# kamenbliznashki/chexpert

Measured on AMD Instinct MI355X. Metric: images/sec fwd+bwd DenseNet121 320x320 bf16 (per-GPU rate in config.images_per_sec_per_gpu), higher is better.
Workload: dtype bf16; 1 GPU; densenet121 bf16 1xMI355X 320x320 bs=256 per GPU, U-Ones labels (BASELINE configs[1]); 14 classes; random-init weights, synthetic uint8 X-rays; per_gpu_batch=256, global_batch=256, parallelism=dp1, rccl_ranks=1, capture_failed=0, launch=hipGraph replay

## Files before the change

chexpert_amd/_lib.py:

```python
import ctypes as C
import os

_HERE = os.path.dirname(os.path.abspath(__file__))
LIB_PATH = os.path.join(_HERE, "libchexpert_hip.so")

PRO_NONE, PRO_AFFINE_RELU, PRO_AFFINE2, PRO_JOIN = 0, 1, 2, 3
MODE_CONV, MODE_POOL2, MODE_STEM = 0, 1, 2
EPI_STORE, EPI_MASK, EPI_JOIN = 0, 1, 2

_vp, _fp, _i32 = C.c_void_p, C.c_void_p, C.c_int32


class CxConv(C.Structure):
    _fields_ = [("x", _vp), ("x2", _vp), ("w", _vp), ("y", _vp),
                ("pa", _fp), ("pb", _fp), ("pc", _fp),
                ("stat_sum", _fp), ("stat_sq", _fp),
                ("ex", _vp), ("e_sc", _fp), ("e_sh", _fp), ("e_mu", _fp), ("e_r", _fp), ("e_scale", _fp),
                ("B", _i32), ("H", _i32), ("W", _i32), ("Ho", _i32), ("Wo", _i32),
                ("K", _i32), ("N", _i32),
                ("ldx", _i32), ("ldx2", _i32), ("ldy", _i32), ("ldex", _i32),
                ("kh", _i32), ("kw", _i32), ("stride", _i32), ("pad", _i32),
                ("prologue", _i32), ("mode", _i32), ("epilogue", _i32), ("accumulate", _i32), ("tstride", _i32),
                ("stat_replicas", _i32), ("stat_rstride", _i32), ("stat_det", _i32), ("dtype", _i32),
                ("pro_out", _vp), ("ldpo", _i32), ("dil", _i32), ("emask", _vp),
                ("x3", _vp), ("po_lo", _vp), ("po_mask", _vp), ("kernel_hint", _i32), ("pad2_", _i32)]


class CxWgrad(C.Structure):
    _fields_ = [("g", _vp), ("g2", _vp), ("x", _vp), ("dw", _fp),
                ("ga", _fp), ("gb", _fp), ("gc", _fp), ("pa", _fp), ("pb", _fp),
                ("B", _i32), ("H", _i32), ("W", _i32), ("Ho", _i32), ("Wo", _i32), ("K", _i32), ("N", _i32),
                ("ldg", _i32), ("ldg2", _i32), ("ldx", _i32),
                ("kh", _i32), ("kw", _i32), ("stride", _i32), ("pad", _i32),
                ("g_prologue", _i32), ("x_prologue", _i32), ("mode", _i32), ("splits", _i32), ("dtype", _i32), ("dil", _i32),
                ("scratch", _fp), ("scratch_floats", C.c_int64), ("kernel_hint", _i32), ("pad_", _i32)]


WGRAD_BATCH_MAX = 24


class CxWgradBatch(C.Structure):
    _fields_ = [("g", _vp * WGRAD_BATCH_MAX), ("x", _vp * WGRAD_BATCH_MAX), ("pa", _fp * WGRAD_BATCH_MAX), ("pb", _fp * WGRAD_BATCH_MAX),
                ("dw", _fp * WGRAD_BATCH_MAX), ("n", _i32), ("pad_", _i32)]


class CxChanMapDesc(C.Structure):
    _fields_ = [("real_off", C.c_int64), ("pad_off", C.c_int64), ("O", _i32), ("taps", _i32), ("Ireal", _i32), ("Ipad", _i32),
                ("c0r", _i32), ("c0p", _i32), ("k", _i32), ("kp", _i32), ("split", _i32), ("shift", _i32)]


class CxPackDesc(C.Structure):
    _fields_ = [("src_off", C.c_int64), ("dst_off", C.c_int64), ("O", _i32), ("I", _i32), ("kh", _i32), ("kw", _i32),
                ("transpose", _i32), ("stem", _i32)]


class CxReduceDesc(C.Structure):
    _fields_ = [("dw", _fp), ("slab", _fp), ("total", C.c_int64), ("splits", _i32), ("vec", _i32), ("first_block", _i32), ("pad_", _i32),
                ("cols", _i32), ("dw_ld", _i32), ("pad2_", C.c_int64)]


_f, _sz, _i = C.c_float, C.c_size_t, C.c_int
SIGNATURES = {
    "cx_abi_version": [],
    "cx_last_pro_out": [],
    "cx_last_kernel": [],
    "cx_wgrad_defer": [C.c_int],
    "cx_wgrad_defer_take": [C.POINTER(CxReduceDesc), C.c_int, C.POINTER(C.c_int64)],
    "cx_last_slab_floats": [],
    "cx_dw_reduce_table": [_vp, C.c_int, C.c_int64, _vp],
    "cx_error_string": [_i],
    "cx_conv_gemm": [C.POINTER(CxConv), _vp],
    "cx_conv3x3_wgrad_batch": [C.POINTER(CxWgrad), C.POINTER(CxWgradBatch), _vp],
    "cx_chan_map_table": [_vp, _vp, _vp, _i, _i, _i, _vp],
    "cx_conv_wgrad": [C.POINTER(CxWgrad), _vp],
    "cx_stem_input_grad": [_vp] * 7 + [_i] * 13 + [_vp],
    "cx_conv1x1_dgrad_wgrad": [C.POINTER(CxConv), _vp, _vp],
    "cx_conv1x1_dgrad_wgrad_ws": [C.POINTER(CxConv), _vp, _vp, C.c_int64, _vp],
    "cx_conv1x1_dgrad_wgrad_ld_ws": [C.POINTER(CxConv), _vp, _i, _vp, C.c_int64, _vp],
    "cx_conv1x1_dgrad_wgrad_pair_ws": [C.POINTER(CxConv), C.POINTER(CxConv), _vp, _i, _vp, _vp, C.c_int64, _vp],
    "cx_pack_weights": [_vp, _vp, _i, _i, _i, _i, _i, _i, _vp],
    "cx_pack_weights_table": [_vp, _vp, _vp, _i, _vp],
    "cx_nchw3_to_nhwc4": [_vp, _vp, _i, _i, _i, _vp],
    "cx_u8_to_nhwc4": [_vp, _vp, _sz, _f, _f, _vp],
    "cx_bn_coef": [_vp, _vp, _f, _vp, _vp, _f, _f, _vp, _vp, _vp, _vp, _vp, _vp, _i, _i, _i, _vp],
    "cx_bn_coef_moments": [_vp, _vp, _f, _vp, _vp, _f, _f, _vp, _vp, _vp, _vp, _i, _vp, _vp, _i, _i, _i, _i, _vp],
    "cx_last_stat_rows": [],
    "cx_bnrelu_maxpool_fwd_f32": [_vp, _vp, _vp, _vp, _vp, _vp, _vp, _i, _i, _i, _i, _i, _i, _vp],
    "cx_bnrelu_maxpool_bwd_f32": [_vp, _vp, _vp, _vp, _vp, _vp, _vp, _vp, _vp, _vp, _vp, _vp, _vp, _vp, _i, _i, _i, _i, _i, _i, _i, _vp],
    "cx_head_fwd_f32": [_vp, _vp, _vp, _vp, _vp, _vp, _vp, _i, _i, _i, _i, _i, _vp],
    "cx_gap_relu_bn_bwd_f32": [_vp, _vp, _vp, _vp, _vp, _vp, _vp, _vp, _vp, _vp, _i, _i, _i, _i, _i, _i, _vp],
    "cx_unpool2_mask_f32": [_vp, _vp, _vp, _vp, _vp, _vp, _vp, _vp, _vp, _vp, _i, _i, _i, _i, _i, _i, _i, _i, _vp],
    "cx_pack_weights_table_f32": [_vp, _vp, _vp, _i, _vp],
    "cx_nchw3_to_nhwc4_f32": [_vp, _vp, _i, _i, _i, _vp],
    "cx_u8_to_nhwc4_f32": [_vp, _vp, _sz, _f, _f, _vp],
    "cx_u8_jitter": [_vp, _vp, _i, _i, _vp, _vp, _vp, _vp],
    "cx_u8_affine": [_vp, _vp, _i, _i, _i, _vp, _i, _vp],
    "cx_u8_mix": [_vp, _vp, _i, _i, _i, _vp, _vp, _vp, _i, _vp],
    "cx_target_mix": [_vp, _vp, _i, _i, _vp, _vp, _vp],
    "cx_u8_clahe_lut": [_vp, _vp, _i, _i, _i, _i, _i, _i, _vp],
    "cx_u8_clahe_apply": [_vp, _vp, _vp, _i, _i, _i, _i, _i, _vp],
    "cx_bn_coef_eval": [_vp, _vp, _vp, _vp, _f, _vp, _vp, _vp, _vp, _i, _vp],
    "cx_bn_bwd_coef": [_vp, _vp, _f, _vp, _vp, _vp, _vp, _vp, _vp, _vp, _vp, _vp, _vp, _i, _i, _i, _vp, _vp, _vp, _i, _i, _vp],
    "cx_bn_bwd_coef_eval": [_vp] * 7 + [_f] + [_vp] * 5 + [_i] * 3 + [_vp] * 3 + [_i, _i, _vp],
    "cx_bn_bwd_slice_coef": [_vp, _vp, _vp, _vp, _vp, _vp, _vp, _i, _vp],
    "cx_bnrelu_maxpool_fwd": [_vp, _vp, _vp, _vp, _vp, _vp, _vp, _i, _i, _i, _i, _i, _i, _vp],
    "cx_bnrelu_maxpool_bwd": [_vp, _vp, _vp, _vp, _vp, _vp, _vp, _vp, _vp, _vp, _vp, _vp, _vp, _vp, _i, _i, _i, _i, _i, _i, _i, _vp],
    "cx_head_fwd": [_vp, _vp, _vp, _vp, _vp, _vp, _vp, _i, _i, _i, _i, _i, _vp],
    "cx_bce_fwd_bwd": [_vp, _vp, _vp, _vp, _vp, _f, _i, _i, _vp],
    "cx_bce_masked_fwd_bwd": [_vp, _vp, _vp, _vp, _vp, _vp, _f, _i, _i, _vp],
    "cx_aucm_fwd_bwd": [_vp, _vp, _vp, _vp, _f, _vp, _vp, _vp, _vp, _f, _i, _i, _vp],
    "cx_aucm_aux_step": [_vp, _vp, _vp, _i, _vp],
    "cx_asl_fwd_bwd": [_vp, _vp, _vp, _vp, _vp, _vp, _vp, _f, _i, _i, _vp],
    "cx_mc3_fwd_bwd": [_vp, _vp, _vp, _vp, _vp, _vp, _f, _i, _i, _vp],
    "cx_mc3_collapse": [_vp, _vp, _vp, _i, _i, _vp],
    "cx_softmax_ce_fwd_bwd": [_vp, _vp, _vp, _vp, _vp, _f, _i, _i, _vp],
    "cx_head_bwd": [_vp, _vp, _vp, _vp, _vp, _vp, _i, _i, _i, _vp],
    "cx_gap_relu_bn_bwd": [_vp, _vp, _vp, _vp, _vp, _vp, _vp, _vp, _vp, _vp, _i, _i, _i, _i, _i, _i, _vp],
    "cx_unpool2_mask": [_vp, _vp, _vp, _vp, _vp, _vp, _vp, _vp, _vp, _vp, _i, _i, _i, _i, _i, _i, _i, _i, _vp],
    "cx_affine2_inplace": [_vp, _vp, _vp, _vp, _vp, _sz, _i, _vp],
    "cx_affine2_relu": [_vp, _vp, _vp, _vp, _vp, _vp, _sz, _i, _vp],
    "cx_relu_bwd_stats": [_vp, _vp, _vp, _vp, _vp, _vp, _vp, _vp, _vp, _vp, _vp, _vp, _sz, _i, _i, _vp],
    "cx_dropout_slice_fwd": [_vp, _i, C.c_int64, _i, C.c_float, _vp, C.c_uint32, _vp, _vp, _i, _vp],
    "cx_dropout_slice_fwd_f32": [_vp, _i, C.c_int64, _i, C.c_float, _vp, C.c_uint32, _vp, _vp, _i, _vp],
    "cx_dropout_slice_bwd": [_vp, _i, _vp, _i, _vp, _vp, _vp, C.c_int64, _i, C.c_float, _vp, C.c_uint32, _vp],
    "cx_dropout_slice_bwd_f32": [_vp, _i, _vp, _i, _vp, _vp, _vp, C.c_int64, _i, C.c_float, _vp, C.c_uint32, _vp],
    "cx_join_fwd": [_vp, _vp, _vp, _vp, _vp, _vp, _vp, _vp, _vp, _sz, _i, _vp],
    "cx_affine2_relu_mask": [_vp, _vp, _vp, _vp, _vp, _vp, _vp, _sz, _i, _vp],
    "cx_affine2_relu_mask_f32": [_vp, _vp, _vp, _vp, _vp, _vp, _vp, _sz, _i, _vp],
    "cx_relu_bwd_stats_mask": [_vp, _vp, _vp, _vp, _vp, _vp, _vp, _vp, _vp, _vp, _vp, _vp, _vp, _sz, _i, _i, _vp],
    "cx_relu_bwd_stats_mask_f32": [_vp, _vp, _vp, _vp, _vp, _vp, _vp, _vp, _vp, _vp, _vp, _vp, _vp, _sz, _i, _i, _vp],
    "cx_adam_step": [_vp, _vp, _vp, _vp, _sz, _f, _f, _f, _f, _f, _i, _f, _vp],
    "cx_sgd_nesterov_step": [_vp, _vp, _vp, _sz, _f, _f, _f, _i, _f, _vp],
    "cx_rmsprop_step": [_vp, _vp, _vp, _vp, _sz, _f, _f, _f, _f, _f, _f, _vp],
    "cx_adam_step_dev": [_vp, _vp, _vp, _vp, _sz, _vp, _f, _f, _f, _f, _f, _vp],
    "cx_sgd_nesterov_step_dev": [_vp, _vp, _vp, _sz, _vp, _f, _f, _f, _vp],
    "cx_rmsprop_step_dev": [_vp, _vp, _vp, _vp, _sz, _vp, _f, _f, _f, _f, _f, _vp],
    "cx_optim_tick": [_vp, _vp],
    "cx_grad_norm_partials": [_sz],
    "cx_grad_norm": [_vp, _sz, _f, _f, _i, _vp, _sz, _vp, _vp],
    "cx_adam_step_ex": [_vp, _vp, _vp, _vp, _sz, _f, _f, _f, _f, _f, _i, _f, _vp, _vp, _f, _i, _i, _vp],
    "cx_sgd_nesterov_step_ex": [_vp, _vp, _vp, _sz, _f, _f, _f, _i, _i, _f, _vp, _vp, _f, _i, _i, _vp],
    "cx_rmsprop_step_ex": [_vp, _vp, _vp, _vp, _sz, _f, _f, _f, _f, _f, _i, _f, _vp, _vp, _f, _i, _i, _vp],
    "cx_adam_step_dev_ex": [_vp, _vp, _vp, _vp, _sz, _vp, _f, _f, _f, _f, _f, _vp, _vp, _f, _i, _i, _vp],
    "cx_sgd_nesterov_step_dev_ex": [_vp, _vp, _vp, _sz, _vp, _f, _f, _f, _vp, _vp, _f, _i, _i, _vp],
    "cx_rmsprop_step_dev_ex": [_vp, _vp, _vp, _vp, _sz, _vp, _f, _f, _f, _f, _f, _vp, _vp, _f, _i, _i, _vp],
    "cx_optim_item_vec4": [],
    "cx_grad_norm_items": [_vp, _sz, _vp, _i, _vp, _i, _f, _f, _i, _vp, _vp, _vp, _vp, _vp],
    "cx_adam_step_items": [_vp, _vp, _vp, _vp, _sz, _vp, _i, _vp, _i, _i, _vp, _f, _i, _f, _f, _f, _f, _vp, _vp, _f, _i, _i, _vp],
    "cx_sgd_nesterov_step_items": [_vp, _vp, _vp, _sz, _vp, _i, _vp, _i, _i, _vp, _f, _i, _f, _f, _vp, _vp, _f, _i, _i, _vp],
    "cx_rmsprop_step_items": [_vp, _vp, _vp, _vp, _sz, _vp, _i, _vp, _i, _i, _vp, _f, _i, _f, _f, _f, _f, _vp, _vp, _f, _i, _i, _vp],
    "cx_aa_attention_fwd": [_vp, _vp, _vp, _vp, _vp, _i, _i, _i, _i, _i, _i, _i, _vp],
    "cx_aa_attention_fwd_f32": [_vp, _vp, _vp, _vp, _vp, _i, _i, _i, _i, _i, _i, _i, _vp],
    "cx_aa_attention_weights": [_vp, _vp, _vp, _vp, _vp, _i, _i, _i, _i, _i, _i, _i, _vp],
    "cx_aa_attention_weights_f32": [_vp, _vp, _vp, _vp, _vp, _i, _i, _i, _i, _i, _i, _i, _vp],
    "cx_aa_attention_bwd": [_vp, _vp, _vp, _vp, _vp, _vp, _vp, _vp, _vp, _i, _i, _i, _i, _i, _i, _i, _vp, C.c_int64, _vp],
    "cx_aa_attention_bwd_f32": [_vp, _vp, _vp, _vp, _vp, _vp, _vp, _vp, _vp, _i, _i, _i, _i, _i, _i, _i, _vp, C.c_int64, _vp],
    "cx_aa_outproj_fwd": [_vp, _vp, _vp, _i, _vp, _vp, _sz, _i, _i, _i, _vp],
    "cx_aa_outproj_fwd_f32": [_vp, _vp, _vp, _i, _vp, _vp, _sz, _i, _i, _i, _vp],
    "cx_aa_outproj_bwd": [_vp, _i, _vp, _i, _vp, _vp, _vp, _vp, _vp, _vp, _vp, _sz, _i, _vp, C.c_int64, _vp],
    "cx_aa_outproj_bwd_f32": [_vp, _i, _vp, _i, _vp, _vp, _vp, _vp, _vp, _vp, _vp, _sz, _i, _vp, C.c_int64, _vp],
    "cx_rows_reduce": [_vp, _vp, _i, _i, _i, _i, _vp],
    "cx_stats_bc": [_vp, _vp, _vp, _i, _i, _i, _i, _vp],
    "cx_stats_bc_f32": [_vp, _vp, _vp, _i, _i, _i, _i, _vp],
    "cx_affine_relu_bc": [_vp, _vp, _vp, _vp, _i, _i, _i, _i, _vp],
    "cx_affine_relu_bc_f32": [_vp, _vp, _vp, _vp, _i, _i, _i, _i, _vp],
    "cx_in_relu_bwd": [_vp, _vp, _vp, _vp, _vp, _vp, _vp, _i, _i, _i, _i, _i, _vp],
    "cx_in_relu_bwd_f32": [_vp, _vp, _vp, _vp, _vp, _vp, _vp, _i, _i, _i, _i, _i, _vp],
    "cx_f32_to_bf16": [_vp, _vp, _sz, _vp],
    "cx_nchw3_to_nhwc8": [_vp, _vp, _i, _i, _i, _vp],
    "cx_nchw3_to_nhwc8_f32": [_vp, _vp, _i, _i, _i, _vp],
    "cx_u8_to_nhwc8": [_vp, _vp, _sz, _f, _f, _vp],
    "cx_u8_to_nhwc8_f32": [_vp, _vp, _sz, _f, _f, _vp],
    "cx_dwconv_fwd": [_vp] * 7 + [_i] * 8 + [_vp],
    "cx_dwconv_fwd_f32": [_vp] * 7 + [_i] * 8 + [_vp],
    "cx_dwconv_dgrad": [_vp] * 14 + [_i] * 9 + [_vp],
    "cx_dwconv_dgrad_f32": [_vp] * 14 + [_i] * 9 + [_vp],
    "cx_dwconv_wgrad": [_vp] * 9 + [_i] * 7 + [_vp, C.c_int64, _vp],
    "cx_dwconv_wgrad_f32": [_vp] * 9 + [_i] * 7 + [_vp, C.c_int64, _vp],
    "cx_pool_head_fwd": [_vp] * 6 + [_i] * 6 + [_vp],
    "cx_pool_head_fwd_f32": [_vp] * 6 + [_i] * 6 + [_vp],
    "cx_pool_head_bwd": [_vp] * 13 + [_i] * 8 + [_vp],
    "cx_pool_head_bwd_f32": [_vp] * 13 + [_i] * 8 + [_vp],
    "cx_pool_p_grad": [_vp] * 5 + [_i, _i, _vp],
    "cx_gap_affine_act": [_vp, _vp, _vp, _vp, _i, _i, _i, _i, _vp, C.c_int64, _vp],
    "cx_gap_affine_act_f32": [_vp, _vp, _vp, _vp, _i, _i, _i, _i, _vp, C.c_int64, _vp],
    "cx_se_fwd": [_vp] * 7 + [_i, _i, _i, _vp],
    "cx_se_bwd_fused": [_vp] * 15 + [_i, _i, _i, _i, _vp, C.c_int64, _vp, C.c_int64, _vp],
    "cx_se_bwd_fused_f32": [_vp] * 15 + [_i, _i, _i, _i, _vp, C.c_int64, _vp, C.c_int64, _vp],
    "cx_gap_se_fwd": [_vp] * 10 + [_i, _i, _i, _i, _i, _vp, C.c_int64, _vp],
    "cx_gap_se_fwd_f32": [_vp] * 10 + [_i, _i, _i, _i, _i, _vp, C.c_int64, _vp],
    "cx_se_bwd": [_vp] * 11 + [_i, _i, _i, _vp, C.c_int64, _vp],
    "cx_scale_act_bc": [_vp, _vp, _vp, _vp, _vp, _i, _i, _i, _vp],
    "cx_scale_act_bc_f32": [_vp, _vp, _vp, _vp, _vp, _i, _i, _i, _vp],
    "cx_se_bwd_reduce": [_vp, _vp, _vp, _vp, _vp, _i, _i, _i, _vp, C.c_int64, _vp],
    "cx_se_bwd_reduce_f32": [_vp, _vp, _vp, _vp, _vp, _i, _i, _i, _vp, C.c_int64, _vp],
    "cx_se_act_bwd": [_vp] * 11 + [_i, _i, _i, _i, _vp],
    "cx_se_act_bwd_f32": [_vp] * 11 + [_i, _i, _i, _i, _vp],
    "cx_bn_lin_bwd_stats": [_vp] * 6 + [_sz, _i, _i, _vp],
    "cx_bn_lin_bwd_stats_f32": [_vp] * 6 + [_sz, _i, _i, _vp],
    "cx_affine2_out": [_vp, _vp, _vp, _vp, _vp, _vp, _sz, _vp, _sz, _i, _vp],
    "cx_affine2_out_f32": [_vp, _vp, _vp, _vp, _vp, _vp, _sz, _vp, _sz, _i, _vp],
    "cx_scale_rows": [_vp, _vp, _sz, _vp, _sz, _i, _vp],
    "cx_scale_rows_f32": [_vp, _vp, _sz, _vp, _sz, _i, _vp],
    "cx_dropout_mask": [_vp, _sz, _f, C.c_ulonglong, _vp],
    "cx_dropout_mask_dev": [_vp, _sz, _f, C.c_ulonglong, _vp, _vp],
    "cx_counter_add": [_vp, C.c_ulonglong, _vp],
    "cx_mul_f32": [_vp, _vp, _vp, _sz, _vp],
    "cx_linear_fwd": [_vp, _vp, _vp, _vp, _i, _i, _i, _vp],
    "cx_gradcam_map": [_vp, _vp, _vp, _vp, _vp, _i, _i, _i, _i, _i, _vp],
    "cx_cam_norm_upsample": [_vp, _vp, _i, _i, _i, _i, _i, _vp],
    "cx_class_cam": [_vp] * 6 + [_i] * 9 + [_vp],
    "cx_class_cam_f32": [_vp] * 6 + [_i] * 9 + [_vp],
    "cx_boot_counts": [_vp, _i, _i, _i, _i, C.c_uint64, _vp],
    "cx_boot_auc": [_vp, _i, _i, _vp, C.POINTER(C.c_int64), C.POINTER(C.c_int32), _i, _vp, _vp, _vp, _i, _vp],
    "cx_boot_sweep": [_vp, _i, _i, _vp, C.POINTER(C.c_int64), C.POINTER(C.c_int32), _i, C.POINTER(C.c_int32), C.POINTER(C.c_int32), _i,
                      _vp, _vp, _vp, _vp, _i, _vp],
    "cx_calib_fit": [_vp, _vp, _i, _i, _i, _i, C.c_double, _i, _vp, _vp],
    "cx_boot_calib": [_vp, _i, _i, _vp, _vp, C.POINTER(C.c_int64), C.POINTER(C.c_int32), _i, _i, _vp, _vp, _vp, _vp, _i, _vp],
    "cx_delong_place": [_vp, C.POINTER(C.c_int64), C.POINTER(C.c_int32), _i, _i, _vp, _i, _vp],
    "cx_delong_gram": [_vp, _i, _i, _i, _vp, _vp],
    "cx_sal_points": [_vp, _vp, _f, _f, _f, _vp, _vp, _vp, C.c_uint64, C.c_uint64, _vp, _i, _i, _i, _i, _vp],
    "cx_sal_accumulate": [_vp, _vp, _vp, _vp, _i, _i, _i, _i, _i, _i, _vp],
    "cx_sal_finish": [_vp, _vp, _vp, _f, _f, _f, _vp, _vp, _vp, _vp, _i, _i, _i, _i, _i, _i, _vp],
    "cx_fill_f32": [_vp, _f, _sz, _vp],
    "cx_copy_stream": [_vp, _vp, _sz, _vp],
    "cx_affine_to_f32_nchw": [_vp, _vp, _vp, _i, _vp, _i, _i, _i, _i, _i, _vp],
    "cx_bf16_to_f32_nchw": [_vp, _vp, _i, _i, _i, _i, _i, _vp],
}

_lib = None


def lib():
    global _lib
    if _lib is None:
        if not os.path.exists(LIB_PATH):
            raise RuntimeError(
                "chexpert_amd: %s is missing -- build it with `python -c 'import __graft_entry__ as g; g.build()'` "
                "(hipcc --offload-arch=gfx950).  There is no CPU fallback." % LIB_PATH)
        import torch
        l = C.CDLL(LIB_PATH)
        for name, args in SIGNATURES.items():
            fn = getattr(l, name)
            fn.argtypes = args
            fn.restype = C.c_char_p if name in ("cx_error_string", "cx_last_kernel") else C.c_int
        if l.cx_abi_version() != 10:
            raise RuntimeError("chexpert_amd: ABI version mismatch")
        _lib = l
    return _lib


def check(rc, what):
    if rc != 0:
        raise RuntimeError("%s failed: %s (code %d)" % (what, lib().cx_error_string(rc).decode(), rc))


def ptr(t):
    return None if t is None else t.data_ptr()


def stream_ptr():
    import torch
    return torch.cuda.current_stream().cuda_stream


def require_cuda(*tensors):
    for t in tensors:
        if t is not None and not t.is_cuda:
            raise RuntimeError("chexpert_amd kernels run on the GPU only (got a %s tensor); there is no CPU fallback"
                               % t.device)
```

chexpert_amd/csrc/conv1x1_fwdk.hip:

```cpp
#include <cstdlib>
#include "common.h"

namespace {

constexpr int BM = 128, BN = 128;
constexpr int WAVES_N = 2, TM = 2, TN = 2;
constexpr int EPITCH = BN + 4;

template <int BK, int PRO>
__global__ __launch_bounds__(256, 2) void pw_fwdk_kernel(const CxConv p, const int M) {
  constexpr int PITCH = BK * 2 + 16;
  constexpr int CPR = BK / 8;
  constexpr int RPP = 256 / CPR;
  constexpr int NL = 128 / RPP;
  constexpr int A_BYTES = BM * PITCH;
  extern __shared__ __attribute__((aligned(16))) char smem[];
  float* coef = reinterpret_cast<float*>(smem);
  char* At = smem + 2 * p.K * 4;
  char* Bt = At + A_BYTES;
  const int tid = threadIdx.x, lane = tid & 63, wave = tid >> 6;
  const int wm = wave / WAVES_N, wn = wave % WAVES_N;
  const int mt = xcd_remap(blockIdx.x, gridDim.x);
  const bf16* __restrict__ X = reinterpret_cast<const bf16*>(p.x);
  const bf16* __restrict__ Wp = reinterpret_cast<const bf16*>(p.w);
  bf16* __restrict__ Y = reinterpret_cast<bf16*>(p.y);

  if (PRO == CX_PRO_AFFINE_RELU)
    for (int i = tid; i < p.K; i += 256) { coef[i] = p.pa[i]; coef[p.K + i] = p.pb[i]; }

  const int q = tid % CPR, r0 = tid / CPR;
  const int nsteps = (p.K + BK - 1) / BK;
  uint4 ra[NL], rw[NL];
  bool kok = true;
  auto issue_loads = [&](int s) __attribute__((always_inline)) {
    const int c = s * BK + q * 8;
    kok = c < p.K;
    const int cc = kok ? c : 0;
#pragma unroll
    for (int i = 0; i < NL; ++i) {
      const int row = r0 + RPP * i;
      const int m = mt * BM + row;
      const int mc = m < M ? m : M - 1;
      ra[i] = *reinterpret_cast<const uint4*>(X + (size_t)mc * p.ldx + cc);
      rw[i] = *reinterpret_cast<const uint4*>(Wp + (size_t)row * p.K + cc);
    }
  };
  auto write_stage = [&](int s) __attribute__((always_inline)) {
    const int c0 = s * BK + q * 8;
#pragma unroll
    for (int i = 0; i < NL; ++i) {
      const int row = r0 + RPP * i;
      U128 o;
      if (!kok || mt * BM + row >= M) {
        o.u = make_uint4(0, 0, 0, 0);
      } else if (PRO == CX_PRO_NONE) {
        o.u = ra[i];
      } else {
        o.u = cx_affine_relu8(ra[i], coef + c0, coef + p.K + c0);
      }
      *reinterpret_cast<uint4*>(At + row * PITCH + q * 16) = o.u;
      *reinterpret_cast<uint4*>(Bt + row * PITCH + q * 16) = kok ? rw[i] : make_uint4(0, 0, 0, 0);
    }
  };

  f32x16 acc[TM][TN];
#pragma unroll
  for (int i = 0; i < TM; ++i)
#pragma unroll
    for (int j = 0; j < TN; ++j)
#pragma unroll
      for (int r = 0; r < 16; ++r) acc[i][j][r] = 0.f;

  issue_loads(0);
  __syncthreads();
  const int lrow = lane & 31, lh = lane >> 5;
  for (int s = 0; s < nsteps; ++s) {
    write_stage(s);
    __syncthreads();
    if (s + 1 < nsteps) issue_loads(s + 1);
#pragma unroll
    for (int kk = 0; kk < BK / 16; ++kk) {
      bf16x8 af[TM], bfr[TN];
#pragma unroll
      for (int i = 0; i < TM; ++i) af[i] = *reinterpret_cast<const bf16x8*>(At + ((wm * TM + i) * 32 + lrow) * PITCH + kk * 32 + lh * 16);
#pragma unroll
      for (int j = 0; j < TN; ++j) bfr[j] = *reinterpret_cast<const bf16x8*>(Bt + ((wn * TN + j) * 32 + lrow) * PITCH + kk * 32 + lh * 16);
#pragma unroll
      for (int i = 0; i < TM; ++i)
#pragma unroll
        for (int j = 0; j < TN; ++j) acc[i][j] = __builtin_amdgcn_mfma_f32_32x32x16_bf16(af[i], bfr[j], acc[i][j], 0, 0, 0);
    }
    __syncthreads();
  }

  constexpr int ECPR = BN / 8, ERPP = 256 / ECPR, NPASS = 64 / ERPP;
  const int cq = tid % ECPR, rr = tid / ECPR;
  float* etile = reinterpret_cast<float*>(At);
  float s1[8], s2[8];
#pragma unroll
  for (int j = 0; j < 8; ++j) s1[j] = s2[j] = 0.f;
  const bool want_stats = p.stat_sum != nullptr;
#pragma unroll
  for (int half = 0; half < 2; ++half) {
    if (wm == half) {
#pragma unroll
      for (int i = 0; i < TM; ++i)
#pragma unroll
        for (int j = 0; j < TN; ++j)
#pragma unroll
          for (int r = 0; r < 16; ++r) {
            const int row = i * 32 + (r & 3) + 8 * (r >> 2) + 4 * lh;
            const int col = (wn * TN + j) * 32 + lrow;
            etile[row * EPITCH + col] = acc[i][j][r];
          }
    }
    __syncthreads();
#pragma unroll
    for (int pass = 0; pass < NPASS; ++pass) {
      const int row = pass * ERPP + rr;
      const int m = mt * BM + half * 64 + row;
      if (m < M) {
        const float4 v0 = *reinterpret_cast<const float4*>(etile + row * EPITCH + cq * 8);
        const float4 v1 = *reinterpret_cast<const float4*>(etile + row * EPITCH + cq * 8 + 4);
        const float v[8] = {v0.x, v0.y, v0.z, v0.w, v1.x, v1.y, v1.z, v1.w};
        U128 o;
        {
          uint32_t w4[4];
#pragma unroll
          for (int j = 0; j < 4; ++j) {
            w4[j] = cx_packbf(v[2 * j], v[2 * j + 1]);
            const float rl = cx_bf_lo(w4[j]), rh = cx_bf_hi(w4[j]);
            s1[2 * j] += rl;
            s1[2 * j + 1] += rh;
            s2[2 * j] += rl * rl;
            s2[2 * j + 1] += rh * rh;
          }
          o.u = make_uint4(w4[0], w4[1], w4[2], w4[3]);
        }
        *reinterpret_cast<uint4*>(Y + (size_t)m * p.ldy + cq * 8) = o.u;
      }
    }
    __syncthreads();
  }
  if (want_stats) {
#pragma unroll
    for (int j = 0; j < 8; ++j) {
#pragma unroll
      for (int d = ECPR; d < 64; d <<= 1) {
        s1[j] += __shfl_xor(s1[j], d);
        s2[j] += __shfl_xor(s2[j], d);
      }
    }
    float* scratch = reinterpret_cast<float*>(At);
    wg_stat_begin<4>(scratch, BN, tid, 256);
    if (lane < ECPR) {
#pragma unroll
      for (int j = 0; j < 8; ++j) wg_stat_put(scratch, BN, wave, cq * 8 + j, s1[j], s2[j]);
    }
    wg_stat_end<4>(scratch, BN, tid, 256, p.stat_sum, p.stat_sq, p.stat_det, (int)blockIdx.x, p.stat_replicas, p.stat_rstride, 0, p.N);
  }
}

template <int PRO, int D>
__global__ __launch_bounds__(256, 2) void pw_fwdp_kernel(const CxConv p, const int M) {
  constexpr int BK = 64;
  constexpr int PITCH = BK * 2 + 16;
  constexpr int CPR = BK / 8;
  constexpr int RPP = 256 / CPR;
  constexpr int NL = 128 / RPP;
  constexpr int A_BYTES = BM * PITCH;
  extern __shared__ __attribute__((aligned(16))) char smem[];
  float* coef = reinterpret_cast<float*>(smem);
  char* At = smem + 2 * p.K * 4;
  char* Bt = At + A_BYTES;
  const int tid = threadIdx.x, lane = tid & 63, wave = tid >> 6;
  const int wm = wave / WAVES_N, wn = wave % WAVES_N;
  const int mt = xcd_remap(blockIdx.x, gridDim.x);
  const bf16* __restrict__ X = reinterpret_cast<const bf16*>(p.x);
  const bf16* __restrict__ Wp = reinterpret_cast<const bf16*>(p.w);
  bf16* __restrict__ Y = reinterpret_cast<bf16*>(p.y);
  if (PRO == CX_PRO_AFFINE_RELU)
    for (int i = tid; i < p.K; i += 256) { coef[i] = p.pa[i]; coef[p.K + i] = p.pb[i]; }
  const int q = tid % CPR, r0 = tid / CPR;
  const int nsteps = (p.K + BK - 1) / BK;
  const bf16* xr[NL];
  const bf16* wr[NL];
#pragma unroll
  for (int i = 0; i < NL; ++i) {
    const int row = r0 + RPP * i;
    const int m = mt * BM + row;
    xr[i] = X + (size_t)(m < M ? m : M - 1) * p.ldx + q * 8;
    wr[i] = Wp + (size_t)row * p.K + q * 8;
  }
  uint4 ra[D][NL], rw[D][NL];
  auto issue = [&](uint4 (&a)[NL], uint4 (&w)[NL], int s) __attribute__((always_inline)) {
    const int sc = s < nsteps ? s : nsteps - 1;
    int c = sc * BK;
    if (c + q * 8 >= p.K) c = p.K - BK;
#pragma unroll
    for (int i = 0; i < NL; ++i) {
      a[i] = *reinterpret_cast<const uint4*>(xr[i] + c);
      w[i] = *reinterpret_cast<const uint4*>(wr[i] + c);
    }
  };
  auto stage = [&](const uint4 (&a)[NL], const uint4 (&w)[NL], int s) __attribute__((always_inline)) {
    const int c0 = s * BK + q * 8;
    const bool kok = c0 < p.K;
#pragma unroll
    for (int i = 0; i < NL; ++i) {
      const int row = r0 + RPP * i;
      U128 o;
      if (!kok || mt * BM + row >= M) {
        o.u = make_uint4(0, 0, 0, 0);
      } else if (PRO == CX_PRO_NONE) {
        o.u = a[i];
      } else {
        o.u = cx_affine_relu8(a[i], coef + c0, coef + p.K + c0);
      }
      *reinterpret_cast<uint4*>(At + row * PITCH + q * 16) = o.u;
      *reinterpret_cast<uint4*>(Bt + row * PITCH + q * 16) = kok ? w[i] : make_uint4(0, 0, 0, 0);
    }
  };
  f32x16 acc[TM][TN];
#pragma unroll
  for (int i = 0; i < TM; ++i)
#pragma unroll
    for (int j = 0; j < TN; ++j)
#pragma unroll
      for (int r = 0; r < 16; ++r) acc[i][j][r] = 0.f;
#pragma unroll
  for (int d = 0; d < D; ++d) issue(ra[d], rw[d], d);
  __syncthreads();
  const int lrow = lane & 31, lh = lane >> 5;
  for (int s0 = 0; s0 < nsteps; s0 += D) {
#pragma unroll
    for (int d = 0; d < D; ++d) {
      const int s = s0 + d;
      if (s < nsteps) {
        stage(ra[d], rw[d], s);
        __syncthreads();
        issue(ra[d], rw[d], s + D);
#pragma unroll
        for (int kk = 0; kk < BK / 16; ++kk) {
          bf16x8 af[TM], bfr[TN];
#pragma unroll
          for (int i = 0; i < TM; ++i) af[i] = *reinterpret_cast<const bf16x8*>(At + ((wm * TM + i) * 32 + lrow) * PITCH + kk * 32 + lh * 16);
#pragma unroll
          for (int j = 0; j < TN; ++j) bfr[j] = *reinterpret_cast<const bf16x8*>(Bt + ((wn * TN + j) * 32 + lrow) * PITCH + kk * 32 + lh * 16);
#pragma unroll
          for (int i = 0; i < TM; ++i)
#pragma unroll
            for (int j = 0; j < TN; ++j) acc[i][j] = __builtin_amdgcn_mfma_f32_32x32x16_bf16(af[i], bfr[j], acc[i][j], 0, 0, 0);
        }
        __syncthreads();
      }
    }
  }
  constexpr int ECPR = BN / 8, ERPP = 256 / ECPR, NPASS = 64 / ERPP;
  const int cq = tid % ECPR, rr = tid / ECPR;
  float* etile = reinterpret_cast<float*>(At);
  float s1[8], s2[8];
#pragma unroll
  for (int j = 0; j < 8; ++j) s1[j] = s2[j] = 0.f;
  const bool want_stats = p.stat_sum != nullptr;
#pragma unroll
  for (int half = 0; half < 2; ++half) {
    if (wm == half) {
#pragma unroll
      for (int i = 0; i < TM; ++i)
#pragma unroll
        for (int j = 0; j < TN; ++j)
#pragma unroll
          for (int r = 0; r < 16; ++r) {
            const int row = i * 32 + (r & 3) + 8 * (r >> 2) + 4 * lh;
            const int col = (wn * TN + j) * 32 + lrow;
            etile[row * EPITCH + col] = acc[i][j][r];
          }
    }
    __syncthreads();
#pragma unroll
    for (int pass = 0; pass < NPASS; ++pass) {
      const int row = pass * ERPP + rr;
      const int m = mt * BM + half * 64 + row;
      if (m < M) {
        const float4 v0 = *reinterpret_cast<const float4*>(etile + row * EPITCH + cq * 8);
        const float4 v1 = *reinterpret_cast<const float4*>(etile + row * EPITCH + cq * 8 + 4);
        const float v[8] = {v0.x, v0.y, v0.z, v0.w, v1.x, v1.y, v1.z, v1.w};
        U128 o;
        {
          uint32_t w4[4];
#pragma unroll
          for (int j = 0; j < 4; ++j) {
            w4[j] = cx_packbf(v[2 * j], v[2 * j + 1]);
            const float rl = cx_bf_lo(w4[j]), rh = cx_bf_hi(w4[j]);
            s1[2 * j] += rl;
            s1[2 * j + 1] += rh;
            s2[2 * j] += rl * rl;
            s2[2 * j + 1] += rh * rh;
          }
          o.u = make_uint4(w4[0], w4[1], w4[2], w4[3]);
        }
        *reinterpret_cast<uint4*>(Y + (size_t)m * p.ldy + cq * 8) = o.u;
      }
    }
    __syncthreads();
  }
  if (want_stats) {
#pragma unroll
    for (int j = 0; j < 8; ++j) {
#pragma unroll
      for (int d = ECPR; d < 64; d <<= 1) {
        s1[j] += __shfl_xor(s1[j], d);
        s2[j] += __shfl_xor(s2[j], d);
      }
    }
    float* scratch = reinterpret_cast<float*>(At);
    wg_stat_begin<4>(scratch, BN, tid, 256);
    if (lane < ECPR) {
#pragma unroll
      for (int j = 0; j < 8; ++j) wg_stat_put(scratch, BN, wave, cq * 8 + j, s1[j], s2[j]);
    }
    wg_stat_end<4>(scratch, BN, tid, 256, p.stat_sum, p.stat_sq, p.stat_det, (int)blockIdx.x, p.stat_replicas, p.stat_rstride, 0, p.N);
  }
}

template <int PRO, int D>
int launch_fwdp(const CxConv& p, hipStream_t st) {
  const long long M = (long long)p.B * p.Ho * p.Wo;
  const int m_tiles = (int)((M + BM - 1) / BM);
  const size_t stage = (size_t)2 * BM * (64 * 2 + 16);
  const size_t epi = (size_t)64 * EPITCH * 4;
  const size_t smem = (size_t)2 * p.K * 4 + (stage > epi ? stage : epi) + 2 * BN * 4;
  static bool attr = false;
  if (!attr) {
    (void)hipFuncSetAttribute(reinterpret_cast<const void*>(&pw_fwdp_kernel<PRO, D>), hipFuncAttributeMaxDynamicSharedMemorySize, 80 * 1024);
    attr = true;
  }
  if (smem > 80 * 1024) return CX_ESHAPE;
  if (const int e = stat_rows_check(p, m_tiles)) return e;
  CX_KTAG("pw_fwdp_kernel<%d, %d>", PRO, D);
  hipLaunchKernelGGL((pw_fwdp_kernel<PRO, D>), dim3(m_tiles), dim3(256), smem, st, p, (int)M);
  return launch_status();
}

template <int BK, int PRO>
int launch_fwdk(const CxConv& p, hipStream_t st) {
  const long long M = (long long)p.B * p.Ho * p.Wo;
  const int m_tiles = (int)((M + BM - 1) / BM);
  const size_t stage = (size_t)2 * BM * (BK * 2 + 16);
  const size_t epi = (size_t)64 * EPITCH * 4;
  const size_t smem = (size_t)2 * p.K * 4 + (stage > epi ? stage : epi) + 2 * BN * 4;
  static bool attr = false;
  if (!attr) {
    (void)hipFuncSetAttribute(reinterpret_cast<const void*>(&pw_fwdk_kernel<BK, PRO>), hipFuncAttributeMaxDynamicSharedMemorySize, 80 * 1024);
    attr = true;
  }
  if (smem > 80 * 1024) return CX_ESHAPE;
  if (const int e = stat_rows_check(p, m_tiles)) return e;
  CX_KTAG("pw_fwdk_kernel<%d, %d>", BK, PRO);
  hipLaunchKernelGGL((pw_fwdk_kernel<BK, PRO>), dim3(m_tiles), dim3(256), smem, st, p, (int)M);
  return launch_status();
}

}

int cx_try_pw_fwdk(const CxConv& p, hipStream_t st, bool* handled) {
  *handled = false;
  if (p.mode != CX_MODE_CONV || p.kh != 1 || p.kw != 1 || p.stride != 1 || p.pad != 0 || p.tstride > 1) return 0;
  if (p.epilogue != CX_EPI_STORE || p.accumulate || p.N != 128 || p.K <= 256 || p.K > 1280) return 0;
  if (p.prologue != CX_PRO_AFFINE_RELU && p.prologue != CX_PRO_NONE) return 0;
  if ((long long)p.B * p.Ho * p.Wo > 200000) return 0;
  *handled = true;
  static const int pipe = cx_diag_int("CX_FWDK_PIPE", 2);
  if (pipe == 2 && p.K % 32 == 0 && p.K >= 512)
    return p.prologue == CX_PRO_AFFINE_RELU ? launch_fwdp<CX_PRO_AFFINE_RELU, 2>(p, st) : launch_fwdp<CX_PRO_NONE, 2>(p, st);
  if (pipe == 3 && p.K % 32 == 0 && p.K >= 192)
    return p.prologue == CX_PRO_AFFINE_RELU ? launch_fwdp<CX_PRO_AFFINE_RELU, 3>(p, st) : launch_fwdp<CX_PRO_NONE, 3>(p, st);
  if (pipe == 4 && p.K % 32 == 0 && p.K >= 256)
    return p.prologue == CX_PRO_AFFINE_RELU ? launch_fwdp<CX_PRO_AFFINE_RELU, 4>(p, st) : launch_fwdp<CX_PRO_NONE, 4>(p, st);
  return p.prologue == CX_PRO_AFFINE_RELU ? launch_fwdk<128, CX_PRO_AFFINE_RELU>(p, st) : launch_fwdk<128, CX_PRO_NONE>(p, st);
}
```

chexpert_amd/csrc/conv1x1_xs.hip:

```cpp
#include <cstdlib>
#include "common.h"

namespace {

#ifndef XS_ABL
#define XS_ABL 0
#endif
constexpr int XS_PITCH = 144;
constexpr int XS_STAGE = 128 * XS_PITCH;
constexpr int XS_EP = 68;
typedef uint32_t xs_u32x4 __attribute__((ext_vector_type(4)));

template <int PRO>
struct XsCoef {
  static constexpr int v = (PRO == CX_PRO_NONE) ? 0 : (PRO == CX_PRO_AFFINE_RELU ? 2 : 3);
};

template <int PRO>
__device__ __forceinline__ uint32_t xs_pro(const uint32_t g, const uint32_t y, const float* ca, const float* cb, const float* cc, const int j) {
  if (PRO == CX_PRO_NONE) return g;
  if (PRO == CX_PRO_AFFINE_RELU)
    return cx_relu_pk(cx_packbf(fmaf(cx_bf_lo(g), ca[2 * j], cb[2 * j]), fmaf(cx_bf_hi(g), ca[2 * j + 1], cb[2 * j + 1])));
  return cx_packbf(fmaf(cx_bf_lo(g), ca[2 * j], fmaf(cx_bf_lo(y), cb[2 * j], cc[2 * j])),
                   fmaf(cx_bf_hi(g), ca[2 * j + 1], fmaf(cx_bf_hi(y), cb[2 * j + 1], cc[2 * j + 1])));
}

template <int KC, int PRO, int EPI>
__global__ __launch_bounds__(256) __attribute__((amdgpu_waves_per_eu(2, 2))) void pw_xs_kernel(const CxConv p, const int M, const int rpt) {
  constexpr int K = KC * 64, NKK = K / 16;
  constexpr int NCO = XsCoef<PRO>::v;
  extern __shared__ __attribute__((aligned(16))) char smem[];
  float* coef = reinterpret_cast<float*>(smem);
  char* Bs = smem + NCO * K * 4;
  float* Es = reinterpret_cast<float*>(Bs + 2 * XS_STAGE);
  float* St = Es + 4 * 32 * XS_EP;
  const int tid = threadIdx.x, lane = tid & 63, wave = tid >> 6;
  const int wm = wave >> 1, wn = wave & 1;
  const int lrow = lane & 31, lh = lane >> 5;
  const int mt = xcd_remap(blockIdx.x, gridDim.x);
  const int m0 = mt * rpt;
  const char* __restrict__ X = reinterpret_cast<const char*>(p.x);
  const char* __restrict__ X2 = reinterpret_cast<const char*>(p.x2);
  const char* __restrict__ Wb = reinterpret_cast<const char*>(p.w);
  bf16* __restrict__ Y = reinterpret_cast<bf16*>(p.y);

  if (PRO != CX_PRO_NONE) {
    for (int i = tid; i < K; i += 256) {
      coef[i] = p.pa[i];
      coef[K + i] = p.pb[i];
      if (PRO == CX_PRO_AFFINE2) coef[2 * K + i] = p.pc[i];
    }
  }

  const int q = tid & 7, r0 = tid >> 3;
  const int NC = p.N >> 7, T = NC * KC;
  const char* wthr = Wb + ((size_t)r0 * K + q * 8) * 2;
  xs_u32x4 wreg[4];
  auto issue_w = [&](int t) __attribute__((always_inline)) {
    t = t < T ? t : T - 1;
    const int nc = t / KC, ks = t - nc * KC;
    const char* src = wthr + ((size_t)nc * 128 * K + ks * 64) * 2;
#pragma unroll
    for (int u = 0; u < 4; ++u) wreg[u] = *reinterpret_cast<const xs_u32x4*>(src + (size_t)u * 32 * K * 2);
  };
  auto store_w = [&](int stage) __attribute__((always_inline)) {
#pragma unroll
    for (int u = 0; u < 4; ++u) *reinterpret_cast<xs_u32x4*>(Bs + stage * XS_STAGE + (r0 + 32 * u) * XS_PITCH + q * 16) = wreg[u];
  };
  issue_w(0);

  xs_u32x4 afr[2][NKK];
  bool rok[2];
#pragma unroll
  for (int i = 0; i < 2; ++i) {
    const int rl = wm * 64 + i * 32 + lrow;
    const int m = m0 + rl;
    rok[i] = rl < rpt && m < M;
    const size_t mc = rok[i] ? m : M - 1;
    const char* xp = X + (mc * p.ldx + lh * 8) * 2;
#pragma unroll
    for (int kk = 0; kk < NKK; ++kk) afr[i][kk] = *reinterpret_cast<const xs_u32x4*>(xp + kk * 32);
  }
  __syncthreads();
  if (PRO != CX_PRO_NONE) {
    const float* cf = coef;
#pragma unroll
    for (int i = 0; i < 2; ++i) {
      xs_u32x4 sec[PRO == CX_PRO_AFFINE2 ? NKK : 1];
      if (PRO == CX_PRO_AFFINE2) {
        const size_t mc = rok[i] ? m0 + wm * 64 + i * 32 + lrow : M - 1;
        const char* xp = X2 + (mc * p.ldx2 + lh * 8) * 2;
#pragma unroll
        for (int kk = 0; kk < NKK; ++kk) sec[kk] = *reinterpret_cast<const xs_u32x4*>(xp + kk * 32);
      }
#pragma unroll
      for (int kk = 0; kk < NKK; ++kk) {
        uint32_t z;
        asm volatile("v_and_b32 %0, 0, %1" : "=v"(z) : "v"(afr[i][kk][0]));
        const int c0 = kk * 16 + lh * 8 + (int)z;
        float ca[8], cb[8], cc[8];
        *reinterpret_cast<float4*>(ca) = *reinterpret_cast<const float4*>(cf + c0);
        *reinterpret_cast<float4*>(ca + 4) = *reinterpret_cast<const float4*>(cf + c0 + 4);
        *reinterpret_cast<float4*>(cb) = *reinterpret_cast<const float4*>(cf + K + c0);
        *reinterpret_cast<float4*>(cb + 4) = *reinterpret_cast<const float4*>(cf + K + c0 + 4);
        if (PRO == CX_PRO_AFFINE2) {
          *reinterpret_cast<float4*>(cc) = *reinterpret_cast<const float4*>(cf + 2 * K + c0);
          *reinterpret_cast<float4*>(cc + 4) = *reinterpret_cast<const float4*>(cf + 2 * K + c0 + 4);
        }
#pragma unroll
        for (int j = 0; j < 4; ++j) afr[i][kk][j] = xs_pro<PRO>(afr[i][kk][j], PRO == CX_PRO_AFFINE2 ? sec[kk][j] : 0u, ca, cb, cc, j);
        asm volatile("" : "+v"(afr[i][kk]));
      }
    }
  }
#pragma unroll
  for (int i = 0; i < 2; ++i) {
    const uint32_t keep = rok[i] ? 0xffffffffu : 0u;
#pragma unroll
    for (int kk = 0; kk < NKK; ++kk) afr[i][kk] &= keep;
  }

  store_w(0);
  issue_w(1);

  const int cq = lane & 7;
  float* Ew = Es + wave * 32 * XS_EP;
  const bool want_stats = p.stat_sum != nullptr;
  const int srow = p.stat_det ? mt : (int)blockIdx.x;

  for (int nc = 0; nc < NC; ++nc) {
    f32x16 acc[2][2];
#pragma unroll
    for (int i = 0; i < 2; ++i)
#pragma unroll
      for (int j = 0; j < 2; ++j)
#pragma unroll
        for (int r = 0; r < 16; ++r) acc[i][j][r] = 0.f;
#pragma unroll
    for (int ks = 0; ks < KC; ++ks) {
      const int t = nc * KC + ks;
      __syncthreads();
      if (ks == 0 && nc > 0 && want_stats && tid < 128) {
        const float* s = St + ((nc - 1) & 1) * 512;
        const int n = (nc - 1) * 128 + tid;
        const float a = s[tid] + s[256 + tid];
        float b = s[128 + tid] + s[384 + tid];
        if (EPI == CX_EPI_JOIN) b = p.e_r[n] * (b - p.e_mu[n] * a);
        if (p.stat_det) {
          p.stat_sum[(size_t)srow * p.stat_rstride + n] = a;
          p.stat_sq[(size_t)srow * p.stat_rstride + n] = b;
        } else {
          const size_t rep = p.stat_replicas > 1 ? (size_t)(srow % p.stat_replicas) * p.stat_rstride : 0;
          atomicAdd(&p.stat_sum[rep + n], a);
          atomicAdd(&p.stat_sq[rep + n], b);
        }
      }
      const char* Bt = Bs + (t & 1) * XS_STAGE + (wn * 64 + lrow) * XS_PITCH + lh * 16;
#pragma unroll
      for (int kk = 0; kk < 4; ++kk) {
        const bf16x8 b0 = *reinterpret_cast<const bf16x8*>(Bt + kk * 32);
        const bf16x8 b1 = *reinterpret_cast<const bf16x8*>(Bt + 32 * XS_PITCH + kk * 32);
        const bf16x8 a0 = __builtin_bit_cast(bf16x8, afr[0][ks * 4 + kk]);
        const bf16x8 a1 = __builtin_bit_cast(bf16x8, afr[1][ks * 4 + kk]);
        acc[0][0] = __builtin_amdgcn_mfma_f32_32x32x16_bf16(a0, b0, acc[0][0], 0, 0, 0);
        acc[0][1] = __builtin_amdgcn_mfma_f32_32x32x16_bf16(a0, b1, acc[0][1], 0, 0, 0);
        acc[1][0] = __builtin_amdgcn_mfma_f32_32x32x16_bf16(a1, b0, acc[1][0], 0, 0, 0);
        acc[1][1] = __builtin_amdgcn_mfma_f32_32x32x16_bf16(a1, b1, acc[1][1], 0, 0, 0);
        if (kk == 1 && !(XS_ABL & 2)) {
          store_w((t + 1) & 1);
          issue_w(t + 2);
        }
      }
    }

    float s1[8], s2[8];
#pragma unroll
    for (int j = 0; j < 8; ++j) s1[j] = s2[j] = 0.f;
    const int ncol = nc * 128 + wn * 64 + cq * 8;
#pragma unroll
    for (int i = 0; i < ((XS_ABL & 1) ? 0 : 2); ++i) {
#pragma unroll
      for (int j = 0; j < 2; ++j)
#pragma unroll
        for (int r = 0; r < 16; ++r) Ew[((r & 3) + 8 * (r >> 2) + 4 * lh) * XS_EP + j * 32 + lrow] = acc[i][j][r];
#pragma unroll
      for (int u = 0; u < 4; ++u) {
        const int row = (lane >> 3) + 8 * u;
        const int rl = wm * 64 + i * 32 + row;
        const int m = m0 + rl;
        const float4 v0 = *reinterpret_cast<const float4*>(Ew + row * XS_EP + cq * 8);
        const float4 v1 = *reinterpret_cast<const float4*>(Ew + row * XS_EP + cq * 8 + 4);
        if (rl < rpt && m < M) {
          float t8[8] = {v0.x, v0.y, v0.z, v0.w, v1.x, v1.y, v1.z, v1.w};
          bf16* yp = Y + (size_t)m * p.ldy + ncol;
          if (EPI == CX_EPI_JOIN) {
            const uint4 old = *reinterpret_cast<const uint4*>(yp);
            const uint4 xv = *reinterpret_cast<const uint4*>(reinterpret_cast<const bf16*>(p.ex) + (size_t)m * p.ldex + ncol);
            const unsigned mk = p.emask[cx_side_chunk((size_t)m, ncol >> 3, (size_t)M, p.N)];
            const uint32_t ow[4] = {old.x, old.y, old.z, old.w}, xw[4] = {xv.x, xv.y, xv.z, xv.w};
            uint32_t w4[4];
#pragma unroll
            for (int j = 0; j < 4; ++j) {
              const uint32_t bits = mk >> (2 * j);
              const uint32_t keep = ((bits & 1u) ? 0x0000ffffu : 0u) | ((bits & 2u) ? 0xffff0000u : 0u);
              w4[j] = cx_packbf(t8[2 * j] + cx_bf_lo(ow[j]), t8[2 * j + 1] + cx_bf_hi(ow[j])) & keep;
              const float dl = cx_bf_lo(w4[j]), du = cx_bf_hi(w4[j]);
              s1[2 * j] += dl;
              s1[2 * j + 1] += du;
              s2[2 * j] = fmaf(dl, cx_bf_lo(xw[j]), s2[2 * j]);
              s2[2 * j + 1] = fmaf(du, cx_bf_hi(xw[j]), s2[2 * j + 1]);
            }
            *reinterpret_cast<uint4*>(yp) = make_uint4(w4[0], w4[1], w4[2], w4[3]);
          } else {
            if (p.accumulate) {
              const uint4 old = *reinterpret_cast<const uint4*>(yp);
              const uint32_t ow[4] = {old.x, old.y, old.z, old.w};
#pragma unroll
              for (int j = 0; j < 4; ++j) { t8[2 * j] += cx_bf_lo(ow[j]); t8[2 * j + 1] += cx_bf_hi(ow[j]); }
            }
            *reinterpret_cast<uint4*>(yp) = cx_pack8_stats(t8, true, true, s1, s2);
          }
        }
      }
    }
    if (XS_ABL & 1) {
      float t = 0.f;
#pragma unroll
      for (int r = 0; r < 16; ++r) t += acc[0][0][r] + acc[0][1][r] + acc[1][0][r] + acc[1][1][r];
      if (t == 1.2345f) Y[0] = f2bf(t);
    }
    if (want_stats) {
#pragma unroll
      for (int j = 0; j < 8; ++j) {
#pragma unroll
        for (int d = 8; d < 64; d <<= 1) {
          s1[j] += __shfl_xor(s1[j], d);
          s2[j] += __shfl_xor(s2[j], d);
        }
      }
      if (lane < 8) {
        float* s = St + (nc & 1) * 512 + wm * 256 + wn * 64 + cq * 8;
#pragma unroll
        for (int j = 0; j < 8; ++j) { s[j] = s1[j]; s[128 + j] = s2[j]; }
      }
    }
  }
  if (want_stats) {
    __syncthreads();
    if (tid < 128) {
      const float* s = St + ((NC - 1) & 1) * 512;
      const int n = (NC - 1) * 128 + tid;
      const float a = s[tid] + s[256 + tid];
      float b = s[128 + tid] + s[384 + tid];
      if (EPI == CX_EPI_JOIN) b = p.e_r[n] * (b - p.e_mu[n] * a);
      if (p.stat_det) {
        p.stat_sum[(size_t)srow * p.stat_rstride + n] = a;
        p.stat_sq[(size_t)srow * p.stat_rstride + n] = b;
      } else {
        const size_t rep = p.stat_replicas > 1 ? (size_t)(srow % p.stat_replicas) * p.stat_rstride : 0;
        atomicAdd(&p.stat_sum[rep + n], a);
        atomicAdd(&p.stat_sq[rep + n], b);
      }
    }
  }
}

template <int KC, int PRO, int EPI>
int launch_xs(const CxConv& p, hipStream_t st, int M, int rpt) {
  const int m_tiles = (M + rpt - 1) / rpt;
  const size_t smem = (size_t)XsCoef<PRO>::v * KC * 64 * 4 + 2 * XS_STAGE + 4 * 32 * XS_EP * 4 + 2 * 512 * 4;
  static bool attr = false;
  if (!attr) {
    (void)hipFuncSetAttribute(reinterpret_cast<const void*>(&pw_xs_kernel<KC, PRO, EPI>), hipFuncAttributeMaxDynamicSharedMemorySize, 80 * 1024);
    attr = true;
  }
  CX_KTAG("pw_xs_kernel<%d, %d, %d>", KC, PRO, EPI);
  hipLaunchKernelGGL((pw_xs_kernel<KC, PRO, EPI>), dim3(m_tiles), dim3(256), smem, st, p, M, rpt);
  return launch_status();
}

template <int PRO, int EPI>
int launch_xs_k(const CxConv& p, hipStream_t st, int M, int rpt) {
  if (p.K == 256) return launch_xs<4, PRO, EPI>(p, st, M, rpt);
  if (p.K == 128) return launch_xs<2, PRO, EPI>(p, st, M, rpt);
  return launch_xs<1, PRO, EPI>(p, st, M, rpt);
}

}

int cx_try_pw_xs(const CxConv& p, hipStream_t st, bool* handled) {
  *handled = false;
  static const int env_on = cx_diag_int("CX_XS", 1);
  const int hint_on = (p.kernel_hint & 0xff) - 1, hint_form = ((p.kernel_hint >> 8) & 0xff) - 1;
  if (hint_on == 0 || (hint_form >= 0 && hint_form != 5) || (!env_on && hint_form != 5)) return 0;
  if (p.mode != CX_MODE_CONV || p.dtype != CX_DT_BF16 || p.kh != 1 || p.kw != 1 || p.stride != 1 || p.pad != 0 || p.tstride > 1) return 0;
  if (p.K != 64 && p.K != 128 && p.K != 256) return 0;
  if ((p.N % 128) || p.N < 2 * p.K || p.N < 256) return 0;
  if (p.epilogue != CX_EPI_STORE && !(p.epilogue == CX_EPI_JOIN && p.prologue == CX_PRO_AFFINE2 && hint_form == 5)) return 0;
  if (p.prologue != CX_PRO_NONE && p.prologue != CX_PRO_AFFINE_RELU && p.prologue != CX_PRO_AFFINE2) return 0;
  if (p.Ho != p.H || p.Wo != p.W) return 0;
  const long long M = (long long)p.B * p.H * p.W;
  if (M >= (1ll << 31)) return 0;
  const long long full = (M + 127) / 128;
  const long long tiles = (full + 511) / 512 * 512;
  int rpt = (int)((M + tiles - 1) / tiles);
  rpt = (rpt + 3) & ~3;
  rpt = rpt < 64 ? 64 : rpt > 128 ? 128 : rpt;
  if (p.stat_det && p.stat_sum && ((M + rpt - 1) / rpt > p.stat_replicas)) rpt = 128;
  if (const int e = stat_rows_check(p, (int)((M + rpt - 1) / rpt))) {
    if (hint_form == 5) { *handled = true; return e; }
    return 0;
  }
  *handled = true;
  if (p.epilogue == CX_EPI_JOIN) return launch_xs_k<CX_PRO_AFFINE2, CX_EPI_JOIN>(p, st, (int)M, rpt);
  if (p.prologue == CX_PRO_NONE) return launch_xs_k<CX_PRO_NONE, CX_EPI_STORE>(p, st, (int)M, rpt);
  if (p.prologue == CX_PRO_AFFINE_RELU) return launch_xs_k<CX_PRO_AFFINE_RELU, CX_EPI_STORE>(p, st, (int)M, rpt);
  return launch_xs_k<CX_PRO_AFFINE2, CX_EPI_STORE>(p, st, (int)M, rpt);
}
```

chexpert_amd/csrc/conv_gemm.hip:

```cpp
#include "common.h"

namespace {

constexpr int BM = 128;
constexpr int BK = 32;
constexpr int PITCH = 80;
constexpr int A_BYTES = BM * PITCH;

template <int BN>
struct Geo {
  static constexpr int WAVES_N = (BN >= 64) ? 2 : 1;
  static constexpr int WAVES_M = 4 / WAVES_N;
  static constexpr int TM = BM / (WAVES_M * 32);
  static constexpr int TN = BN / (WAVES_N * 32);
  static constexpr int B_BYTES = BN * PITCH;
  static constexpr int STAGE = A_BYTES + B_BYTES;
  static constexpr int EPITCH = BN + 4;
  static constexpr int EPI_BYTES = 64 * EPITCH * 4;
  static constexpr int MAIN_BYTES = (2 * STAGE > EPI_BYTES) ? 2 * STAGE : EPI_BYTES;
};

template <int PRO>
struct NCoef {
  static constexpr int v = (PRO == CX_PRO_NONE) ? 0 : (PRO == CX_PRO_AFFINE_RELU ? 2 : 3);
// ... 63 lines not shown
    (void)s;
    const int tap = q_tap, kc = q_kc;
    const int dy = (MODE == CX_MODE_CONV) ? q_dy * cdil : tap;
    const int dx = (MODE == CX_MODE_CONV) ? q_dx * cdil : 0;
    w_kc = kc;
#pragma unroll
    for (int i = 0; i < 2; ++i) {
      if (MODE == CX_MODE_STEM) {
        const int iy = riy[i] + dy, ix = rix[i];
        av[i] = rvalid[i] & (iy >= 0) & (iy < p.H) & (ix >= 0) & (ix < p.W);
        const int cy = av[i] ? iy : 0, cx = av[i] ? ix : 0;
        ra[i][0] = *reinterpret_cast<const uint4*>(X + ((size_t)(rb[i] * p.H + cy) * p.W + cx) * 4);
      } else if (MODE == CX_MODE_POOL2) {
        av[i] = rvalid[i];
#pragma unroll
        for (int a = 0; a < 4; ++a) {
          const size_t pix = (size_t)(rb[i] * p.H + riy[i] + (a >> 1)) * p.W + rix[i] + (a & 1);
          ra[i][a] = *reinterpret_cast<const uint4*>(X + pix * p.ldx + kc * BK + qa * 8);
        }
      } else {
        int iy = riy[i] + dy, ix = rix[i] + dx;
        bool ok = rvalid[i] & (iy >= 0) & (ix >= 0) & (((iy | ix) & ts_sh) == 0);
        iy >>= ts_sh;
        ix >>= ts_sh;
        const bool kok = kc * BK + qa * 8 < p.K;
        av[i] = ok & (iy < p.H) & (ix < p.W) & kok;
        const int cy = av[i] ? iy : 0, cx = av[i] ? ix : 0;
        const int ck = kok ? kc * BK + qa * 8 : 0;
        const size_t pix = (size_t)(rb[i] * p.H + cy) * p.W + cx;
        ra[i][0] = *reinterpret_cast<const uint4*>(X + pix * p.ldx + ck);
        if (PRO == CX_PRO_AFFINE2) ra2[i] = *reinterpret_cast<const uint4*>(X2 + pix * p.ldx2 + ck);
      }
    }
#pragma unroll
    for (int i = 0; i < 2; ++i) {
      const int nb = (tid >> 2) + 64 * i;
      if (nb < BN) {
        const int n = n0 + nb;
        const bool kok = (MODE == CX_MODE_STEM) || (kc * BK + qa * 8 < p.K);
        wv[i] = n < p.N && kok;
        const int nc = wv[i] ? n : 0;
        const size_t off = ((size_t)tap * p.N + nc) * (size_t)(MODE == CX_MODE_STEM ? BK : p.K) + (kok ? kc * BK + qa * 8 : 0);
        rbw[i] = *reinterpret_cast<const uint4*>(Wp + off);
      }
    }
    if (++q_kc == kpt) {
      q_kc = 0;
      ++q_tap;
      if (++q_dx == p.kw) {
        q_dx = 0;
        ++q_dy;
      }
    }
  };

  auto write_stage = [&](int s, int buf) {
    (void)s;
    const int tap = 0, kc = w_kc;
    char* A = tiles + buf * G::STAGE;
    char* Bt = A + A_BYTES;
    const int c0 = kc * BK + qa * 8;
#pragma unroll
    for (int i = 0; i < 2; ++i) {
      U128 o;
      if (!av[i]) {
        o.u = make_uint4(0, 0, 0, 0);
      } else if (PRO == CX_PRO_NONE) {
        o.u = ra[i][0];
      } else if (PRO == CX_PRO_AFFINE_RELU) {
        float acc[8];
#pragma unroll
        for (int j = 0; j < 8; ++j) acc[j] = 0.f;
#pragma unroll
        for (int a = 0; a < NSRC; ++a) {
          const uint32_t w4[4] = {ra[i][a].x, ra[i][a].y, ra[i][a].z, ra[i][a].w};
#pragma unroll
          for (int j = 0; j < 4; ++j) {
            acc[2 * j] += fmaxf(fmaf(cx_bf_lo(w4[j]), coef[c0 + 2 * j], coef[p.K + c0 + 2 * j]), 0.f);
            acc[2 * j + 1] += fmaxf(fmaf(cx_bf_hi(w4[j]), coef[c0 + 2 * j + 1], coef[p.K + c0 + 2 * j + 1]), 0.f);
          }
        }
        {
          const float sc_ = NSRC == 4 ? 0.25f : 1.f;
          o.u = make_uint4(cx_packbf(acc[0] * sc_, acc[1] * sc_), cx_packbf(acc[2] * sc_, acc[3] * sc_), cx_packbf(acc[4] * sc_, acc[5] * sc_),
                           cx_packbf(acc[6] * sc_, acc[7] * sc_));
        }
      } else {
        o.u = cx_affine2_8(ra[i][0], ra2[i], coef + c0, coef + p.K + c0, coef + 2 * p.K + c0);
      }
      *reinterpret_cast<uint4*>(A + ((tid >> 2) + 64 * i) * PITCH + qa * 16) = o.u;
    }
#pragma unroll
    for (int i = 0; i < 2; ++i) {
      const int nb = (tid >> 2) + 64 * i;
      if (nb < BN) *reinterpret_cast<uint4*>(Bt + nb * PITCH + qa * 16) = wv[i] ? rbw[i] : make_uint4(0, 0, 0, 0);
    }
    (void)tap;
  };

  f32x16 acc[G::TM][G::TN];
#pragma unroll
  for (int i = 0; i < G::TM; ++i)
#pragma unroll
    for (int j = 0; j < G::TN; ++j)
#pragma unroll
      for (int r = 0; r < 16; ++r) acc[i][j][r] = 0.f;

  issue_loads(0);
  __syncthreads();
  write_stage(0, 0);
  __syncthreads();

  const int lrow = lane & 31, lh = lane >> 5;
  for (int s = 0; s < nsteps; ++s) {
    const int buf = s & 1;
    if (s + 1 < nsteps) issue_loads(s + 1);
    const char* A = tiles + buf * G::STAGE;
    const char* Bt = A + A_BYTES;
#pragma unroll
    for (int kk = 0; kk < 2; ++kk) {
      bf16x8 af[G::TM], bfr[G::TN];
#pragma unroll
      for (int i = 0; i < G::TM; ++i)
        af[i] = *reinterpret_cast<const bf16x8*>(A + ((wm * G::TM + i) * 32 + lrow) * PITCH + kk * 32 + lh * 16);
#pragma unroll
      for (int j = 0; j < G::TN; ++j)
        bfr[j] = *reinterpret_cast<const bf16x8*>(Bt + ((wn * G::TN + j) * 32 + lrow) * PITCH + kk * 32 + lh * 16);
#pragma unroll
      for (int i = 0; i < G::TM; ++i)
#pragma unroll
        for (int j = 0; j < G::TN; ++j)
          acc[i][j] = __builtin_amdgcn_mfma_f32_32x32x16_bf16(af[i], bfr[j], acc[i][j], 0, 0, 0);
    }
    if (s + 1 < nsteps) write_stage(s + 1, buf ^ 1);
    __syncthreads();
  }

  constexpr int CPR = BN / 8;
  constexpr int RPP = 256 / CPR;
  const int cq = tid % CPR, rr = tid / CPR;
  const int nch = n0 + cq * 8;
  const bool nvalid = nch < p.N;
  float* etile = reinterpret_cast<float*>(tiles);
  bf16* __restrict__ Y = reinterpret_cast<bf16*>(p.y);
  const bf16* __restrict__ EX = reinterpret_cast<const bf16*>(p.ex);
  float s1[8], s2[8];
#pragma unroll
  for (int j = 0; j < 8; ++j) s1[j] = s2[j] = 0.f;
  float esc[8], esh[8], emu[8], er[8], escale[8];
  if (EPI == CX_EPI_MASK && nvalid) {
#pragma unroll
    for (int j = 0; j < 8; ++j) {
      esc[j] = p.e_sc[nch + j];
      esh[j] = p.e_sh[nch + j];
      emu[j] = p.e_mu[nch + j];
      er[j] = p.e_r[nch + j];
      escale[j] = p.e_scale[nch + j];
    }
  }
  const bool want_stats = p.stat_sum != nullptr;

  constexpr int NPASS = 64 / RPP;
  U128 xv[2][NPASS], old[2][NPASS];
  {
    const int ncl = nvalid ? nch : 0;
    if (EPI == CX_EPI_MASK) {
#pragma unroll
      for (int half = 0; half < 2; ++half)
#pragma unroll
        for (int pass = 0; pass < NPASS; ++pass) {
          const int m = mt * BM + half * 64 + pass * RPP + rr;
          const int mc = m < M ? m : M - 1;
          xv[half][pass].u = *reinterpret_cast<const uint4*>(EX + (size_t)mc * p.ldex + ncl);
        }
    }
    if (p.accumulate) {
#pragma unroll
      for (int half = 0; half < 2; ++half)
#pragma unroll
        for (int pass = 0; pass < NPASS; ++pass) {
          const int m = mt * BM + half * 64 + pass * RPP + rr;
          const int mc = m < M ? m : M - 1;
          old[half][pass].u = *reinterpret_cast<const uint4*>(Y + (size_t)mc * p.ldy + ncl);
        }
    } else {
#pragma unroll
      for (int half = 0; half < 2; ++half)
#pragma unroll
        for (int pass = 0; pass < NPASS; ++pass) old[half][pass].u = make_uint4(0, 0, 0, 0);
    }
  }

#pragma unroll
  for (int half = 0; half < 2; ++half) {
    if (wm / (G::WAVES_M / 2) == half) {
      const int wml = wm % (G::WAVES_M / 2);
#pragma unroll
      for (int i = 0; i < G::TM; ++i)
#pragma unroll
        for (int j = 0; j < G::TN; ++j)
#pragma unroll
          for (int r = 0; r < 16; ++r) {
            const int row = (wml * G::TM + i) * 32 + (r & 3) + 8 * (r >> 2) + 4 * lh;
            const int col = (wn * G::TN + j) * 32 + lrow;
            etile[row * G::EPITCH + col] = acc[i][j][r];
          }
    }
    __syncthreads();
#pragma unroll
    for (int pass = 0; pass < NPASS; ++pass) {
      const int row = pass * RPP + rr;
      const int m = mt * BM + half * 64 + row;
      if (m < M && nvalid) {
        const float4 v0 = *reinterpret_cast<const float4*>(etile + row * G::EPITCH + cq * 8);
        const float4 v1 = *reinterpret_cast<const float4*>(etile + row * G::EPITCH + cq * 8 + 4);
        float v[8] = {v0.x, v0.y, v0.z, v0.w, v1.x, v1.y, v1.z, v1.w};
        U128 o;
        const uint32_t ow[4] = {old[half][pass].u.x, old[half][pass].u.y, old[half][pass].u.z, old[half][pass].u.w};
        if (EPI == CX_EPI_STORE) {
          float t[8];
#pragma unroll
          for (int j = 0; j < 4; ++j) { t[2 * j] = v[2 * j] + cx_bf_lo(ow[j]); t[2 * j + 1] = v[2 * j + 1] + cx_bf_hi(ow[j]); }
          o.u = cx_pack8_stats(t, true, true, s1, s2);
        } else {
          const uint32_t xw[4] = {xv[half][pass].u.x, xv[half][pass].u.y, xv[half][pass].u.z, xv[half][pass].u.w};
          uint32_t w4[4];
#pragma unroll
          for (int j = 0; j < 4; ++j) {
            const float xl = cx_bf_lo(xw[j]), xu = cx_bf_hi(xw[j]);
            const float dl = (fmaf(xl, esc[2 * j], esh[2 * j]) > 0.f) ? v[2 * j] : 0.f;
            const float du = (fmaf(xu, esc[2 * j + 1], esh[2 * j + 1]) > 0.f) ? v[2 * j + 1] : 0.f;
            s1[2 * j] += dl;
            s1[2 * j + 1] += du;
            s2[2 * j] += dl * (xl - emu[2 * j]) * er[2 * j];
            s2[2 * j + 1] += du * (xu - emu[2 * j + 1]) * er[2 * j + 1];
            w4[j] = cx_packbf(fmaf(escale[2 * j], dl, cx_bf_lo(ow[j])), fmaf(escale[2 * j + 1], du, cx_bf_hi(ow[j])));
          }
          o.u = make_uint4(w4[0], w4[1], w4[2], w4[3]);
        }
        *reinterpret_cast<uint4*>(Y + (size_t)m * p.ldy + nch) = o.u;
      }
    }
    __syncthreads();
  }

  if (want_stats) {
#pragma unroll
    for (int j = 0; j < 8; ++j) {
#pragma unroll
      for (int d = CPR; d < 64; d <<= 1) {
        s1[j] += __shfl_xor(s1[j], d);
        s2[j] += __shfl_xor(s2[j], d);
      }
    }
    float* scratch = reinterpret_cast<float*>(tiles);
    wg_stat_begin<4>(scratch, BN, tid, 256);
    if (lane < CPR) {
#pragma unroll
      for (int j = 0; j < 8; ++j) wg_stat_put(scratch, BN, wave, cq * 8 + j, s1[j], s2[j]);
    }
    wg_stat_end<4>(scratch, BN, tid, 256, p.stat_sum, p.stat_sq, p.stat_det, p.stat_det ? mt : (int)blockIdx.x, p.stat_replicas,
                   p.stat_rstride, n0, p.N);
  }
}

template <int BN, int PRO, int MODE, int EPI>
int launch(const CxConv& p, hipStream_t st) {
  using G = Geo<BN>;
  const long long M = (long long)p.B * p.Ho * p.Wo;
  const int m_tiles = (int)((M + BM - 1) / BM);
  const int n_tiles = (p.N + BN - 1) / BN;
  const size_t smem = (size_t)NCoef<PRO>::v * p.K * 4 + G::MAIN_BYTES + 2 * BN * 4;
  if (smem > 160 * 1024) return CX_ESHAPE;
  if (const int e = stat_rows_check(p, m_tiles)) return e;
  static bool attr_set = false;
  if (!attr_set && smem > 64 * 1024) {
    (void)hipFuncSetAttribute(reinterpret_cast<const void*>(&conv_gemm_kernel<BN, PRO, MODE, EPI>),
                        hipFuncAttributeMaxDynamicSharedMemorySize, 160 * 1024);
    attr_set = true;
  }
  CX_KTAG("conv_gemm_kernel<%d, %d, %d, %d>", BN, PRO, MODE, EPI);
  hipLaunchKernelGGL((conv_gemm_kernel<BN, PRO, MODE, EPI>), dim3(m_tiles * n_tiles), dim3(256), smem, st, p, (int)M,
                     n_tiles);
  return launch_status();
}

template <int PRO, int MODE, int EPI>
int launch_bn(const CxConv& p, hipStream_t st) {
  if (p.N % 128 == 0) return launch<128, PRO, MODE, EPI>(p, st);
  if (p.N == 32) return launch<32, PRO, MODE, EPI>(p, st);
  return launch<64, PRO, MODE, EPI>(p, st);
}

}

int cx_try_pc_fwd(const CxConv& p, hipStream_t st, bool* handled);
int cx_try_ring_fwd(const CxConv& p, hipStream_t st, bool* handled);
int cx_try_strip_fwd(const CxConv& p, hipStream_t st, bool* handled);
int cx_try_ring_dgrad(const CxConv& p, hipStream_t st, bool* handled);
int cx_try_strip_dgrad(const CxConv& p, hipStream_t st, bool* handled);
int cx_try_pw_dgrad(const CxConv& p, hipStream_t st, bool* handled);
int cx_try_pw_fwd(const CxConv& p, hipStream_t st, bool* handled);
int cx_try_pw_fwdk(const CxConv& p, hipStream_t st, bool* handled);
int cx_try_pw_xs(const CxConv& p, hipStream_t st, bool* handled);
int cx_try_stem_fwd(const CxConv& p, hipStream_t st, bool* handled);
int cx_conv_gemm_f32(const CxConv& p, hipStream_t st);
int cx_try_conv_mm(const CxConv& p, hipStream_t st, bool* handled);

thread_local int cx_tl_stat_rows = 0;
thread_local int cx_tl_pro_out = 0;
thread_local char cx_tl_kernel[112] = "";
extern "C" const char* cx_last_kernel(void) { return cx_tl_kernel; }
extern "C" int cx_last_stat_rows(void) { return cx_tl_stat_rows; }
extern "C" int cx_last_pro_out(void) { return cx_tl_pro_out; }

static inline int dil_extent(int k, int dil) { return (dil > 1 ? dil : 1) * (k - 1) + 1; }

extern "C" int cx_conv_gemm(const CxConv* pp, void* stream) {
  if (!pp) return CX_EINVAL;
  const CxConv& p = *pp;
  cx_tl_pro_out = 0;
  if (!p.x || !p.w || !p.y) return CX_EINVAL;
  if (p.B <= 0 || p.H <= 0 || p.W <= 0 || p.Ho <= 0 || p.Wo <= 0) return CX_ESHAPE;
  if (p.dtype == CX_DT_F32) {
    if (p.K <= 0 || p.N <= 0) return CX_ESHAPE;
    if (!aligned16(p.x) || !aligned16(p.y) || !aligned16(p.w)) return CX_EALIGN;
    if ((long long)p.B * p.Ho * p.Wo >= (1ll << 31)) return CX_ESHAPE;
    if (p.prologue != CX_PRO_NONE && (!p.pa || !p.pb)) return CX_EINVAL;
    if (p.prologue == CX_PRO_AFFINE2 && (!p.x2 || !p.pc)) return CX_EINVAL;
    if (p.epilogue == CX_EPI_MASK && (!p.ex || !p.e_sc || !p.e_sh || !p.e_mu || !p.e_r || !p.e_scale || !p.stat_sum || !p.stat_sq))
      return CX_EINVAL;
    if ((p.stat_sum == nullptr) != (p.stat_sq == nullptr)) return CX_EINVAL;
    if (p.mode == CX_MODE_CONV) {
      if (p.kh <= 0 || p.kw <= 0 || p.stride <= 0 || p.pad < 0 || p.ldx < p.K || p.dil < 0) return CX_ESHAPE;
      const int keh = dil_extent(p.kh, p.dil), kew = dil_extent(p.kw, p.dil);
      if (p.tstride > 1) {
        const int fpad = keh - 1 - p.pad;
        if (p.stride != 1 || fpad < 0) return CX_ESHAPE;
        if (p.H != (p.Ho + 2 * fpad - keh) / p.tstride + 1 || p.W != (p.Wo + 2 * fpad - kew) / p.tstride + 1) return CX_ESHAPE;
      } else if (p.Ho != (p.H + 2 * p.pad - keh) / p.stride + 1 || p.Wo != (p.W + 2 * p.pad - kew) / p.stride + 1) {
        return CX_ESHAPE;
      }
    } else if (p.mode == CX_MODE_POOL2) {
      if ((p.H & 1) || (p.W & 1) || p.Ho != p.H / 2 || p.Wo != p.W / 2 || p.ldx < p.K) return CX_ESHAPE;
    }
    return cx_conv_gemm_f32(p, as_stream(stream));
  }
  if (p.dtype != CX_DT_BF16) return CX_EINVAL;
  if (p.K <= 0 || p.N <= 0 || (p.K % 8) || (p.N % 8)) return CX_ESHAPE;
  if (p.mode == CX_MODE_POOL2 && (p.K % 32)) return CX_ESHAPE;
  if (p.mode == CX_MODE_STEM ? (p.ldx != 4) : (p.ldx % 8 != 0)) return CX_EALIGN;
  if ((p.ldy % 8) || !aligned16(p.x) || !aligned16(p.y) || !aligned16(p.w)) return CX_EALIGN;
  if ((long long)p.B * p.Ho * p.Wo >= (1ll << 31)) return CX_ESHAPE;
  if (p.prologue != CX_PRO_NONE && (!p.pa || !p.pb)) return CX_EINVAL;
  if (p.prologue == CX_PRO_AFFINE2 && (!p.x2 || !p.pc || (p.ldx2 % 8) || !aligned16(p.x2))) return CX_EINVAL;
  if (p.epilogue == CX_EPI_MASK) {
    if (!p.ex || !p.e_sc || !p.e_sh || !p.e_mu || !p.e_r || !p.e_scale || !p.stat_sum || !p.stat_sq) return CX_EINVAL;
    if ((p.ldex % 8) || !aligned16(p.ex)) return CX_EALIGN;
  }
  if (p.epilogue == CX_EPI_JOIN) {
    if (!p.ex || !p.emask || !p.e_mu || !p.e_r || !p.stat_sum || !p.stat_sq || !p.accumulate) return CX_EINVAL;
    if ((p.ldex % 8) || !aligned16(p.ex)) return CX_EALIGN;
  }
  if ((p.stat_sum == nullptr) != (p.stat_sq == nullptr)) return CX_EINVAL;
  if (p.stat_replicas < 0 || (p.stat_replicas > 1 && p.stat_rstride < p.N)) return CX_EINVAL;
  hipStream_t st = as_stream(stream);
  if (p.prologue == CX_PRO_JOIN) {
    if (!p.x2 || !p.pc || !p.pro_out) return CX_EINVAL;
    if ((p.ldx2 % 8) || (p.ldpo % 8) || !aligned16(p.x2) || !aligned16(p.pro_out) || (((uintptr_t)p.po_lo) & 7) || (p.x3 && (((uintptr_t)p.x3) & 7)))
      return CX_EALIGN;
    if (p.mode != CX_MODE_CONV || p.epilogue != CX_EPI_STORE || p.kh != 1 || p.kw != 1 || p.stride != 1 || p.pad != 0 || p.tstride > 1 ||
        p.accumulate || (p.K % 64) || p.Ho != p.H || p.Wo != p.W || p.ldx < p.K || p.ldx2 < p.K || p.ldpo < p.K)
      return CX_EUNSUPPORTED;
    bool handled = false;
    const int rc = cx_try_conv_mm(p, st, &handled);
    return handled ? rc : CX_EUNSUPPORTED;
  }
  if (p.mode == CX_MODE_CONV) {
    if (p.kh <= 0 || p.kw <= 0 || p.stride <= 0 || p.pad < 0 || p.dil < 0) return CX_ESHAPE;
    if (p.tstride > 2) return CX_EUNSUPPORTED;
    const int keh = dil_extent(p.kh, p.dil), kew = dil_extent(p.kw, p.dil);
    if (p.tstride > 1) {
      const int fpad = keh - 1 - p.pad;
      if (p.stride != 1 || fpad < 0) return CX_ESHAPE;
      if (p.H != (p.Ho + 2 * fpad - keh) / p.tstride + 1 || p.W != (p.Wo + 2 * fpad - kew) / p.tstride + 1) return CX_ESHAPE;
    } else if (p.Ho != (p.H + 2 * p.pad - keh) / p.stride + 1 || p.Wo != (p.W + 2 * p.pad - kew) / p.stride + 1) {
      return CX_ESHAPE;
    }
    if (p.ldx < p.K) return CX_ESHAPE;
    if (p.dil <= 1) {
      bool handled = false;
      int rc = cx_try_pc_fwd(p, st, &handled);
      if (handled) return rc;
      rc = cx_try_ring_fwd(p, st, &handled);
      if (handled) return rc;
      rc = cx_try_strip_fwd(p, st, &handled);
      if (handled) return rc;
      rc = cx_try_ring_dgrad(p, st, &handled);
      if (handled) return rc;
      rc = cx_try_strip_dgrad(p, st, &handled);
      if (handled) return rc;
      rc = cx_try_pw_dgrad(p, st, &handled);
      if (handled) return rc;
      rc = cx_try_pw_fwd(p, st, &handled);
      if (handled) return rc;
      rc = cx_try_pw_fwdk(p, st, &handled);
      if (handled) return rc;
      rc = cx_try_pw_xs(p, st, &handled);
      if (handled) return rc;
      rc = cx_try_conv_mm(p, st, &handled);
      if (handled) return rc;
    }
    if (p.epilogue == CX_EPI_STORE) {
      if (p.prologue == CX_PRO_NONE) return launch_bn<CX_PRO_NONE, CX_MODE_CONV, CX_EPI_STORE>(p, st);
      if (p.prologue == CX_PRO_AFFINE_RELU) return launch_bn<CX_PRO_AFFINE_RELU, CX_MODE_CONV, CX_EPI_STORE>(p, st);
      if (p.prologue == CX_PRO_AFFINE2) return launch_bn<CX_PRO_AFFINE2, CX_MODE_CONV, CX_EPI_STORE>(p, st);
    } else if (p.epilogue == CX_EPI_MASK) {
      if (p.prologue == CX_PRO_AFFINE2) return launch_bn<CX_PRO_AFFINE2, CX_MODE_CONV, CX_EPI_MASK>(p, st);
      if (p.prologue == CX_PRO_NONE) return launch_bn<CX_PRO_NONE, CX_MODE_CONV, CX_EPI_MASK>(p, st);
    }
    return CX_EUNSUPPORTED;
  }
  if (p.mode == CX_MODE_POOL2) {
    if (p.prologue != CX_PRO_AFFINE_RELU || p.epilogue != CX_EPI_STORE) return CX_EUNSUPPORTED;
    if ((p.H & 1) || (p.W & 1) || p.Ho != p.H / 2 || p.Wo != p.W / 2 || p.ldx < p.K) return CX_ESHAPE;
    return launch_bn<CX_PRO_AFFINE_RELU, CX_MODE_POOL2, CX_EPI_STORE>(p, st);
  }
  if (p.mode == CX_MODE_STEM) {
    if (p.prologue != CX_PRO_NONE || p.epilogue != CX_EPI_STORE) return CX_EUNSUPPORTED;
    if (p.K != 32 || (p.W & 1) || p.Ho != (p.H + 6 - 7) / 2 + 1 || p.Wo != (p.W + 6 - 7) / 2 + 1) return CX_ESHAPE;
    {
      bool handled = false;
      const int rc = cx_try_stem_fwd(p, st, &handled);
      if (handled) return rc;
    }
    return launch_bn<CX_PRO_NONE, CX_MODE_STEM, CX_EPI_STORE>(p, st);
  }
  return CX_EUNSUPPORTED;
}
```

chexpert_amd/csrc/conv_mm.hip:

```cpp
#include <cstdlib>
#include <type_traits>
#include "common.h"

namespace {

typedef float f32x2 __attribute__((ext_vector_type(2)));
typedef uint32_t u32x4 __attribute__((ext_vector_type(4)));

#ifndef CX_MM_INTERLEAVE
#define CX_MM_INTERLEAVE 1
#endif
constexpr bool kInterleave = CX_MM_INTERLEAVE;
constexpr int BK = 64;
constexpr int PITCH = 144;

template <int WMW, int WNW>
struct MG {
  static constexpr int BM = 64 * WMW;
  static constexpr int BN = 64 * WNW;
  static constexpr int NW = WMW * WNW;
  static constexpr int NT = 64 * NW;
  static constexpr int RSTEP = NT / 8;
  static constexpr int NA = BM / RSTEP;
  static constexpr int NB = BN / RSTEP;
// ... 257 lines not shown
        acc[q >> 1][q & 1] = __builtin_amdgcn_mfma_f32_32x32x16_bf16(fa[cur][q >> 1], fb[cur][q & 1], acc[q >> 1][q & 1], 0, 0, 0);
        if (FENCE) __builtin_amdgcn_sched_barrier(0);
        const int slot = kk * 4 + q;
        if (ISSUE && q == 0 && kk < G::NA) issue_a(Rn, kk);
        if (STAGE) {
          if ((slot * G::NA) % 4 == 0) {
            const int u = slot * G::NA / 4;
            stage_unit(Rc, u >> 2, u & 3, o[u >> 2], As);
          }
          if (q == 2 && kk < G::NB) stage_w(kk, Bs);
        }
        if (ISSUE) {
          if (q == 3 && kk < G::NB) issue_w(kk);
          if (slot == 15) advance(Rn);
        }
        if (FENCE) __builtin_amdgcn_sched_barrier(0);
      }
    }
  };
  using T = std::true_type;
  using F = std::false_type;

  {
#pragma unroll
    for (int i = 0; i < G::NA; ++i) issue_a(set0, i);
#pragma unroll
    for (int i = 0; i < G::NB; ++i) issue_w(i);
    advance(set0);
    __syncthreads();
    load_coef(set0);
    u32x4 o[G::NA];
#pragma unroll
    for (int i = 0; i < G::NA; ++i)
#pragma unroll
      for (int j = 0; j < 4; ++j) stage_unit(set0, i, j, o[i], tiles);
#pragma unroll
    for (int i = 0; i < G::NB; ++i) stage_w(i, tiles + G::A_BYTES);
    if (nsteps > 1) {
#pragma unroll
      for (int i = 0; i < G::NA; ++i) issue_a(set1, i);
#pragma unroll
      for (int i = 0; i < G::NB; ++i) issue_w(i);
      advance(set1);
    }
    __syncthreads();
  }

  int s = 0;
  unsigned long long tacc[5] = {0, 0, 0, 0, 0}, tprev = 0;
  auto stamp = [&](int k) __attribute__((always_inline)) {
    if (DBG) {
      const unsigned long long t = __builtin_amdgcn_s_memtime();
      tacc[k] += t - tprev;
      tprev = t;
    }
  };
  if (DBG) tprev = __builtin_amdgcn_s_memtime();
  for (; s + 3 < nsteps; s += 2) {
    step(set0, set1, 0, 1, T{}, T{});
    stamp(0);
    __syncthreads();
    stamp(1);
    step(set1, set0, 1, 0, T{}, T{});
    stamp(0);
    __syncthreads();
    stamp(1);
  }
  if (DBG && (wave == 0 || wave == G::NW - 1) && lane == 0 && blockIdx.x < 2048) {
    unsigned long long* o = conv_mm_stamps + (blockIdx.x * 2 + (wave ? 1 : 0)) * 8;
    for (int k = 0; k < 4; ++k) o[k] = tacc[k];
    o[4] = s;
  }
  const int left = nsteps - s;
  if (left == 3) {
    step(set0, set1, 0, 1, T{}, T{});
    __syncthreads();
    step(set1, set0, 1, 0, F{}, T{});
    __syncthreads();
    step(set0, set1, 0, 1, F{}, F{});
  } else if (left == 2) {
    step(set0, set1, 0, 1, F{}, T{});
    __syncthreads();
    step(set1, set0, 1, 0, F{}, F{});
  } else {
    step(set0, set1, 0, 1, F{}, F{});
  }
  __syncthreads();

  constexpr int CPR = BN / 8;
  constexpr int RPP = G::NT / CPR;
  constexpr int NPASS = 64 / RPP;
  constexpr int NGRP = G::BM / 64;
  const int cq = tid % CPR, rr = tid / CPR;
  const bool nok = n0 + cq * 8 < p.N;
  const int nch = nok ? n0 + cq * 8 : 0;
  float* etile = reinterpret_cast<float*>(tiles);
  bf16* __restrict__ Y = reinterpret_cast<bf16*>(p.y);
  const bf16* __restrict__ EX = reinterpret_cast<const bf16*>(p.ex);
  float s1[8], s2[8];
#pragma unroll
  for (int j = 0; j < 8; ++j) s1[j] = s2[j] = 0.f;
  float esc[8], esh[8], emu[8], er[8], escale[8];
  if (EPI == CX_EPI_MASK) {
#pragma unroll
    for (int j = 0; j < 8; ++j) {
      esc[j] = p.e_sc[nch + j];
      esh[j] = p.e_sh[nch + j];
      emu[j] = p.e_mu[nch + j];
      er[j] = p.e_r[nch + j];
      escale[j] = p.e_scale[nch + j];
    }
  }
  if (EPI == CX_EPI_JOIN) {
#pragma unroll
    for (int j = 0; j < 8; ++j) {
      emu[j] = p.e_mu[nch + j];
      er[j] = p.e_r[nch + j];
    }
  }
  unsigned mkb[NGRP][NPASS];
  const bool want_stats = p.stat_sum != nullptr;

  U128 xv[NGRP][NPASS], old[NGRP][NPASS];
  int mo[NGRP][NPASS];
#pragma unroll
  for (int g = 0; g < NGRP; ++g)
#pragma unroll
    for (int pass = 0; pass < NPASS; ++pass) {
      const int m = mt * c.rpt + g * 64 + pass * RPP + rr;
      int mc = m < M ? m : M - 1;
      if (c.o_mul != 1) {
        const int hw = c.Hq * c.Wq;
        const int b = mc / hw;
        const int rem = mc - b * hw;
        const int oy = rem / c.Wq, ox = rem - oy * c.Wq;
        mc = (b * p.Ho + oy * c.o_mul + c.oy_add) * p.Wo + ox * c.o_mul + c.ox_add;
      }
      mo[g][pass] = mc;
      if (EPI == CX_EPI_MASK || EPI == CX_EPI_JOIN) xv[g][pass].u = *reinterpret_cast<const uint4*>(EX + (size_t)mc * p.ldex + nch);
      if (EPI == CX_EPI_JOIN) mkb[g][pass] = p.emask[cx_side_chunk((size_t)mc, nch >> 3, (size_t)p.B * p.Ho * p.Wo, p.N)];
      if (p.accumulate)
        old[g][pass].u = *reinterpret_cast<const uint4*>(Y + (size_t)mc * p.ldy + nch);
      else
        old[g][pass].u = make_uint4(0, 0, 0, 0);
    }

#pragma unroll
  for (int g = 0; g < NGRP; ++g) {
    if (wm == g) {
#pragma unroll
      for (int i = 0; i < 2; ++i)
#pragma unroll
        for (int j = 0; j < 2; ++j)
#pragma unroll
          for (int r = 0; r < 16; ++r) {
            const int row = i * 32 + (r & 3) + 8 * (r >> 2) + 4 * lh;
            const int col = (wn * 2 + j) * 32 + lrow;
            etile[row * G::EPITCH + col] = acc[i][j][r];
          }
    }
    __syncthreads();
#pragma unroll
    for (int pass = 0; pass < NPASS; ++pass) {
      const int row = pass * RPP + rr;
      const int m = mt * c.rpt + g * 64 + row;
      if (m < M && g * 64 + row < c.rpt && nok) {
        const float4 v0 = *reinterpret_cast<const float4*>(etile + row * G::EPITCH + cq * 8);
        const float4 v1 = *reinterpret_cast<const float4*>(etile + row * G::EPITCH + cq * 8 + 4);
        float v[8] = {v0.x, v0.y, v0.z, v0.w, v1.x, v1.y, v1.z, v1.w};
        U128 o;
        if (EPI == CX_EPI_STORE) {
          const uint32_t ow[4] = {old[g][pass].u.x, old[g][pass].u.y, old[g][pass].u.z, old[g][pass].u.w};
          float t[8];
#pragma unroll
          for (int j = 0; j < 4; ++j) { t[2 * j] = v[2 * j] + cx_bf_lo(ow[j]); t[2 * j + 1] = v[2 * j + 1] + cx_bf_hi(ow[j]); }
          o.u = cx_pack8_stats(t, true, true, s1, s2);
        } else if (EPI == CX_EPI_JOIN) {
          const uint32_t ow[4] = {old[g][pass].u.x, old[g][pass].u.y, old[g][pass].u.z, old[g][pass].u.w};
          const uint32_t xw[4] = {xv[g][pass].u.x, xv[g][pass].u.y, xv[g][pass].u.z, xv[g][pass].u.w};
          uint32_t w4[4];
#pragma unroll
          for (int j = 0; j < 4; ++j) {
            const uint32_t bits = mkb[g][pass] >> (2 * j);
            const uint32_t keep = ((bits & 1u) ? 0x0000ffffu : 0u) | ((bits & 2u) ? 0xffff0000u : 0u);
            w4[j] = cx_packbf(v[2 * j] + cx_bf_lo(ow[j]), v[2 * j + 1] + cx_bf_hi(ow[j])) & keep;
            const float dl = cx_bf_lo(w4[j]), du = cx_bf_hi(w4[j]);
            s1[2 * j] += dl;
            s1[2 * j + 1] += du;
            s2[2 * j] += dl * (cx_bf_lo(xw[j]) - emu[2 * j]) * er[2 * j];
            s2[2 * j + 1] += du * (cx_bf_hi(xw[j]) - emu[2 * j + 1]) * er[2 * j + 1];
          }
          o.u = make_uint4(w4[0], w4[1], w4[2], w4[3]);
        } else {
          const uint32_t ow[4] = {old[g][pass].u.x, old[g][pass].u.y, old[g][pass].u.z, old[g][pass].u.w};
          const uint32_t xw[4] = {xv[g][pass].u.x, xv[g][pass].u.y, xv[g][pass].u.z, xv[g][pass].u.w};
          uint32_t w4[4];
#pragma unroll
          for (int j = 0; j < 4; ++j) {
            const float xl = cx_bf_lo(xw[j]), xu = cx_bf_hi(xw[j]);
            const float dl = (fmaf(xl, esc[2 * j], esh[2 * j]) > 0.f) ? v[2 * j] : 0.f;
            const float du = (fmaf(xu, esc[2 * j + 1], esh[2 * j + 1]) > 0.f) ? v[2 * j + 1] : 0.f;
            s1[2 * j] += dl;
            s1[2 * j + 1] += du;
            s2[2 * j] += dl * (xl - emu[2 * j]) * er[2 * j];
            s2[2 * j + 1] += du * (xu - emu[2 * j + 1]) * er[2 * j + 1];
            w4[j] = cx_packbf(fmaf(escale[2 * j], dl, cx_bf_lo(ow[j])), fmaf(escale[2 * j + 1], du, cx_bf_hi(ow[j])));
          }
          o.u = make_uint4(w4[0], w4[1], w4[2], w4[3]);
        }
        *reinterpret_cast<uint4*>(Y + (size_t)mo[g][pass] * p.ldy + nch) = o.u;
      }
    }
    __syncthreads();
  }

  if (want_stats) {
#pragma unroll
    for (int j = 0; j < 8; ++j) {
#pragma unroll
      for (int d = CPR; d < 64; d <<= 1) {
        s1[j] += __shfl_xor(s1[j], d);
        s2[j] += __shfl_xor(s2[j], d);
      }
    }
    float* scratch = reinterpret_cast<float*>(tiles);
    wg_stat_begin<G::NW>(scratch, BN, tid, G::NT);
    if (lane < CPR) {
#pragma unroll
      for (int j = 0; j < 8; ++j) wg_stat_put(scratch, BN, wave, cq * 8 + j, s1[j], s2[j]);
    }
    wg_stat_end<G::NW>(scratch, BN, tid, G::NT, p.stat_sum, p.stat_sq, p.stat_det, p.stat_det ? c.row0 + mt : (int)blockIdx.x, p.stat_replicas,
                       p.stat_rstride, n0, p.N);
  }
}

#ifdef CX_DIAG
static int g_mm_dbg = 0;
extern "C" int dbg_conv_mm_stamps(unsigned long long* host, int n_words) {
  if (!host) {
    g_mm_dbg = n_words;
    return 0;
  }
  return (int)hipMemcpyFromSymbol(host, HIP_SYMBOL(conv_mm_stamps), (size_t)n_words * 8, 0, hipMemcpyDeviceToHost);
}
#endif

template <int WMW, int WNW, int PRO, int EPI>
int launch(const CxConv& p, const Cls& c, hipStream_t st) {
  using G = MG<WMW, WNW>;
  const int m_tiles = (c.Mq + c.rpt - 1) / c.rpt;
  const int n_tiles = (p.N + G::BN - 1) / G::BN;
  const size_t smem = (size_t)NCoef<PRO>::v * ((p.K + BK - 1) / BK * BK) * 4 + G::MAIN_BYTES;
  if (smem > 160 * 1024) return CX_ESHAPE;
  static bool attr_set = false;
  if (!attr_set) {
    (void)hipFuncSetAttribute(reinterpret_cast<const void*>(&conv_mm_kernel<WMW, WNW, PRO, EPI>), hipFuncAttributeMaxDynamicSharedMemorySize,
                              160 * 1024);
    attr_set = true;
  }
#ifdef CX_DIAG
  if (g_mm_dbg && (PRO == CX_PRO_AFFINE_RELU || PRO == CX_PRO_NONE) && EPI == CX_EPI_STORE) {
    constexpr int DP = PRO == CX_PRO_NONE ? CX_PRO_NONE : CX_PRO_AFFINE_RELU;
    (void)hipFuncSetAttribute(reinterpret_cast<const void*>(&conv_mm_kernel<WMW, WNW, DP, CX_EPI_STORE, true>),
                              hipFuncAttributeMaxDynamicSharedMemorySize, 160 * 1024);
    hipLaunchKernelGGL((conv_mm_kernel<WMW, WNW, DP, CX_EPI_STORE, true>), dim3(m_tiles * n_tiles), dim3(G::NT), smem, st, p, c, n_tiles);
    return launch_status();
  }
#endif
  CX_KTAG("conv_mm_kernel<%d, %d, %d, %d, false>%s", WMW, WNW, PRO, EPI, p.tstride > 1 ? " x parity classes" : "");
  hipLaunchKernelGGL((conv_mm_kernel<WMW, WNW, PRO, EPI>), dim3(m_tiles * n_tiles), dim3(G::NT), smem, st, p, c, n_tiles);
  return launch_status();
}

template <int PRO, int EPI>
int launch_form(const CxConv& p, const Cls& c, hipStream_t st, int form) {
  if (form == 3) return launch<2, 4, PRO, EPI>(p, c, st);
  return launch<2, 2, PRO, EPI>(p, c, st);
}

int launch_any(const CxConv& p, const Cls& c, hipStream_t st, int form) {
  if (p.prologue == CX_PRO_JOIN) return launch<2, 4, CX_PRO_JOIN, CX_EPI_STORE>(p, c, st);
  if (p.epilogue == CX_EPI_STORE) {
    if (p.prologue == CX_PRO_NONE) return launch_form<CX_PRO_NONE, CX_EPI_STORE>(p, c, st, form);
    if (p.prologue == CX_PRO_AFFINE_RELU) return launch_form<CX_PRO_AFFINE_RELU, CX_EPI_STORE>(p, c, st, form);
    return launch_form<CX_PRO_AFFINE2, CX_EPI_STORE>(p, c, st, form);
  }
  if (p.epilogue == CX_EPI_JOIN) return launch_form<CX_PRO_AFFINE2, CX_EPI_JOIN>(p, c, st, form);
  if (p.prologue == CX_PRO_AFFINE2) return launch_form<CX_PRO_AFFINE2, CX_EPI_MASK>(p, c, st, form);
  return launch_form<CX_PRO_NONE, CX_EPI_MASK>(p, c, st, form);
}

}


static int mm_min_steps() {
  static const int v = cx_diag_int("CX_MM_MIN_STEPS", 14);
  return v;
}

int cx_try_conv_mm(const CxConv& p, hipStream_t st, bool* handled) {
  *handled = false;
  static const int env_on0 = cx_diag_int("CX_MM", 1);
  static const int env_form0 = cx_diag_int("CX_MM_FORM", 0);
  const int g_mm_on = (p.kernel_hint & 0xff) - 1, g_mm_form = ((p.kernel_hint >> 8) & 0xff) - 1;
  const bool pjoin = p.prologue == CX_PRO_JOIN;
  const int env_on = (p.epilogue == CX_EPI_JOIN || pjoin) ? 1 : g_mm_on >= 0 ? g_mm_on : env_on0;
  const int env_form = g_mm_form >= 0 ? g_mm_form : env_form0;
  if (!env_on || p.mode != CX_MODE_CONV || p.tstride > 2 || (p.K % 8) || p.K < BK || (p.N % 8) || p.kh * p.kw > 32 || p.dtype != CX_DT_BF16) return 0;
  const bool ok_combo = (p.epilogue == CX_EPI_STORE && (p.prologue == CX_PRO_NONE || p.prologue == CX_PRO_AFFINE_RELU || p.prologue == CX_PRO_AFFINE2)) ||
                        (p.epilogue == CX_EPI_MASK && (p.prologue == CX_PRO_NONE || p.prologue == CX_PRO_AFFINE2)) ||
                        (p.epilogue == CX_EPI_JOIN && p.prologue == CX_PRO_AFFINE2 && p.tstride <= 1 && (p.N % 128) == 0) ||
                        (pjoin && p.epilogue == CX_EPI_STORE);
  if (!ok_combo) return 0;
  const bool join = p.epilogue == CX_EPI_JOIN || pjoin;
  if ((unsigned long long)p.B * p.H * p.W * (unsigned long long)(p.ldx > p.ldx2 ? p.ldx : p.ldx2) * 2 >= (1ull << 32)) return 0;
  if ((unsigned long long)p.kh * p.kw * p.N * p.K * 2 >= (1ull << 32)) return 0;
  if (pjoin && (unsigned long long)p.B * p.H * p.W * (unsigned long long)p.ldpo * 2 >= (1ull << 32)) return 0;
  const int ts = p.tstride > 1 ? 2 : 1;
  const int nsteps = (ts == 2 ? (p.kh * p.kw + 3) / 4 : p.kh * p.kw) * ((p.K + BK - 1) / BK);
  if (!env_form && !join && ts == 1 && nsteps <= 2) return 0;
  if (!env_form && !pjoin && (p.N % 128) && (nsteps < mm_min_steps() || p.N < 96)) return 0;
  const int pad1 = (p.N + 127) / 128 * 128, pad3 = (p.N + 255) / 256 * 256;
  int form = (pad3 == pad1 && nsteps > 4) ? 3 : 1;
  if (env_form) form = env_form == 3 ? 3 : 1;
  if (form == 3 && (size_t)NCoef<CX_PRO_AFFINE2>::v * ((p.K + BK - 1) / BK * BK) * 4 + MG<2, 4>::MAIN_BYTES > 160 * 1024) form = 1;
  const int bm = 128;

  if (ts == 1) {
    Cls c;
    c.nty = p.kh, c.ntx = p.kw;
    c.i_mul = p.stride, c.iy_add = -p.pad, c.ix_add = -p.pad;
    c.wy0 = c.wx0 = 0, c.wstep = 1;
    c.Hq = p.Ho, c.Wq = p.Wo, c.Mq = p.B * p.Ho * p.Wo;
    c.o_mul = 1, c.oy_add = c.ox_add = 0, c.row0 = 0;
    c.rpt = bm;
    if (pjoin && p.N <= 256) {
      const int rounds = ((c.Mq + bm - 1) / bm + 255) / 256;
      int r = (c.Mq + rounds * 256 - 1) / (rounds * 256);
      r = (r + 3) & ~3;
      c.rpt = r < 32 ? 32 : r > bm ? bm : r;
    }
    if (const int e = stat_rows_check(p, (c.Mq + c.rpt - 1) / c.rpt)) {
      *handled = true;
      return e;
    }
    *handled = true;
    return launch_any(p, c, st, form);
  }

  Cls cls[4];
  int n = 0, rows = 0;
  for (int py = 0; py < 2; ++py)
    for (int px = 0; px < 2; ++px) {
      const int d0y = (p.pad + py) & 1, d0x = (p.pad + px) & 1;
      Cls c;
      c.nty = d0y < p.kh ? (p.kh - d0y + 1) / 2 : 0;
      c.ntx = d0x < p.kw ? (p.kw - d0x + 1) / 2 : 0;
      c.Hq = (p.Ho - py + 1) / 2, c.Wq = (p.Wo - px + 1) / 2;
      c.Mq = p.B * c.Hq * c.Wq;
      if (c.Mq <= 0) continue;
      if (c.nty * c.ntx == 0) {
        if (!p.accumulate) return 0;
        continue;
      }
      c.i_mul = 1;
      c.iy_add = (py + d0y - p.pad) >> 1, c.ix_add = (px + d0x - p.pad) >> 1;
      c.wy0 = d0y, c.wx0 = d0x, c.wstep = 2;
      c.o_mul = 2, c.oy_add = py, c.ox_add = px;
      c.row0 = rows;
      c.rpt = bm;
      rows += (c.Mq + bm - 1) / bm;
      cls[n++] = c;
    }
  if (n == 0) return 0;
  *handled = true;
  if (const int e = stat_rows_check(p, rows)) return e;
  for (int i = 0; i < n; ++i)
    if (const int e = launch_any(p, cls[i], st, form)) return e;
  return 0;
}
```

chexpert_amd/ops.py:

```python
import os

import torch

from . import _lib as L
from ._lib import (EPI_JOIN, EPI_MASK, EPI_STORE, MODE_CONV, MODE_POOL2, MODE_STEM, PRO_AFFINE2, PRO_AFFINE_RELU, PRO_JOIN, PRO_NONE,
                   CxConv, CxWgrad, check, lib, ptr, require_cuda, stream_ptr)
import ctypes as C


def _nhwc(t):
    assert t.dtype in (torch.bfloat16, torch.float32) and t.dim() == 4, "expected a bf16 (or fp32-mode) NHWC tensor"
    B, H, W, Cc = t.shape
    sb, sh, sw, sc = t.stride()
    assert sc == 1 and sh == W * sw and sb == H * sh, "NHWC slice must be dense in (B,H,W) with a channel pitch"
    return B, H, W, Cc, sw


def _dense(t, like=None):
    B, H, W, Cc, ld = _nhwc(t)
    assert ld == Cc, "this kernel takes dense NHWC tensors (no channel pitch)"
    assert like is None or (t.shape == like.shape and t.dtype == like.dtype), "NHWC operands of one launch share shape and storage type"
    return B, H, W, Cc


def _f32(*tensors, n=0):
    for t in tensors:
        assert t is None or (t.dtype == torch.float32 and t.is_contiguous() and t.numel() >= n), "expected a contiguous fp32 tensor"


WGRAD_SCRATCH_DEFAULT = 0 if os.environ.get("CHEXPERT_DET_WGRAD", "1") == "0" else 16 << 20
WGRAD_SCRATCH_FLOATS = 0


def set_det_wgrad(on):
    global WGRAD_SCRATCH_FLOATS
    WGRAD_SCRATCH_FLOATS = WGRAD_SCRATCH_DEFAULT if on else 0


_wgrad_scratch = {}


def wgrad_scratch(device):
    if WGRAD_SCRATCH_FLOATS <= 0:
        return None
    key = (device.index, torch.cuda.current_stream(device).cuda_stream)
    t = _wgrad_scratch.get(key)
    if t is None or t.numel() != WGRAD_SCRATCH_FLOATS:
        t = _wgrad_scratch[key] = torch.empty(WGRAD_SCRATCH_FLOATS, dtype=torch.float32, device=device)
    return t


class _WgradArena:
    START = int(os.environ.get("CHEXPERT_WGRAD_ARENA_MB", "256")) * (1 << 20) // 4
    MIN_FREE = 16 << 20

    def __init__(self, device):
        self.device = device
        self.buf = torch.empty(self.START, dtype=torch.float32, device=device)
        self.off = 0
        self.need = 0
        self.tables = {}
        self.active = False


_arenas = {}


def _arena(device):
    a = _arenas.get(device.index)
    if a is None:
        a = _arenas[device.index] = _WgradArena(device)
    return a


def wgrad_defer_begin(device):
    if WGRAD_SCRATCH_FLOATS <= 0:
        return False
    a = _arena(device)
    if a.need > a.buf.numel():
        a.buf = None
        a.buf = torch.empty(int(a.need * 1.05) + a.MIN_FREE, dtype=torch.float32, device=device)
        a.tables.clear()
    a.off, a.need, a.active = 0, 0, True
    lib().cx_wgrad_defer(1)
    return True


def _wgrad_ws(device):
    a = _arenas.get(device.index)
    if a is not None and a.active:
        if a.buf.numel() - a.off >= a.MIN_FREE:
            return a.buf[a.off:], a, True
        lib().cx_wgrad_defer(0)
        return wgrad_scratch(device), a, False
    return wgrad_scratch(device), None, False


def _wgrad_used(a, deferred):
    if a is not None:
        n = (lib().cx_last_slab_floats() + 63) // 64 * 64
        a.need += n
        if deferred:
            a.off += n
        else:
            lib().cx_wgrad_defer(1)


def wgrad_defer_flush(device, keep=False):
    a = _arenas.get(device.index)
    if a is None or not a.active:
        return
    a.active = bool(keep)
    cap = 1024
    arr = (L.CxReduceDesc * cap)()
    blocks = C.c_int64(0)
    n = lib().cx_wgrad_defer_take(arr, cap, C.byref(blocks))
    if not keep:
        lib().cx_wgrad_defer(-1)
    if n < 0:
        raise RuntimeError("more than %d deferred weight-gradient sums" % cap)
    if n == 0:
        return
    key = bytes(memoryview(arr).cast("B")[:n * C.sizeof(L.CxReduceDesc)])
    t = a.tables.get(key)
    if t is None:
        if len(a.tables) > 256:
            a.tables.clear()
        t = a.tables[key] = torch.frombuffer(bytearray(key), dtype=torch.uint8).to(device)
    check(lib().cx_dw_reduce_table(ptr(t), n, blocks.value, stream_ptr()), "cx_dw_reduce_table")


def wgrad_defer_abort(device):
    a = _arenas.get(device.index)
    if a is not None and a.active:
        a.active = False
        lib().cx_wgrad_defer(-1)


def conv_gemm(x, w_packed, y, *, fused_dw=None, **kw):
    p = _conv_params(x, w_packed, y, **kw)
    if fused_dw is None:
        check(lib().cx_conv_gemm(C.byref(p), stream_ptr()), "cx_conv_gemm")
    else:
        require_cuda(fused_dw)
        assert x.dtype == torch.bfloat16, "the fused 1x1 input + weight gradient is a bf16 kernel"
        assert fused_dw.dtype == torch.float32
        ws, arena, dfr = _wgrad_ws(fused_dw.device)
        check(lib().cx_conv1x1_dgrad_wgrad_ld_ws(C.byref(p), ptr(fused_dw), _dw_pitch(fused_dw, p.N), ptr(ws),
                                                 0 if ws is None else ws.numel(), stream_ptr()), "cx_conv1x1_dgrad_wgrad_ld_ws")
        _wgrad_used(arena, dfr)
    return lib().cx_last_stat_rows() if p.stat_det else None


def _dw_pitch(dw, n):
    if dw.dim() == 1:
        assert dw.numel() == 128 * n and dw.is_contiguous()
        return n
    assert dw.shape[0] == 128 and dw.shape[1] == n and dw.numel() == 128 * n and dw.stride(1) == 1 and dw.stride(0) >= n, \
        (tuple(dw.shape), dw.stride())
    return dw.stride(0)


def conv1x1_bwd_pair(a, b, dw_a, dw_b):
    pa = _conv_params(a[0], a[1], a[2], **a[3])
    pb = _conv_params(b[0], b[1], b[2], **b[3])
    require_cuda(dw_a, dw_b)
    assert dw_a.dtype == torch.float32 and dw_b.dtype == torch.float32 and dw_b.is_contiguous()
    ws, arena, dfr = _wgrad_ws(dw_a.device)
    check(lib().cx_conv1x1_dgrad_wgrad_pair_ws(C.byref(pa), C.byref(pb), ptr(dw_a), _dw_pitch(dw_a, pa.N), ptr(dw_b), ptr(ws),
                                               0 if ws is None else ws.numel(), stream_ptr()), "cx_conv1x1_dgrad_wgrad_pair_ws")
    _wgrad_used(arena, dfr)
    return lib().cx_last_stat_rows() if pa.stat_det else None


def last_stat_rows():
    return lib().cx_last_stat_rows()


def last_kernel():
    return lib().cx_last_kernel().decode()


def last_pro_out():
    return bool(lib().cx_last_pro_out())


def kernel_hint(on=-1, form=-1):
    return (0 if on < 0 else on + 1) | ((0 if form < 0 else form + 1) << 8)


KERNEL_HINT = 0


def _conv_params(x, w_packed, y, *, N, kh=1, kw=1, stride=1, pad=0, mode=MODE_CONV, prologue=PRO_NONE, pa=None, pb=None,
                 pc=None, x2=None, epilogue=EPI_STORE, stat_sum=None, stat_sq=None, ex=None, e_sc=None, e_sh=None,
                 e_mu=None, e_r=None, e_scale=None, accumulate=False, K=None, tstride=1, stat_replicas=1, stat_rstride=0,
                 stat_det=False, pro_out=None, emask=None, x3=None, po_lo=None, po_mask=None, dil=1, hint=None):
    require_cuda(x, w_packed, y)
    p = CxConv()
    p.kernel_hint = KERNEL_HINT if hint is None else hint
    B, H, W, Cx, ldx = _nhwc(x)
    By, Ho, Wo, Cy, ldy = _nhwc(y)
    assert By == B and Cy == N
    p.x, p.w, p.y = ptr(x), ptr(w_packed), ptr(y)
    p.B, p.H, p.W, p.Ho, p.Wo = B, H, W, Ho, Wo
    p.K = (32 if mode == MODE_STEM else Cx) if K is None else K
    p.N = N
    p.ldx, p.ldy = ldx, ldy
    p.kh, p.kw, p.stride, p.pad = kh, kw, stride, pad
    p.prologue, p.mode, p.epilogue, p.accumulate = prologue, mode, epilogue, int(accumulate)
    p.dil = dil
    p.tstride = tstride
    p.pa, p.pb, p.pc = ptr(pa), ptr(pb), ptr(pc)
    if x2 is not None:
        assert x2.shape == x.shape
        p.x2, p.ldx2 = ptr(x2), _nhwc(x2)[4]
    p.stat_sum, p.stat_sq = ptr(stat_sum), ptr(stat_sq)
    p.stat_replicas, p.stat_rstride, p.stat_det = stat_replicas, stat_rstride, int(bool(stat_det))
    p.dtype = 1 if x.dtype == torch.float32 else 0
    for t_ in (w_packed, y, x2, ex):
        assert t_ is None or t_.dtype == x.dtype, "all tensors of one convolution share the storage type"
    if ex is not None:
        assert ex.shape == y.shape
        p.ex, p.ldex = ptr(ex), _nhwc(ex)[4]
    p.e_sc, p.e_sh, p.e_mu, p.e_r, p.e_scale = ptr(e_sc), ptr(e_sh), ptr(e_mu), ptr(e_r), ptr(e_scale)
    if pro_out is not None:
        require_cuda(pro_out)
        assert pro_out.dtype == x.dtype and tuple(pro_out.shape) == tuple(x.shape)
        p.pro_out, p.ldpo = ptr(pro_out), _nhwc(pro_out)[4]
    if emask is not None:
        require_cuda(emask)
        assert emask.dtype == torch.uint8 and emask.is_contiguous() and emask.numel() * 8 == B * Ho * Wo * N
        p.emask = ptr(emask)
    if prologue == PRO_JOIN:
        assert x2 is not None and pro_out is not None and x.is_contiguous() and x2.is_contiguous()
        for t_, n_ in ((x3, x.numel()), (po_lo, x.numel()), (po_mask, x.numel() // 8)):
            if t_ is not None:
                require_cuda(t_)
                assert t_.dtype in (torch.int8, torch.uint8) and t_.is_contiguous() and t_.numel() == n_
        p.x3, p.po_lo, p.po_mask = ptr(x3), ptr(po_lo), ptr(po_mask)
    p._keep = (x, w_packed, y, pa, pb, pc, x2, stat_sum, stat_sq, ex, e_sc, e_sh, e_mu, e_r, e_scale, pro_out, emask, x3, po_lo, po_mask)
    return p


def conv_wgrad(g, x, dw, *, kh=1, kw=1, stride=1, pad=0, mode=MODE_CONV, g_prologue=PRO_NONE, g2=None, ga=None, gb=None,
               gc=None, x_prologue=PRO_NONE, pa=None, pb=None, splits=0, K=None, dil=1, hint=None):
    require_cuda(g, x, dw)
    p = CxWgrad()
    p.kernel_hint = KERNEL_HINT if hint is None else hint
    p.dil = dil
    B, Ho, Wo, N, ldg = _nhwc(g)
    Bx, H, W, Cx, ldx = _nhwc(x)
    assert Bx == B and dw.dtype == torch.float32 and dw.is_contiguous()
    p.g, p.x, p.dw = ptr(g), ptr(x), ptr(dw)
    p.B, p.H, p.W, p.Ho, p.Wo = B, H, W, Ho, Wo
    p.K = (32 if mode == MODE_STEM else Cx) if K is None else K
    p.N = N
    p.ldg, p.ldx = ldg, ldx
    if g2 is not None:
        assert g2.shape == g.shape
        p.g2, p.ldg2 = ptr(g2), _nhwc(g2)[4]
    p.ga, p.gb, p.gc, p.pa, p.pb = ptr(ga), ptr(gb), ptr(gc), ptr(pa), ptr(pb)
    p.kh, p.kw, p.stride, p.pad = kh, kw, stride, pad
    p.g_prologue, p.x_prologue, p.mode, p.splits = g_prologue, x_prologue, mode, splits
    p.dtype = 1 if g.dtype == torch.float32 else 0
    assert x.dtype == g.dtype and (g2 is None or g2.dtype == g.dtype)
    ws, arena, dfr = _wgrad_ws(dw.device)
    if ws is not None:
        p.scratch, p.scratch_floats = ptr(ws), ws.numel()
    check(lib().cx_conv_wgrad(C.byref(p), stream_ptr()), "cx_conv_wgrad")
    _wgrad_used(arena, dfr)


def stem_input_grad(dz, y, pa, pb, pc, w, dx, *, stride, pad):
    require_cuda(dz, y, pa, pb, pc, w, dx)
    B, Ho, Wo, C0, ldz = _nhwc(dz)
    By, Hy, Wy, Cy, ldy = _nhwc(y)
    assert (By, Hy, Wy, Cy) == (B, Ho, Wo, C0) and y.dtype == dz.dtype
    assert w.dtype == torch.float32 and w.is_contiguous() and w.dim() == 4 and w.shape[0] == C0 and w.shape[2] == w.shape[3]
    assert dx.dtype == torch.float32 and dx.is_contiguous() and dx.dim() == 4 and dx.shape[:2] == (B, 3)
    for t in (pa, pb, pc):
        assert t.dtype == torch.float32 and t.is_contiguous() and t.numel() >= C0
    H, W = dx.shape[2], dx.shape[3]
    check(lib().cx_stem_input_grad(ptr(dz), ptr(y), ptr(pa), ptr(pb), ptr(pc), ptr(w), ptr(dx), ldz, ldy, w.shape[1], B, H, W, Ho, Wo, C0,
                                   w.shape[2], stride, pad, 1 if dz.dtype == torch.float32 else 0, stream_ptr()), "cx_stem_input_grad")
    return dx


def conv3x3_wgrad_batch(items):
    n = len(items)
    if n == 0:
        return True
    g0, x0 = items[0][0], items[0][1]
    if n > L.WGRAD_BATCH_MAX or g0.dtype != torch.bfloat16:
        return False
    p, bt = CxWgrad(), L.CxWgradBatch()
    B, H, W, N, ldg = _nhwc(g0)
    _, _, _, K, ldx = _nhwc(x0)
    p.B, p.H, p.W, p.Ho, p.Wo, p.K, p.N = B, H, W, H, W, K, N
    p.ldg, p.ldx = ldg, ldx
    p.kh, p.kw, p.stride, p.pad = 3, 3, 1, 1
    p.g_prologue, p.x_prologue, p.mode, p.dtype = PRO_NONE, PRO_AFFINE_RELU, MODE_CONV, 0
    for i, (g, x, pa, pb, dw) in enumerate(items):
        require_cuda(g, x, dw)
        assert _nhwc(g) == (B, H, W, N, ldg) and _nhwc(x) == (B, H, W, K, ldx) and g.dtype == x.dtype == torch.bfloat16
        assert dw.dtype == torch.float32 and dw.is_contiguous() and dw.numel() == N * K * 9
        bt.g[i], bt.x[i], bt.pa[i], bt.pb[i], bt.dw[i] = ptr(g), ptr(x), ptr(pa), ptr(pb), ptr(dw)
    bt.n = n
    ws, arena, dfr = _wgrad_ws(g0.device)
    if ws is None:
        return False
    p.scratch, p.scratch_floats = ptr(ws), ws.numel()
    rc = lib().cx_conv3x3_wgrad_batch(C.byref(p), C.byref(bt), stream_ptr())
    if rc == -4:
        if arena is not None and not dfr:
            lib().cx_wgrad_defer(1)
        return False
    check(rc, "cx_conv3x3_wgrad_batch")
    _wgrad_used(arena, dfr)
    return True


def pack_weights(w, transpose=False, stem=False, out=None):
    require_cuda(w)
    O, I, kh, kw = w.shape
    n = 7 * O * 32 if stem else kh * kw * O * I
    if out is None:
        out = torch.empty(n, dtype=torch.bfloat16, device=w.device)
    assert w.is_contiguous() and w.dtype == torch.float32 and out.numel() >= n
    check(lib().cx_pack_weights(ptr(w), ptr(out), O, I, kh, kw, int(transpose), int(stem), stream_ptr()), "cx_pack_weights")
    return out


def _fn(name, t):
    return getattr(lib(), name + "_f32" if t.dtype == torch.float32 else name)


def pack_weights_table(flat, packed, desc_dev, n_desc):
    if packed.dtype == torch.float32:
        check(lib().cx_pack_weights_table_f32(ptr(flat), ptr(packed), ptr(desc_dev), n_desc, stream_ptr()), "cx_pack_weights_table_f32")
    else:
        check(lib().cx_pack_weights_table(ptr(flat), ptr(packed), ptr(desc_dev), n_desc, stream_ptr()), "cx_pack_weights_table")


def u8_to_nhwc4(x, out=None, mean=0.5330, std=0.0349):
    require_cuda(x)
    assert x.dtype == torch.uint8 and x.is_contiguous()
    if x.dim() == 4:
        assert x.shape[1] == 1
        B, _, H, W = x.shape
    else:
        B, H, W = x.shape
    if out is None:
        out = torch.empty(B, H, W, 4, dtype=torch.bfloat16, device=x.device)
    check(_fn("cx_u8_to_nhwc4", out)(ptr(x), ptr(out), B * H * W, mean, std, stream_ptr()), "cx_u8_to_nhwc4")
    return out


def u8_jitter(x, brightness, contrast, order, out=None):
    require_cuda(x, brightness, contrast, order)
    assert x.dtype == torch.uint8 and x.is_contiguous() and order.dtype == torch.int32
    B = x.shape[0]
    HW = x.numel() // B
    if out is None:
        out = torch.empty_like(x)
    check(lib().cx_u8_jitter(ptr(x), ptr(out), B, HW, ptr(brightness), ptr(contrast), ptr(order), stream_ptr()), "cx_u8_jitter")
    return out


def u8_affine(x, mat, fill=0, out=None):
    require_cuda(x, mat, out)
    assert x.dtype == torch.uint8 and x.is_contiguous() and x.dim() in (3, 4) and (x.dim() == 3 or x.shape[1] == 1)
    B, H, W = x.shape[0], x.shape[-2], x.shape[-1]
    assert mat.dtype == torch.float32 and mat.is_contiguous() and tuple(mat.shape) == (B, 6)
    if out is None:
        out = torch.empty_like(x)
    assert out.dtype == torch.uint8 and out.shape == x.shape and out.is_contiguous()
    check(lib().cx_u8_affine(ptr(x), ptr(out), B, H, W, ptr(mat), int(fill), stream_ptr()), "cx_u8_affine")
    return out


def _plan_i32(v, shape, name):
    assert v.dtype == torch.int32 and v.is_contiguous() and tuple(v.shape) == shape, "%s: int32 %s expected" % (name, shape)


def u8_mix(x, perm, lam_q, box, fill=0, out=None):
    require_cuda(x, perm, lam_q, box, out)
    assert x.dtype == torch.uint8 and x.is_contiguous() and x.dim() in (3, 4) and (x.dim() == 3 or x.shape[1] == 1)
    B, H, W = x.shape[0], x.shape[-2], x.shape[-1]
    _plan_i32(perm, (B,), "perm"), _plan_i32(lam_q, (B,), "lam_q"), _plan_i32(box, (B, 4), "box")
    if out is None:
        out = torch.empty_like(x)
    assert out.dtype == torch.uint8 and out.shape == x.shape and out.is_contiguous()
    check(lib().cx_u8_mix(ptr(x), ptr(out), B, H, W, ptr(perm), ptr(lam_q), ptr(box), int(fill), stream_ptr()), "cx_u8_mix")
    return out


def target_mix(t, perm, tw_q, out=None):
    require_cuda(t, perm, tw_q, out)
    assert t.dtype == torch.float32 and t.is_contiguous() and t.dim() == 2
    B, n = t.shape
    _plan_i32(perm, (B,), "perm"), _plan_i32(tw_q, (B,), "tw_q")
    if out is None:
        out = torch.empty_like(t)
    assert out.dtype == torch.float32 and out.shape == t.shape and out.is_contiguous()
    check(lib().cx_target_mix(ptr(t), ptr(out), B, n, ptr(perm), ptr(tw_q), stream_ptr()), "cx_target_mix")
    return out


def _u8_images(x):
    assert x.dtype == torch.uint8 and x.is_contiguous() and x.dim() in (3, 4) and (x.dim() == 3 or x.shape[1] == 1)
    return x.shape[0], x.shape[-2], x.shape[-1]


def u8_clahe_lut(x, grid, clip_count):
    require_cuda(x)
    B, H, W = _u8_images(x)
    GY, GX = int(grid[0]), int(grid[1])
    lut = torch.empty(B, max(GY, 0), max(GX, 0), 256, dtype=torch.uint8, device=x.device)
    check(lib().cx_u8_clahe_lut(ptr(x), ptr(lut), B, H, W, GY, GX, int(clip_count), stream_ptr()), "cx_u8_clahe_lut")
    return lut


def u8_clahe_apply(x, lut, out=None):
    require_cuda(x, lut, out)
    B, H, W = _u8_images(x)
    assert lut.dtype == torch.uint8 and lut.is_contiguous() and lut.dim() == 4 and lut.shape[0] == B and lut.shape[3] == 256
    if out is None:
        out = torch.empty_like(x)
    assert out.dtype == torch.uint8 and out.shape == x.shape and out.is_contiguous()
    check(lib().cx_u8_clahe_apply(ptr(x), ptr(lut), ptr(out), B, H, W, lut.shape[1], lut.shape[2], stream_ptr()), "cx_u8_clahe_apply")
    return out


def u8_clahe(x, grid=(8, 8), clip_limit=2.0, out=None):
    from .augment import clahe_clip_count
    B, H, W = _u8_images(x)
    GY, GX = int(grid[0]), int(grid[1])
    if GY < 1 or GX < 1 or H % GY or W % GX:
        raise RuntimeError("u8_clahe: grid %s does not divide a %d x %d image (unsupported shape)" % ((GY, GX), H, W))
    return u8_clahe_apply(x, u8_clahe_lut(x, (GY, GX), clahe_clip_count(clip_limit, H // GY, W // GX)), out)


def nchw3_to_nhwc4(x, out=None):
    require_cuda(x)
    B, Cc, H, W = x.shape
    assert Cc == 3 and x.dtype == torch.float32 and x.is_contiguous()
    if out is None:
        out = torch.empty(B, H, W, 4, dtype=torch.bfloat16, device=x.device)
    check(_fn("cx_nchw3_to_nhwc4", out)(ptr(x), ptr(out), B, H, W, stream_ptr()), "cx_nchw3_to_nhwc4")
    return out


def u8_to_nhwc8(x, out, mean=0.5330, std=0.0349):
    require_cuda(x, out)
    B, H, W, Cc = _dense(out)
    assert x.dtype == torch.uint8 and x.is_contiguous() and tuple(x.shape) == (B, 1, H, W) and Cc == 8
    check(_fn("cx_u8_to_nhwc8", out)(ptr(x), ptr(out), B * H * W, mean, std, stream_ptr()), "cx_u8_to_nhwc8")


def nchw3_to_nhwc8(x, out):
    require_cuda(x, out)
    B, H, W, Cc = _dense(out)
    assert x.dtype == torch.float32 and x.is_contiguous() and tuple(x.shape) == (B, 3, H, W) and Cc == 8
    check(_fn("cx_nchw3_to_nhwc8", out)(ptr(x), ptr(out), B, H, W, stream_ptr()), "cx_nchw3_to_nhwc8")


def chan_map_table(real, padded, table, n_desc, direction, accumulate=0):
    require_cuda(real, padded, table)
    _f32(real, padded)
    assert table.dtype == torch.uint8 and table.is_contiguous() and table.numel() == n_desc * C.sizeof(L.CxChanMapDesc)
    check(lib().cx_chan_map_table(ptr(real), ptr(padded), ptr(table), n_desc, direction, accumulate, stream_ptr()), "cx_chan_map_table")


def bn_coef(s, q, count, gamma, beta, eps, momentum, rmean, rvar, scale, shift, mean, rstd, Cn=None, replicas=1, rstride=0):
    Cn = Cn if Cn is not None else s.numel()
    check(lib().cx_bn_coef(ptr(s), ptr(q), float(count), ptr(gamma), ptr(beta), eps, momentum, ptr(rmean), ptr(rvar),
                           ptr(scale), ptr(shift), ptr(mean), ptr(rstd), Cn, replicas, rstride, stream_ptr()), "cx_bn_coef")


def bn_coef_moments(mean, rstd, count, gamma, beta, eps, momentum, rmean, rvar, scale, shift, Cn, fresh=None):
    fs, fq, rows, rstride, c_lo, c_n = fresh if fresh is not None else (None, None, 0, 0, 0, 0)
    check(lib().cx_bn_coef_moments(ptr(mean), ptr(rstd), float(count), ptr(gamma), ptr(beta), eps, momentum, ptr(rmean), ptr(rvar),
                                   ptr(scale), ptr(shift), Cn, ptr(fs), ptr(fq), rows, rstride, c_lo, c_n, stream_ptr()),
          "cx_bn_coef_moments")


def bn_coef_eval(rmean, rvar, gamma, beta, eps, scale, shift, mean, rstd, Cn=None):
    Cn = Cn if Cn is not None else rmean.numel()
    check(lib().cx_bn_coef_eval(ptr(rmean), ptr(rvar), ptr(gamma), ptr(beta), eps, ptr(scale), ptr(shift), ptr(mean),
                                ptr(rstd), Cn, stream_ptr()), "cx_bn_coef_eval")


# ... 924 lines not shown
```

include/chexpert_hip.h:

```cpp
#ifndef CHEXPERT_HIP_H
#define CHEXPERT_HIP_H

#include <stddef.h>
#include <stdint.h>

#ifdef __cplusplus
extern "C" {
#endif

#define CX_ABI_VERSION 10

enum { CX_EINVAL = -1, CX_EALIGN = -2, CX_ESHAPE = -3, CX_EUNSUPPORTED = -4, CX_ESTATROWS = -5 };

enum { CX_DT_BF16 = 0, CX_DT_F32 = 1 };

enum {
  CX_PRO_NONE = 0,
  CX_PRO_AFFINE_RELU = 1,
  CX_PRO_AFFINE2 = 2,
  CX_PRO_JOIN = 3
};
enum {
  CX_MODE_CONV = 0,
  CX_MODE_POOL2 = 1,
  CX_MODE_STEM = 2
};
enum {
  CX_EPI_STORE = 0,
  CX_EPI_MASK = 1,
  CX_EPI_JOIN = 2
};

typedef struct CxConv {
  const void* x;
  const void* x2;
  const void* w;
  void* y;
  const float* pa; const float* pb; const float* pc;
  float* stat_sum; float* stat_sq;
  const void* ex;
  const float* e_sc; const float* e_sh; const float* e_mu; const float* e_r; const float* e_scale;
  int32_t B, H, W, Ho, Wo;
  int32_t K, N;
  int32_t ldx, ldx2, ldy, ldex;
  int32_t kh, kw, stride, pad;
  int32_t prologue, mode, epilogue, accumulate;
  int32_t tstride;
  int32_t stat_replicas;
  int32_t stat_rstride;
  int32_t stat_det;
  int32_t dtype;
  void* pro_out;
  int32_t ldpo;
  int32_t dil;
  const uint8_t* emask;
  const int8_t* x3;
  int8_t* po_lo;
  uint8_t* po_mask;
  int32_t kernel_hint;
  int32_t pad2_;
} CxConv;
#define CX_KERNEL_HINT(on, form) ((((on) < 0) ? 0 : (on) + 1) | ((((form) < 0) ? 0 : (form) + 1) << 8))

typedef struct CxWgrad {
  const void* g; const void* g2;
  const void* x;
  float* dw;
  const float* ga; const float* gb; const float* gc;
  const float* pa; const float* pb;
  int32_t B, H, W, Ho, Wo, K, N;
  int32_t ldg, ldg2, ldx;
  int32_t kh, kw, stride, pad;
  int32_t g_prologue, x_prologue, mode;
  int32_t splits;
  int32_t dtype;
  int32_t dil;
  float* scratch;
  int64_t scratch_floats;
  int32_t kernel_hint;
  int32_t pad_;
} CxWgrad;

#define CX_WGRAD_BATCH_MAX 24
typedef struct CxWgradBatch {
  const void* g[CX_WGRAD_BATCH_MAX];
  const void* x[CX_WGRAD_BATCH_MAX];
  const float* pa[CX_WGRAD_BATCH_MAX];
  const float* pb[CX_WGRAD_BATCH_MAX];
  float* dw[CX_WGRAD_BATCH_MAX];
  int32_t n, pad_;
} CxWgradBatch;
int cx_conv3x3_wgrad_batch(const CxWgrad* geo, const CxWgradBatch* items, void* stream);

typedef struct CxChanMapDesc {
  int64_t real_off, pad_off;
  int32_t O, taps, Ireal, Ipad;
  int32_t c0r, c0p, k, kp;
  int32_t split, shift;
} CxChanMapDesc;
int cx_chan_map_table(float* real_flat, float* padded_flat, const CxChanMapDesc* table_dev, int n_desc, int dir, int accumulate,
                      void* stream);

typedef struct CxReduceDesc {
  float* dw; const float* slab;
  int64_t total;
  int32_t splits, vec, first_block, pad_;
  int32_t cols, dw_ld;
  int64_t pad2_;
} CxReduceDesc;
int cx_wgrad_defer(int on);
int cx_wgrad_defer_take(CxReduceDesc* out_host, int capacity, int64_t* total_blocks);
int cx_last_slab_floats(void);
int cx_dw_reduce_table(const CxReduceDesc* table_dev, int n, int64_t total_blocks, void* stream);

int cx_abi_version(void);
int cx_last_pro_out(void);
const char* cx_error_string(int code);
const char* cx_last_kernel(void);
int cx_last_stat_rows(void);

int cx_conv_gemm(const CxConv* p, void* stream);
int cx_conv_wgrad(const CxWgrad* p, void* stream);
int cx_stem_input_grad(const void* dz, const void* y, const float* pa, const float* pb, const float* pc, const float* w, float* dx,
                       int ldz, int ldy, int wc, int B, int H, int W, int Ho, int Wo, int C0, int k, int stride, int pad, int dtype,
                       void* stream);

int cx_conv1x1_dgrad_wgrad(const CxConv* p, float* dw, void* stream);
int cx_conv1x1_dgrad_wgrad_ws(const CxConv* p, float* dw, float* scratch, int64_t scratch_floats, void* stream);
int cx_conv1x1_dgrad_wgrad_ld_ws(const CxConv* p, float* dw, int dw_ld, float* scratch, int64_t scratch_floats, void* stream);
int cx_conv1x1_dgrad_wgrad_pair_ws(const CxConv* a, const CxConv* b, float* dw_a, int dw_ld_a, float* dw_b, float* scratch,
                                   int64_t scratch_floats, void* stream);

int cx_pack_weights(const float* w_oihw, void* packed, int O, int I, int kh, int kw, int transpose, int stem,
                    void* stream);

typedef struct CxPackDesc {
  int64_t src_off, dst_off;
  int32_t O, I, kh, kw, transpose, stem;
} CxPackDesc;
int cx_pack_weights_table(const float* flat, void* packed, const CxPackDesc* table_dev, int n_desc, void* stream);

int cx_nchw3_to_nhwc4(const float* x, void* y, int B, int H, int W, void* stream);
int cx_u8_to_nhwc4(const uint8_t* x, void* y, size_t npix, float mean, float std, void* stream);

int cx_bn_coef(const float* sum, const float* sq, float count, const float* gamma, const float* beta, float eps,
               float momentum, float* running_mean, float* running_var, float* scale, float* shift, float* mean,
               float* rstd, int C, int replicas, int rstride, void* stream);
int cx_bn_coef_moments(float* mean, float* rstd, float count, const float* gamma, const float* beta, float eps, float momentum,
                       float* running_mean, float* running_var, float* scale, float* shift, int C, const float* sum, const float* sq,
                       int rows, int rstride, int c_lo, int c_n, void* stream);
int cx_bn_coef_eval(const float* running_mean, const float* running_var, const float* gamma, const float* beta,
                    float eps, float* scale, float* shift, float* mean, float* rstd, int C, void* stream);

int cx_bn_bwd_coef(const float* S1, const float* S2, float count, const float* gamma, const float* mean,
                   const float* rstd, float* dgamma, float* dbeta, float* A, float* Bc, float* pa, float* pb,
                   float* pc, int C, int replicas, int rstride,
                   float* qa, float* qb, float* qc, int q_lo, int q_n, void* stream);
int cx_bn_bwd_coef_eval(const float* S1, const float* S2, const float* mean, const float* rstd, const float* running_mean,
                        const float* running_var, const float* gamma, float eps, float* dgamma, float* dbeta, float* pa, float* pb,
                        float* pc, int C, int replicas, int rstride, float* qa, float* qb, float* qc, int q_lo, int q_n,
                        void* stream);
int cx_bn_bwd_slice_coef(const float* A, const float* Bc, const float* mean, const float* rstd, float* pa,
                         float* pb, float* pc, int C, void* stream);

int cx_bnrelu_maxpool_fwd(const void* x, const float* scale, const float* shift, void* y, uint8_t* argmax,
                          float* stat_sum, float* stat_sq, int B, int H, int W, int C, int ldy, int stat_rows, void* stream);
int cx_bnrelu_maxpool_bwd(const void* x, const float* scale, const float* shift, const float* mean,
                          const float* rstd, const uint8_t* argmax, const void* g, const void* gx, const float* ga,
                          const float* gb, const float* gc, void* dz, float* S1, float* S2, int B, int H, int W, int C,
                          int ldg, int ldgx, int stat_rows, void* stream);

int cx_head_fwd(const void* x, const float* scale, const float* shift, const float* w, const float* bias,
                float* pooled, float* logits, int B, int HW, int C, int ldx, int n_classes, void* stream);
int cx_bce_fwd_bwd(const float* logits, const float* target, float* loss, float* loss_elem, float* dlogits,
                   float grad_scale, int B, int n_classes, void* stream);
int cx_bce_masked_fwd_bwd(const float* logits, const float* target, const float* pos_weight, float* loss, float* loss_elem,
                          float* dlogits, float grad_scale, int B, int n_classes, void* stream);
int cx_aucm_fwd_bwd(const float* logits, const float* target, const float* prior, const float* aux, float margin, float* loss,
                    float* loss_class, float* dlogits, float* daux, float grad_scale, int B, int n_classes, void* stream);
int cx_aucm_aux_step(float* aux, const float* daux, const float* lr_aux_dev, int n_classes, void* stream);
int cx_asl_fwd_bwd(const float* logits, const float* target, const float* pos_weight, const float* focus, float* loss,
                   float* loss_elem, float* dlogits, float grad_scale, int B, int n_classes, void* stream);
int cx_mc3_fwd_bwd(const float* logits, const float* target, const float* class_weight, float* loss, float* loss_elem,
                   float* dlogits, float grad_scale, int B, int n, void* stream);
int cx_mc3_collapse(const float* logits, float* z, float* p_unc, int B, int n, void* stream);
int cx_softmax_ce_fwd_bwd(const float* logits, const int64_t* target, float* loss, float* loss_elem, float* dlogits,
                          float grad_scale, int B, int n_classes, void* stream);
int cx_head_bwd(const float* dlogits, const float* pooled, const float* w, float* dw, float* db,
                float* dpooled, int B, int C, int n_classes, void* stream);
int cx_gap_relu_bn_bwd(const float* dpooled, const void* x, const float* scale, const float* shift,
                       const float* mean, const float* rstd, const float* e_scale, void* g, float* S1, float* S2,
                       int B, int HW, int C, int ldx, int ldg, int stat_rows, void* stream);

int cx_unpool2_mask(const void* d, const void* x, const float* sc, const float* sh, const float* mean,
                    const float* rstd, const float* e_scale, void* g, float* S1, float* S2, int B, int H, int W,
                    int C, int ldd, int ldx, int ldg, int stat_rows, void* stream);

int cx_affine2_relu(const void* a, const void* b, const float* pa, const float* pb, const float* pc, void* out, size_t rows,
                    int C, void* stream);
int cx_dropout_slice_fwd(void* y, int ld, int64_t rows, int C, float p, const int64_t* seed, uint32_t uid, float* S1, float* S2,
                         int stat_rows, void* stream);
int cx_dropout_slice_fwd_f32(void* y, int ld, int64_t rows, int C, float p, const int64_t* seed, uint32_t uid, float* S1, float* S2,
                             int stat_rows, void* stream);
int cx_dropout_slice_bwd(void* g, int ldg, const void* x, int ldx, const float* qa, const float* qb, const float* qc, int64_t rows, int C,
                         float p, const int64_t* seed, uint32_t uid, void* stream);
int cx_dropout_slice_bwd_f32(void* g, int ldg, const void* x, int ldx, const float* qa, const float* qb, const float* qc, int64_t rows,
                             int C, float p, const int64_t* seed, uint32_t uid, void* stream);
int cx_relu_bwd_stats(const void* dout, const void* out, const void* a, const float* mu_a, const float* r_a, const void* b,
                      const float* mu_b, const float* r_b, void* dz, float* S1, float* S2a, float* S2b, size_t rows, int C,
                      int stat_rows, void* stream);
int cx_join_fwd(const void* a, const void* b, const int8_t* b_lo, const float* pa, const float* pb, const float* pc, void* out,
                int8_t* out_lo, uint8_t* mask, size_t rows, int C, void* stream);
int cx_affine2_relu_mask(const void* a, const void* b, const float* pa, const float* pb, const float* pc, void* out, uint8_t* mask,
                         size_t rows, int C, void* stream);
int cx_relu_bwd_stats_mask(const void* dout, const void* out, const uint8_t* mask, const void* a, const float* mu_a,
                           const float* r_a, const void* b, const float* mu_b, const float* r_b, void* dz, float* S1, float* S2a,
                           float* S2b, size_t rows, int C, int stat_rows, void* stream);
int cx_affine2_relu_mask_f32(const void* a, const void* b, const float* pa, const float* pb, const float* pc, void* out, uint8_t* mask,
                             size_t rows, int C, void* stream);
int cx_relu_bwd_stats_mask_f32(const void* dout, const void* out, const uint8_t* mask, const void* a, const float* mu_a, const float* r_a,
                               const void* b, const float* mu_b, const float* r_b, void* dz, float* S1, float* S2a, float* S2b,
                               size_t rows, int C, int stat_rows, void* stream);

int cx_affine2_inplace(void* dz, const void* x, const float* pa, const float* pb, const float* pc, size_t rows,
                       int C, void* stream);

int cx_adam_step(float* p, const float* g, float* m, float* v, size_t n, float lr, float beta1, float beta2,
                 float eps, float weight_decay, int step, float grad_scale, void* stream);
int cx_sgd_nesterov_step(float* p, const float* g, float* buf, size_t n, float lr, float momentum,
                         float weight_decay, int first_step, float grad_scale, void* stream);
int cx_rmsprop_step(float* p, const float* g, float* sq, float* buf, size_t n, float lr, float alpha, float eps,
                    float momentum, float weight_decay, float grad_scale, void* stream);

int cx_adam_step_dev(float* p, const float* g, float* m, float* v, size_t n, const float* hyper, float beta1, float beta2,
                     float eps, float weight_decay, float grad_scale, void* stream);
int cx_sgd_nesterov_step_dev(float* p, const float* g, float* buf, size_t n, const float* hyper, float momentum,
                             float weight_decay, float grad_scale, void* stream);
int cx_rmsprop_step_dev(float* p, const float* g, float* sq, float* buf, size_t n, const float* hyper, float alpha, float eps,
                        float momentum, float weight_decay, float grad_scale, void* stream);
int cx_optim_tick(float* hyper, void* stream);

int cx_grad_norm_partials(size_t n);
int cx_grad_norm(const float* g, size_t n, float grad_scale, float max_norm, int skip_nonfinite, float* workspace,
                 size_t workspace_floats, float* clip, void* stream);
int cx_adam_step_ex(float* p, const float* g, float* m, float* v, size_t n, float lr, float beta1, float beta2, float eps,
                    float weight_decay, int step, float grad_scale, const float* clip, float* ema, float ema_decay, int ema_warmup,
                    int skip_nonfinite, void* stream);
int cx_sgd_nesterov_step_ex(float* p, const float* g, float* buf, size_t n, float lr, float momentum, float weight_decay,
                            int first_step, int step, float grad_scale, const float* clip, float* ema, float ema_decay,
                            int ema_warmup, int skip_nonfinite, void* stream);
int cx_rmsprop_step_ex(float* p, const float* g, float* sq, float* buf, size_t n, float lr, float alpha, float eps, float momentum,
                       float weight_decay, int step, float grad_scale, const float* clip, float* ema, float ema_decay,
                       int ema_warmup, int skip_nonfinite, void* stream);
int cx_adam_step_dev_ex(float* p, const float* g, float* m, float* v, size_t n, const float* hyper, float beta1, float beta2,
                        float eps, float weight_decay, float grad_scale, const float* clip, float* ema, float ema_decay,
                        int ema_warmup, int skip_nonfinite, void* stream);
int cx_sgd_nesterov_step_dev_ex(float* p, const float* g, float* buf, size_t n, const float* hyper, float momentum,
                                float weight_decay, float grad_scale, const float* clip, float* ema, float ema_decay, int ema_warmup,
                                int skip_nonfinite, void* stream);
int cx_rmsprop_step_dev_ex(float* p, const float* g, float* sq, float* buf, size_t n, const float* hyper, float alpha, float eps,
                           float momentum, float weight_decay, float grad_scale, const float* clip, float* ema, float ema_decay,
                           int ema_warmup, int skip_nonfinite, void* stream);

int cx_optim_item_vec4(void);
int cx_grad_norm_items(const float* g, size_t n, const uint32_t* items, int n_items, const float* groups, int n_groups,
                       float grad_scale, float max_norm, int skip_nonfinite, float* partials, float* group_sq, float* group_norm,
                       float* clip, void* stream);
int cx_adam_step_items(float* p, const float* g, float* m, float* v, size_t n, const uint32_t* items, int n_items, const float* groups,
                       int n_groups, int decoupled, const float* hyper, float lr, int step, float beta1, float beta2, float eps,
                       float grad_scale, const float* clip, float* ema, float ema_decay, int ema_warmup, int skip_nonfinite,
                       void* stream);
int cx_sgd_nesterov_step_items(float* p, const float* g, float* buf, size_t n, const uint32_t* items, int n_items, const float* groups,
                               int n_groups, int decoupled, const float* hyper, float lr, int step, float momentum, float grad_scale,
                               const float* clip, float* ema, float ema_decay, int ema_warmup, int skip_nonfinite, void* stream);
int cx_rmsprop_step_items(float* p, const float* g, float* sq, float* buf, size_t n, const uint32_t* items, int n_items,
                          const float* groups, int n_groups, int decoupled, const float* hyper, float lr, int step, float alpha, float eps,
                          float momentum, float grad_scale, const float* clip, float* ema, float ema_decay, int ema_warmup,
                          int skip_nonfinite, void* stream);

int cx_aa_attention_fwd(const void* qkv, const float* key_rel_h, const float* key_rel_w, float* o, float* lse, int B, int H, int W,
                        int nh, int dk, int dv, int ldq, void* stream);
int cx_aa_attention_weights(const void* qkv, const float* key_rel_h, const float* key_rel_w, const float* lse, float* weights, int B,
                            int H, int W, int nh, int dk, int dv, int ldq, void* stream);
int cx_aa_attention_bwd(const void* qkv, const float* key_rel_h, const float* key_rel_w, const float* o, const float* d_o,
                        const float* lse, float* dqkv, float* d_rel_h, float* d_rel_w, int B, int H, int W, int nh, int dk, int dv,
                        int ldq, float* scratch, int64_t scratch_floats, void* stream);
int cx_aa_outproj_fwd(const float* o, const float* w, void* y, int ldy, float* stat_sum, float* stat_sq, size_t npix, int dv,
                      int stat_rows, int stat_rstride, void* stream);
int cx_aa_outproj_bwd(const void* g, int ldg, const void* gx, int ldgx, const float* ga, const float* gb, const float* gc,
                      const float* o, const float* w, float* d_o, float* dw, size_t npix, int dv, float* scratch, int64_t scratch_floats,
                      void* stream);
int cx_rows_reduce(float* dst, const float* rows, int n_rows, int C, int rstride, int accumulate, void* stream);
int cx_stats_bc(const void* x, float* sum, float* sq, int B, int HW, int C, int ldx, void* stream);
int cx_affine_relu_bc(const void* x, const float* sc, const float* sh, void* y, int B, int HW, int C, int ldx, void* stream);
int cx_in_relu_bwd(const void* da, const void* x, const float* sc, const float* sh, float* S1, float* S2, void* gout, int B, int HW,
                   int C, int ldx, int ldg, void* stream);
int cx_aa_attention_fwd_f32(const void* qkv, const float* rel_h, const float* rel_w, float* o, float* lse, int B, int H, int W, int nh,
                        int dk, int dv, int ldq, void* stream);
int cx_aa_attention_weights_f32(const void* qkv, const float* rel_h, const float* rel_w, const float* lse, float* weights, int B, int H,
                            int W, int nh, int dk, int dv, int ldq, void* stream);
int cx_aa_attention_bwd_f32(const void* qkv, const float* rel_h, const float* rel_w, const float* o, const float* d_o, const float* lse,
                        float* dqkv, float* d_rel_h, float* d_rel_w, int B, int H, int W, int nh, int dk, int dv, int ldq,
                        float* scratch, int64_t scratch_floats, void* stream);
int cx_stats_bc_f32(const void* x, float* sum, float* sq, int B, int HW, int C, int ldx, void* stream);
int cx_affine_relu_bc_f32(const void* x, const float* sc, const float* sh, void* y, int B, int HW, int C, int ldx, void* stream);
int cx_aa_outproj_fwd_f32(const float* o, const float* w, void* y, int ldy, float* stat_sum, float* stat_sq, size_t npix, int dv,
                      int stat_rows, int stat_rstride, void* stream);
int cx_aa_outproj_bwd_f32(const void* g, int ldg, const void* gx, int ldgx, const float* ga, const float* gb, const float* gc,
                      const float* o, const float* w, float* d_o, float* dw, size_t npix, int dv, float* scratch, int64_t scratch_floats,
                      void* stream);
int cx_in_relu_bwd_f32(const void* da, const void* x, const float* sc, const float* sh, float* S1, float* S2, void* gout, int B, int HW,
                   int C, int ldx, int ldg, void* stream);
int cx_f32_to_bf16(const float* x, void* y, size_t n, void* stream);

int cx_nchw3_to_nhwc8(const float* x, void* y, int B, int H, int W, void* stream);
int cx_u8_to_nhwc8(const uint8_t* x, void* y, size_t npix, float mean, float std, void* stream);
int cx_dwconv_fwd(const void* x, const float* w, const float* sc, const float* sh, void* y, float* stat_sum, float* stat_sq, int B, int H,
                  int W, int C, int k, int stride, int pad, int stat_rows, void* stream);
int cx_dwconv_dgrad(const void* g, const void* g2, const float* ga, const float* gb, const float* gc, const float* w, const void* x,
                    const float* sc, const float* sh, const float* mean, const float* rstd, void* dz, float* S1, float* S2, int B, int H,
                    int W, int C, int k, int stride, int pad, int accumulate, int stat_rows, void* stream);
int cx_dwconv_wgrad(const void* g, const void* g2, const float* ga, const float* gb, const float* gc, const void* x, const float* sc,
                    const float* sh, float* dw, int B, int H, int W, int C, int k, int stride, int pad, float* scratch,
                    int64_t scratch_floats, void* stream);
int cx_gap_affine_act(const void* x, const float* sc, const float* sh, float* pooled, int B, int HW, int C, int act, float* scratch,
                      int64_t scratch_floats, void* stream);
int cx_se_fwd(const float* pooled, const float* w1, const float* b1, const float* w2, const float* b2, float* h1, float* s, int B, int C,
              int R, void* stream);
int cx_gap_se_fwd(const void* x, const float* sc, const float* sh, float* pooled, const float* w1, const float* b1, const float* w2,
                  const float* b2, float* h1, float* s, int B, int HW, int C, int R, int act, float* scratch, int64_t scratch_floats,
                  void* stream);
int cx_gap_se_fwd_f32(const void* x, const float* sc, const float* sh, float* pooled, const float* w1, const float* b1, const float* w2,
                      const float* b2, float* h1, float* s, int B, int HW, int C, int R, int act, float* scratch, int64_t scratch_floats,
                      void* stream);
int cx_se_bwd(const float* ds, const float* s, const float* h1, const float* pooled, const float* w1, const float* w2, float* dw1,
              float* db1, float* dw2, float* db2, float* dpooled, int B, int C, int R, float* scratch, int64_t scratch_floats,
              void* stream);
int cx_se_bwd_fused(const void* du, const void* x, const float* sc, const float* sh, float* ds, const float* s, const float* h1,
                    const float* pooled, const float* w1, const float* w2, float* dw1, float* db1, float* dw2, float* db2, float* dpooled,
                    int B, int HW, int C, int R, float* rows_scratch, int64_t rows_floats, float* scratch, int64_t scratch_floats,
                    void* stream);
int cx_se_bwd_fused_f32(const void* du, const void* x, const float* sc, const float* sh, float* ds, const float* s, const float* h1,
                        const float* pooled, const float* w1, const float* w2, float* dw1, float* db1, float* dw2, float* db2, float* dpooled,
                        int B, int HW, int C, int R, float* rows_scratch, int64_t rows_floats, float* scratch, int64_t scratch_floats,
                        void* stream);
int cx_scale_act_bc(const void* x, const float* sc, const float* sh, const float* s, void* u, int B, int HW, int C, void* stream);
int cx_se_bwd_reduce(const void* du, const void* x, const float* sc, const float* sh, float* ds, int B, int HW, int C, float* scratch,
                     int64_t scratch_floats, void* stream);
int cx_se_act_bwd(const void* du, const void* x, const float* sc, const float* sh, const float* mean, const float* rstd, const float* s,
                  const float* dpooled, void* dz, float* S1, float* S2, int B, int HW, int C, int stat_rows, void* stream);
int cx_bn_lin_bwd_stats(const void* g, const void* y, const float* mean, const float* rstd, float* S1, float* S2, size_t rows, int C,
                        int stat_rows, void* stream);
int cx_affine2_out(const void* a, const void* b, const float* pa, const float* pb, const float* pc, const float* sample_scale,
                   size_t rows_per_sample, void* out, size_t rows, int C, void* stream);
int cx_scale_rows(const void* g, const float* sample_scale, size_t rows_per_sample, void* out, size_t rows, int C, void* stream);
int cx_nchw3_to_nhwc8_f32(const float* x, void* y, int B, int H, int W, void* stream);
int cx_u8_to_nhwc8_f32(const uint8_t* x, void* y, size_t npix, float mean, float std, void* stream);
int cx_dwconv_fwd_f32(const void* x, const float* w, const float* sc, const float* sh, void* y, float* stat_sum, float* stat_sq, int B, int H,
                  int W, int C, int k, int stride, int pad, int stat_rows, void* stream);
int cx_dwconv_dgrad_f32(const void* g, const void* g2, const float* ga, const float* gb, const float* gc, const float* w, const void* x,
                    const float* sc, const float* sh, const float* mean, const float* rstd, void* dz, float* S1, float* S2, int B, int H,
                    int W, int C, int k, int stride, int pad, int accumulate, int stat_rows, void* stream);
int cx_dwconv_wgrad_f32(const void* g, const void* g2, const float* ga, const float* gb, const float* gc, const void* x, const float* sc,
                    const float* sh, float* dw, int B, int H, int W, int C, int k, int stride, int pad, float* scratch,
                    int64_t scratch_floats, void* stream);
int cx_gap_affine_act_f32(const void* x, const float* sc, const float* sh, float* pooled, int B, int HW, int C, int act, float* scratch,
                      int64_t scratch_floats, void* stream);
int cx_scale_act_bc_f32(const void* x, const float* sc, const float* sh, const float* s, void* u, int B, int HW, int C, void* stream);
int cx_bn_lin_bwd_stats_f32(const void* g, const void* y, const float* mean, const float* rstd, float* S1, float* S2, size_t rows, int C,
                        int stat_rows, void* stream);
int cx_se_bwd_reduce_f32(const void* du, const void* x, const float* sc, const float* sh, float* ds, int B, int HW, int C, float* scratch,
                     int64_t scratch_floats, void* stream);
int cx_se_act_bwd_f32(const void* du, const void* x, const float* sc, const float* sh, const float* mean, const float* rstd, const float* s,
                  const float* dpooled, void* dz, float* S1, float* S2, int B, int HW, int C, int stat_rows, void* stream);
int cx_affine2_out_f32(const void* a, const void* b, const float* pa, const float* pb, const float* pc, const float* sample_scale,
                   size_t rows_per_sample, void* out, size_t rows, int C, void* stream);
int cx_scale_rows_f32(const void* g, const float* sample_scale, size_t rows_per_sample, void* out, size_t rows, int C, void* stream);
int cx_dropout_mask(float* out, size_t n, float keep_prob, unsigned long long seed, void* stream);
int cx_dropout_mask_dev(float* out, size_t n, float keep_prob, unsigned long long base, const unsigned long long* step, void* stream);
int cx_counter_add(unsigned long long* counter, unsigned long long inc, void* stream);
int cx_mul_f32(const float* a, const float* b, float* out, size_t n, void* stream);
int cx_linear_fwd(const float* x, const float* w, const float* bias, float* y, int B, int C, int N, void* stream);

int cx_gradcam_map(const void* x, const float* scale, const float* shift, const float* w, float* cam, int B, int HW, int C,
                   int ldx, int inner_relu, void* stream);
int cx_cam_norm_upsample(const float* cam, float* out, int B, int h, int w, int H, int W, void* stream);

enum { CX_CAM_ACT_NONE = 0, CX_CAM_ACT_RELU = 1, CX_CAM_ACT_SWISH = 2 };
int cx_class_cam(const void* x, const float* scale, const float* shift, const float* w, const int* cls, float* cam, int B, int HW, int C,
                 int ldx, int n_classes, int ldw, int K, int act, int relu, void* stream);
int cx_class_cam_f32(const void* x, const float* scale, const float* shift, const float* w, const int* cls, float* cam, int B, int HW,
                     int C, int ldx, int n_classes, int ldw, int K, int act, int relu, void* stream);


int cx_u8_jitter(const uint8_t* x, uint8_t* y, int B, int HW, const float* brightness, const float* contrast, const int* order,
                 void* stream);
int cx_u8_affine(const uint8_t* x, uint8_t* y, int B, int H, int W, const float* mat , int fill, void* stream);
int cx_u8_mix(const uint8_t* x, uint8_t* y, int B, int H, int W, const int* perm , const int* lam_q ,
              const int* box , int fill, void* stream);
int cx_target_mix(const float* t, float* out, int B, int n, const int* perm , const int* tw_q ,
                  void* stream);
int cx_u8_clahe_lut(const uint8_t* x, uint8_t* lut, int B, int H, int W, int GY, int GX, int clip_count, void* stream);
int cx_u8_clahe_apply(const uint8_t* x, const uint8_t* lut, uint8_t* y, int B, int H, int W, int GY, int GX, void* stream);

enum { CX_BOOT_TILE = 8192, CX_BOOT_MAX_TILES = 8, CX_BOOT_MAX_UNITS = 1 << 24 };
int cx_boot_counts(uint32_t* counts, int ld, int U, int first, int n_rep, uint64_t seed, void* stream);
int cx_boot_auc(const uint32_t* counts, int ld, int n_rep, const int32_t* order , const int64_t* offs ,
                const int32_t* len , int C, uint64_t* num2, uint32_t* wpos, uint32_t* wneg, int U, void* stream);

enum { CX_BOOT_MAX_POINTS = 8, CX_BOOT_SENS = 0, CX_BOOT_SPEC = 1 };
int cx_boot_sweep(const uint32_t* counts, int ld, int n_rep, const int32_t* order , const int64_t* offs ,
                  const int32_t* len , int C, const int32_t* pt_type , const int32_t* pt_ppm ,
                  int P, uint64_t* apnum, uint32_t* wpos, uint32_t* wneg, uint32_t* pts, int U, void* stream);

enum { CX_CALIB_TEMPERATURE = 0, CX_CALIB_PLATT = 1, CX_CALIB_MAX_ITER = 1000, CX_CALIB_MAX_BINS = 64 };
int cx_calib_fit(const float* logits, const float* targets, int C, int N, int method, int smooth, double g_tol, int max_iter, double* out,
                 void* stream);
int cx_boot_calib(const uint32_t* counts, int ld, int n_rep, const int32_t* order , const uint32_t* conf ,
                  const int64_t* offs , const int32_t* len , int C, int M, uint32_t* wsum, uint32_t* wpos,
                  uint64_t* csum, uint64_t* bnum, int U, void* stream);

enum { CX_DELONG_MAX_ROWS = 128, CX_DELONG_WG_ENTRIES = 16384, CX_DELONG_TILE = 32 };
int cx_delong_place(const int32_t* order , const int64_t* offs , const int32_t* len , int C,
                    int U, int64_t* z, int ldz, void* stream);
int cx_delong_gram(const int64_t* z, int ldz, int Q, int U, int64_t* g, void* stream);

enum { CX_SAL_NONE = 0, CX_SAL_SUM = 1, CX_SAL_ABS = 2, CX_SAL_MAX = 3, CX_SAL_PARTIALS = 128 };
int cx_sal_points(const float* x, const float* base, float base0, float base1, float base2, const int32_t* img, const float* alpha,
                  const float* sigma, uint64_t seed, uint64_t first_row, float* out, int B, int R, int H, int W, void* stream);
int cx_sal_accumulate(const float* g, const int32_t* slot, const float* w, float* acc, int R, int P, int H, int W, int square,
                      int accumulate, void* stream);
int cx_sal_finish(const float* acc, const float* x, const float* base, float base0, float base1, float base2, const int32_t* img_of,
                  float* out, double* total, double* partial, int P, int B, int H, int W, int times_input, int mode, void* stream);

enum { CX_POOL_AVG = 0, CX_POOL_MAX = 1, CX_POOL_LSE = 2, CX_POOL_GEM = 3 };
enum { CX_POOL_ACT_RELU = 1, CX_POOL_ACT_SWISH = 2 };
int cx_pool_head_fwd(const void* x, const float* sc, const float* sh, float* pooled, float* aux, const float* param, int B, int HW,
                     int C, int ldx, int act, int kind, void* stream);
int cx_pool_head_bwd(const float* dpooled, const float* pooled, const float* aux, const float* param, const void* x, const float* sc,
                     const float* sh, const float* mean, const float* rstd, const float* e_scale, void* g, float* S1, float* S2, int B,
                     int HW, int C, int ldx, int ldg, int act, int kind, int stat_rows, void* stream);
int cx_pool_p_grad(const float* dpooled, const float* pooled, const float* aux, const float* p, float* dp, int B, int C, void* stream);
int cx_pool_head_fwd_f32(const void* x, const float* sc, const float* sh, float* pooled, float* aux, const float* param, int B, int HW,
                         int C, int ldx, int act, int kind, void* stream);
int cx_pool_head_bwd_f32(const float* dpooled, const float* pooled, const float* aux, const float* param, const void* x,
                         const float* sc, const float* sh, const float* mean, const float* rstd, const float* e_scale, void* g,
                         float* S1, float* S2, int B, int HW, int C, int ldx, int ldg, int act, int kind, int stat_rows, void* stream);

int cx_pack_weights_table_f32(const float* flat, float* packed, const CxPackDesc* table_dev, int n_desc, void* stream);
int cx_nchw3_to_nhwc4_f32(const float* x, float* y, int B, int H, int W, void* stream);
int cx_u8_to_nhwc4_f32(const uint8_t* x, float* y, size_t npix, float mean, float std, void* stream);
int cx_bnrelu_maxpool_fwd_f32(const void* x, const float* scale, const float* shift, void* y, uint8_t* argmax,
                          float* stat_sum, float* stat_sq, int B, int H, int W, int C, int ldy, int stat_rows, void* stream);
// ... 24 lines not shown
```

Baseline: 9766 images/sec.

## Add persistent weight-resident 1x1 fwd kernel and smaller pixel tiles for fwdk

Adds a persistent 1x1 forward conv kernel that keeps the whole 128-output weight matrix resident in LDS and streams 32-pixel activation tiles through it. It is used by default for large-M layers with K between 288 and 480, which the fwdk path previously did not take. The fwdk/fwdp kernels are also templated on the pixel tile size (128/64/32), with a heuristic that picks 64-row tiles when M is mid-sized so the grid fills the CUs better. Hint-form decoding is adjusted so the new parent hints do not collide with the mm/xs kernel selectors. The persistent kernel runs at one 512-thread workgroup per CU with a large LDS footprint, which reduces occupancy and latency hiding.

```diff
diff --git a/chexpert_amd/_lib.py b/chexpert_amd/_lib.py
--- a/chexpert_amd/_lib.py
+++ b/chexpert_amd/_lib.py
@@ -84,6 +84,7 @@
     "cx_u8_to_nhwc4": [_vp, _vp, _sz, _f, _f, _vp],
     "cx_bn_coef": [_vp, _vp, _f, _vp, _vp, _f, _f, _vp, _vp, _vp, _vp, _vp, _vp, _i, _i, _i, _vp],
     "cx_bn_coef_moments": [_vp, _vp, _f, _vp, _vp, _f, _f, _vp, _vp, _vp, _vp, _i, _vp, _vp, _i, _i, _i, _i, _vp],
+    "cx_pw_fwdk_tile": [C.c_int64, _i],
     "cx_last_stat_rows": [],
     "cx_bnrelu_maxpool_fwd_f32": [_vp, _vp, _vp, _vp, _vp, _vp, _vp, _i, _i, _i, _i, _i, _i, _vp],
     "cx_bnrelu_maxpool_bwd_f32": [_vp, _vp, _vp, _vp, _vp, _vp, _vp, _vp, _vp, _vp, _vp, _vp, _vp, _vp, _i, _i, _i, _i, _i, _i, _i, _vp],
diff --git a/chexpert_amd/csrc/conv1x1_fwdk.hip b/chexpert_amd/csrc/conv1x1_fwdk.hip
--- a/chexpert_amd/csrc/conv1x1_fwdk.hip
+++ b/chexpert_amd/csrc/conv1x1_fwdk.hip
@@ -3,17 +3,29 @@
 
 namespace {
 
-constexpr int BM = 128, BN = 128;
-constexpr int WAVES_N = 2, TM = 2, TN = 2;
+constexpr int BN = 128;
 constexpr int EPITCH = BN + 4;
-
-template <int BK, int PRO>
+constexpr int CX_CUS = 256, CX_SLOTS = 2 * CX_CUS;
+
+template <int BM>
+struct Tile {
+  static_assert(BM == 128 || BM == 64 || BM == 32, "pixel tile");
+  static constexpr int WAVES_M = BM >= 64 ? 2 : 1, WAVES_N = 4 / WAVES_M;
+  static constexpr int TM = BM / (32 * WAVES_M), TN = BN / (32 * WAVES_N);
+  static constexpr int NH = BM == 128 ? 2 : 1;
+  static constexpr int EH = BM / NH;
+};
+
+template <int BK, int PRO, int BM>
 __global__ __launch_bounds__(256, 2) void pw_fwdk_kernel(const CxConv p, const int M) {
   constexpr int PITCH = BK * 2 + 16;
   constexpr int CPR = BK / 8;
   constexpr int RPP = 256 / CPR;
   constexpr int NL = 128 / RPP;
+  constexpr int NLA = BM / RPP;
   constexpr int A_BYTES = BM * PITCH;
+  typedef Tile<BM> T;
+  constexpr int WAVES_N = T::WAVES_N, TM = T::TM, TN = T::TN;
   extern __shared__ __attribute__((aligned(16))) char smem[];
   float* coef = reinterpret_cast<float*>(smem);
   char* At = smem + 2 * p.K * 4;
@@ -30,7 +42,7 @@
 
   const int q = tid % CPR, r0 = tid / CPR;
   const int nsteps = (p.K + BK - 1) / BK;
-  uint4 ra[NL], rw[NL];
+  uint4 ra[NLA], rw[NL];
   bool kok = true;
   auto issue_loads = [&](int s) __attribute__((always_inline)) {
     const int c = s * BK + q * 8;
@@ -39,9 +51,11 @@
 #pragma unroll
     for (int i = 0; i < NL; ++i) {
       const int row = r0 + RPP * i;
-      const int m = mt * BM + row;
-      const int mc = m < M ? m : M - 1;
-      ra[i] = *reinterpret_cast<const uint4*>(X + (size_t)mc * p.ldx + cc);
+      if (i < NLA) {
+        const int m = mt * BM + row;
+        const int mc = m < M ? m : M - 1;
+        ra[i] = *reinterpret_cast<const uint4*>(X + (size_t)mc * p.ldx + cc);
+      }
       rw[i] = *reinterpret_cast<const uint4*>(Wp + (size_t)row * p.K + cc);
     }
   };
@@ -50,15 +64,17 @@
 #pragma unroll
     for (int i = 0; i < NL; ++i) {
       const int row = r0 + RPP * i;
-      U128 o;
-      if (!kok || mt * BM + row >= M) {
-        o.u = make_uint4(0, 0, 0, 0);
-      } else if (PRO == CX_PRO_NONE) {
-        o.u = ra[i];
-      } else {
-        o.u = cx_affine_relu8(ra[i], coef + c0, coef + p.K + c0);
-      }
-      *reinterpret_cast<uint4*>(At + row * PITCH + q * 16) = o.u;
+      if (i < NLA) {
+        U128 o;
+        if (!kok || mt * BM + row >= M) {
+          o.u = make_uint4(0, 0, 0, 0);
+        } else if (PRO == CX_PRO_NONE) {
+          o.u = ra[i];
+        } else {
+          o.u = cx_affine_relu8(ra[i], coef + c0, coef + p.K + c0);
+        }
+        *reinterpret_cast<uint4*>(At + row * PITCH + q * 16) = o.u;
+      }
       *reinterpret_cast<uint4*>(Bt + row * PITCH + q * 16) = kok ? rw[i] : make_uint4(0, 0, 0, 0);
     }
   };
@@ -93,7 +109,7 @@
     __syncthreads();
   }
 
-  constexpr int ECPR = BN / 8, ERPP = 256 / ECPR, NPASS = 64 / ERPP;
+  constexpr int ECPR = BN / 8, ERPP = 256 / ECPR, NPASS = T::EH / ERPP;
   const int cq = tid % ECPR, rr = tid / ECPR;
   float* etile = reinterpret_cast<float*>(At);
   float s1[8], s2[8];
@@ -101,15 +117,15 @@
   for (int j = 0; j < 8; ++j) s1[j] = s2[j] = 0.f;
   const bool want_stats = p.stat_sum != nullptr;
 #pragma unroll
-  for (int half = 0; half < 2; ++half) {
-    if (wm == half) {
+  for (int half = 0; half < T::NH; ++half) {
+    if (T::NH == 1 || wm == half) {
 #pragma unroll
       for (int i = 0; i < TM; ++i)
 #pragma unroll
         for (int j = 0; j < TN; ++j)
 #pragma unroll
           for (int r = 0; r < 16; ++r) {
-            const int row = i * 32 + (r & 3) + 8 * (r >> 2) + 4 * lh;
+            const int row = (T::NH == 1 ? wm * TM + i : i) * 32 + (r & 3) + 8 * (r >> 2) + 4 * lh;
             const int col = (wn * TN + j) * 32 + lrow;
             etile[row * EPITCH + col] = acc[i][j][r];
           }
@@ -118,7 +134,7 @@
 #pragma unroll
     for (int pass = 0; pass < NPASS; ++pass) {
       const int row = pass * ERPP + rr;
-      const int m = mt * BM + half * 64 + row;
+      const int m = mt * BM + half * T::EH + row;
       if (m < M) {
         const float4 v0 = *reinterpret_cast<const float4*>(etile + row * EPITCH + cq * 8);
         const float4 v1 = *reinterpret_cast<const float4*>(etile + row * EPITCH + cq * 8 + 4);
@@ -161,14 +177,17 @@
   }
 }
 
-template <int PRO, int D>
+template <int PRO, int D, int BM>
 __global__ __launch_bounds__(256, 2) void pw_fwdp_kernel(const CxConv p, const int M) {
   constexpr int BK = 64;
   constexpr int PITCH = BK * 2 + 16;
   constexpr int CPR = BK / 8;
   constexpr int RPP = 256 / CPR;
   constexpr int NL = 128 / RPP;
+  constexpr int NLA = BM / RPP;
   constexpr int A_BYTES = BM * PITCH;
+  typedef Tile<BM> T;
+  constexpr int WAVES_N = T::WAVES_N, TM = T::TM, TN = T::TN;
   extern __shared__ __attribute__((aligned(16))) char smem[];
   float* coef = reinterpret_cast<float*>(smem);
   char* At = smem + 2 * p.K * 4;
@@ -183,41 +202,43 @@
     for (int i = tid; i < p.K; i += 256) { coef[i] = p.pa[i]; coef[p.K + i] = p.pb[i]; }
   const int q = tid % CPR, r0 = tid / CPR;
   const int nsteps = (p.K + BK - 1) / BK;
-  const bf16* xr[NL];
+  const bf16* xr[NLA];
   const bf16* wr[NL];
 #pragma unroll
   for (int i = 0; i < NL; ++i) {
     const int row = r0 + RPP * i;
     const int m = mt * BM + row;
-    xr[i] = X + (size_t)(m < M ? m : M - 1) * p.ldx + q * 8;
+    if (i < NLA) xr[i] = X + (size_t)(m < M ? m : M - 1) * p.ldx + q * 8;
     wr[i] = Wp + (size_t)row * p.K + q * 8;
   }
-  uint4 ra[D][NL], rw[D][NL];
-  auto issue = [&](uint4 (&a)[NL], uint4 (&w)[NL], int s) __attribute__((always_inline)) {
+  uint4 ra[D][NLA], rw[D][NL];
+  auto issue = [&](uint4 (&a)[NLA], uint4 (&w)[NL], int s) __attribute__((always_inline)) {
     const int sc = s < nsteps ? s : nsteps - 1;
     int c = sc * BK;
     if (c + q * 8 >= p.K) c = p.K - BK;
 #pragma unroll
     for (int i = 0; i < NL; ++i) {
-      a[i] = *reinterpret_cast<const uint4*>(xr[i] + c);
+      if (i < NLA) a[i] = *reinterpret_cast<const uint4*>(xr[i] + c);
       w[i] = *reinterpret_cast<const uint4*>(wr[i] + c);
     }
   };
-  auto stage = [&](const uint4 (&a)[NL], const uint4 (&w)[NL], int s) __attribute__((always_inline)) {
+  auto stage = [&](const uint4 (&a)[NLA], const uint4 (&w)[NL], int s) __attribute__((always_inline)) {
     const int c0 = s * BK + q * 8;
     const bool kok = c0 < p.K;
 #pragma unroll
     for (int i = 0; i < NL; ++i) {
       const int row = r0 + RPP * i;
-      U128 o;
-      if (!kok || mt * BM + row >= M) {
-        o.u = make_uint4(0, 0, 0, 0);
-      } else if (PRO == CX_PRO_NONE) {
-        o.u = a[i];
-      } else {
-        o.u = cx_affine_relu8(a[i], coef + c0, coef + p.K + c0);
-      }
-      *reinterpret_cast<uint4*>(At + row * PITCH + q * 16) = o.u;
+      if (i < NLA) {
+        U128 o;
+        if (!kok || mt * BM + row >= M) {
+          o.u = make_uint4(0, 0, 0, 0);
+        } else if (PRO == CX_PRO_NONE) {
+          o.u = a[i];
+        } else {
+          o.u = cx_affine_relu8(a[i], coef + c0, coef + p.K + c0);
+        }
+        *reinterpret_cast<uint4*>(At + row * PITCH + q * 16) = o.u;
+      }
       *reinterpret_cast<uint4*>(Bt + row * PITCH + q * 16) = kok ? w[i] : make_uint4(0, 0, 0, 0);
     }
   };
@@ -256,7 +277,7 @@
       }
     }
   }
-  constexpr int ECPR = BN / 8, ERPP = 256 / ECPR, NPASS = 64 / ERPP;
+  constexpr int ECPR = BN / 8, ERPP = 256 / ECPR, NPASS = T::EH / ERPP;
   const int cq = tid % ECPR, rr = tid / ECPR;
   float* etile = reinterpret_cast<float*>(At);
   float s1[8], s2[8];
@@ -264,15 +285,15 @@
   for (int j = 0; j < 8; ++j) s1[j] = s2[j] = 0.f;
   const bool want_stats = p.stat_sum != nullptr;
 #pragma unroll
-  for (int half = 0; half < 2; ++half) {
-    if (wm == half) {
+  for (int half = 0; half < T::NH; ++half) {
+    if (T::NH == 1 || wm == half) {
 #pragma unroll
       for (int i = 0; i < TM; ++i)
 #pragma unroll
         for (int j = 0; j < TN; ++j)
 #pragma unroll
           for (int r = 0; r < 16; ++r) {
-            const int row = i * 32 + (r & 3) + 8 * (r >> 2) + 4 * lh;
+            const int row = (T::NH == 1 ? wm * TM + i : i) * 32 + (r & 3) + 8 * (r >> 2) + 4 * lh;
             const int col = (wn * TN + j) * 32 + lrow;
             etile[row * EPITCH + col] = acc[i][j][r];
           }
@@ -281,7 +302,7 @@
 #pragma unroll
     for (int pass = 0; pass < NPASS; ++pass) {
       const int row = pass * ERPP + rr;
-      const int m = mt * BM + half * 64 + row;
+      const int m = mt * BM + half * T::EH + row;
       if (m < M) {
         const float4 v0 = *reinterpret_cast<const float4*>(etile + row * EPITCH + cq * 8);
         const float4 v1 = *reinterpret_cast<const float4*>(etile + row * EPITCH + cq * 8 + 4);
@@ -324,44 +345,63 @@
   }
 }
 
-template <int PRO, int D>
+template <int BM>
+constexpr size_t tile_smem(int bk) {
+  const size_t stage = (size_t)(BM + BN) * (bk * 2 + 16);
+  const size_t epi = (size_t)Tile<BM>::EH * EPITCH * 4;
+  return (stage > epi ? stage : epi) + 2 * BN * 4;
+}
+static_assert(2 * 1280 * 4 + tile_smem<128>(128) <= 80 * 1024 && 2 * 1280 * 4 + tile_smem<128>(64) <= 80 * 1024, "LDS");
+static_assert(tile_smem<64>(64) <= tile_smem<128>(64) && tile_smem<32>(64) <= tile_smem<64>(64), "LDS");
+static_assert(tile_smem<64>(128) <= tile_smem<128>(128) && tile_smem<32>(128) <= tile_smem<64>(128), "LDS");
+static_assert(tile_smem<32>(64) >= (size_t)4 * 2 * BN * 4, "LDS");
+
+template <int PRO, int D, int BM>
 int launch_fwdp(const CxConv& p, hipStream_t st) {
   const long long M = (long long)p.B * p.Ho * p.Wo;
   const int m_tiles = (int)((M + BM - 1) / BM);
-  const size_t stage = (size_t)2 * BM * (64 * 2 + 16);
-  const size_t epi = (size_t)64 * EPITCH * 4;
-  const size_t smem = (size_t)2 * p.K * 4 + (stage > epi ? stage : epi) + 2 * BN * 4;
+  const size_t smem = (size_t)2 * p.K * 4 + tile_smem<BM>(64);
   static bool attr = false;
   if (!attr) {
-    (void)hipFuncSetAttribute(reinterpret_cast<const void*>(&pw_fwdp_kernel<PRO, D>), hipFuncAttributeMaxDynamicSharedMemorySize, 80 * 1024);
+    (void)hipFuncSetAttribute(reinterpret_cast<const void*>(&pw_fwdp_kernel<PRO, D, BM>), hipFuncAttributeMaxDynamicSharedMemorySize, 80 * 1024);
     attr = true;
   }
   if (smem > 80 * 1024) return CX_ESHAPE;
   if (const int e = stat_rows_check(p, m_tiles)) return e;
-  CX_KTAG("pw_fwdp_kernel<%d, %d>", PRO, D);
-  hipLaunchKernelGGL((pw_fwdp_kernel<PRO, D>), dim3(m_tiles), dim3(256), smem, st, p, (int)M);
+  CX_KTAG("pw_fwdp_kernel<%d, %d, %d>", PRO, D, BM);
+  hipLaunchKernelGGL((pw_fwdp_kernel<PRO, D, BM>), dim3(m_tiles), dim3(256), smem, st, p, (int)M);
   return launch_status();
 }
 
-template <int BK, int PRO>
+template <int BK, int PRO, int BM>
 int launch_fwdk(const CxConv& p, hipStream_t st) {
   const long long M = (long long)p.B * p.Ho * p.Wo;
   const int m_tiles = (int)((M + BM - 1) / BM);
-  const size_t stage = (size_t)2 * BM * (BK * 2 + 16);
-  const size_t epi = (size_t)64 * EPITCH * 4;
-  const size_t smem = (size_t)2 * p.K * 4 + (stage > epi ? stage : epi) + 2 * BN * 4;
+  const size_t smem = (size_t)2 * p.K * 4 + tile_smem<BM>(BK);
   static bool attr = false;
   if (!attr) {
-    (void)hipFuncSetAttribute(reinterpret_cast<const void*>(&pw_fwdk_kernel<BK, PRO>), hipFuncAttributeMaxDynamicSharedMemorySize, 80 * 1024);
+    (void)hipFuncSetAttribute(reinterpret_cast<const void*>(&pw_fwdk_kernel<BK, PRO, BM>), hipFuncAttributeMaxDynamicSharedMemorySize, 80 * 1024);
     attr = true;
   }
   if (smem > 80 * 1024) return CX_ESHAPE;
   if (const int e = stat_rows_check(p, m_tiles)) return e;
-  CX_KTAG("pw_fwdk_kernel<%d, %d>", BK, PRO);
-  hipLaunchKernelGGL((pw_fwdk_kernel<BK, PRO>), dim3(m_tiles), dim3(256), smem, st, p, (int)M);
+  CX_KTAG("pw_fwdk_kernel<%d, %d, %d>", BK, PRO, BM);
+  hipLaunchKernelGGL((pw_fwdk_kernel<BK, PRO, BM>), dim3(m_tiles), dim3(256), smem, st, p, (int)M);
   return launch_status();
 }
 
+template <int BM>
+int launch_tile(const CxConv& p, hipStream_t st, bool piped) {
+  const bool ar = p.prologue == CX_PRO_AFFINE_RELU;
+  if (piped) return ar ? launch_fwdp<CX_PRO_AFFINE_RELU, 2, BM>(p, st) : launch_fwdp<CX_PRO_NONE, 2, BM>(p, st);
+  return ar ? launch_fwdk<128, CX_PRO_AFFINE_RELU, BM>(p, st) : launch_fwdk<128, CX_PRO_NONE, BM>(p, st);
+}
+
+}
+
+extern "C" int cx_pw_fwdk_tile(int64_t M, int K) {
+  (void)K;
+  return (M > 16384 && (M + 63) / 64 <= CX_SLOTS) ? 64 : 128;
 }
 
 int cx_try_pw_fwdk(const CxConv& p, hipStream_t st, bool* handled) {
@@ -369,14 +409,15 @@
   if (p.mode != CX_MODE_CONV || p.kh != 1 || p.kw != 1 || p.stride != 1 || p.pad != 0 || p.tstride > 1) return 0;
   if (p.epilogue != CX_EPI_STORE || p.accumulate || p.N != 128 || p.K <= 256 || p.K > 1280) return 0;
   if (p.prologue != CX_PRO_AFFINE_RELU && p.prologue != CX_PRO_NONE) return 0;
-  if ((long long)p.B * p.Ho * p.Wo > 200000) return 0;
+  const long long M = (long long)p.B * p.Ho * p.Wo;
+  if (M > 200000) return 0;
   *handled = true;
-  static const int pipe = cx_diag_int("CX_FWDK_PIPE", 2);
-  if (pipe == 2 && p.K % 32 == 0 && p.K >= 512)
-    return p.prologue == CX_PRO_AFFINE_RELU ? launch_fwdp<CX_PRO_AFFINE_RELU, 2>(p, st) : launch_fwdp<CX_PRO_NONE, 2>(p, st);
-  if (pipe == 3 && p.K % 32 == 0 && p.K >= 192)
-    return p.prologue == CX_PRO_AFFINE_RELU ? launch_fwdp<CX_PRO_AFFINE_RELU, 3>(p, st) : launch_fwdp<CX_PRO_NONE, 3>(p, st);
-  if (pipe == 4 && p.K % 32 == 0 && p.K >= 256)
-    return p.prologue == CX_PRO_AFFINE_RELU ? launch_fwdp<CX_PRO_AFFINE_RELU, 4>(p, st) : launch_fwdp<CX_PRO_NONE, 4>(p, st);
-  return p.prologue == CX_PRO_AFFINE_RELU ? launch_fwdk<128, CX_PRO_AFFINE_RELU>(p, st) : launch_fwdk<128, CX_PRO_NONE>(p, st);
-}
+  const bool piped = p.K % 32 == 0 && p.K >= 512;
+  const int form = ((p.kernel_hint >> 8) & 0xff) - 1;
+  int tile = cx_pw_fwdk_tile(M, p.K);
+  if (form == CX_HINT_PARENT) tile = 128;
+  if (form >= CX_HINT_PARENT + 1 && form <= CX_HINT_PARENT + 3) tile = 128 >> (form - CX_HINT_PARENT - 1);
+  if (tile == 64) return launch_tile<64>(p, st, piped);
+  if (tile == 32) return launch_tile<32>(p, st, piped);
+  return launch_tile<128>(p, st, piped);
+}
diff --git a/chexpert_amd/csrc/conv1x1_fwdr.hip b/chexpert_amd/csrc/conv1x1_fwdr.hip
--- /dev/null
+++ b/chexpert_amd/csrc/conv1x1_fwdr.hip
@@ -0,0 +1,221 @@
+#include <type_traits>
+#include "common.h"
+
+namespace {
+
+constexpr int NO = 128;
+constexpr int BM = 32;
+constexpr int NT = 512;
+constexpr int OP = NO * 2 + 16;
+constexpr int LDS_MAX = 160 * 1024;
+typedef uint32_t fr_u32x4 __attribute__((ext_vector_type(4)));
+
+template <int KT>
+struct Lds {
+  static constexpr int K = KT * 32, xp = K * 2 + 16;
+  static constexpr int coef = 2 * K * 4, w = NO * xp, x = BM * xp, o = BM * OP;
+  static constexpr bool alias = coef + w + x + o > LDS_MAX;
+  static constexpr int total = coef + w + x + (alias ? 0 : o);
+  static_assert(o <= x, "the out tile must fit the activation image it may alias");
+  static_assert(8 * 2 * NO * 4 <= x, "the statistic scratch (8 waves x 2 x 128 floats) must fit the activation image");
+  static_assert(total <= LDS_MAX, "LDS");
+};
+
+template <int PRO, int KT>
+__global__ __launch_bounds__(NT, 1) void pw_fwdr_kernel(const CxConv p, const int M, const int m_tiles, const int tiles_per_wg) {
+  extern __shared__ __attribute__((aligned(16))) char smem[];
+  typedef Lds<KT> L;
+  constexpr int K = L::K, cpr = K >> 3, xp = L::xp;
+  constexpr int NCH = (BM * cpr + NT - 1) / NT;
+  float* coef = reinterpret_cast<float*>(smem);
+  char* Wt = smem + L::coef;
+  char* Xl = Wt + L::w;
+  char* Ol = L::alias ? Xl : Xl + L::x;
+
+  const int tid = threadIdx.x, lane = tid & 63, wave = tid >> 6;
+  const int l16 = lane & 15, lq = lane >> 4;
+  const bf16* __restrict__ X = reinterpret_cast<const bf16*>(p.x);
+  const bf16* __restrict__ Wp = reinterpret_cast<const bf16*>(p.w);
+  bf16* __restrict__ Y = reinterpret_cast<bf16*>(p.y);
+
+  const int t0 = blockIdx.x * tiles_per_wg;
+  const int t1 = min(m_tiles, t0 + tiles_per_wg);
+
+  if (PRO == CX_PRO_AFFINE_RELU) {
+    for (int i = tid; i < K; i += NT) {
+      coef[i] = p.pa[i];
+      coef[K + i] = p.pb[i];
+    }
+  }
+  for (int i = tid; i < NO * cpr; i += NT) {
+    const int n = i / cpr, c = i - n * cpr;
+    *reinterpret_cast<uint4*>(Wt + n * xp + c * 16) = *reinterpret_cast<const uint4*>(Wp + (size_t)n * K + c * 8);
+  }
+
+  int srow[NCH], sch[NCH];
+  bool sok[NCH];
+#pragma unroll
+  for (int i = 0; i < NCH; ++i) {
+    const int cid = tid + NT * i;
+    sok[i] = cid < BM * cpr;
+    const int c = sok[i] ? cid : 0;
+    srow[i] = c / cpr;
+    sch[i] = c - srow[i] * cpr;
+  }
+  fr_u32x4 xa[NCH], xb[NCH];
+  auto request = [&](int mt, fr_u32x4 (&xr)[NCH]) __attribute__((always_inline)) {
+    const int mtc = mt < t1 ? mt : t1 - 1;
+#pragma unroll
+    for (int i = 0; i < NCH; ++i) {
+      const int m = mtc * BM + srow[i];
+      const int mc = m < M ? m : M - 1;
+      xr[i] = *reinterpret_cast<const fr_u32x4*>(X + (size_t)mc * p.ldx + sch[i] * 8);
+    }
+  };
+  request(t0, xa);
+  request(t0 + 1, xb);
+
+  float s1[4], s2[4];
+#pragma unroll
+  for (int e = 0; e < 4; ++e) s1[e] = s2[e] = 0.f;
+  const bool want_stats = p.stat_sum != nullptr;
+  const int q = tid & 15, orow = tid >> 4;
+  __syncthreads();
+
+  auto tile = [&](const int mt, fr_u32x4 (&xr)[NCH]) __attribute__((always_inline)) {
+    const int m0 = mt * BM;
+    const bool tvalid = mt < t1;
+#pragma unroll
+    for (int i = 0; i < NCH; ++i) {
+      if (sok[i]) {
+        uint4 v = make_uint4(xr[i][0], xr[i][1], xr[i][2], xr[i][3]);
+        if (PRO == CX_PRO_AFFINE_RELU) {
+          const float* sc = coef + sch[i] * 8;
+          v = cx_affine_relu8(v, sc, sc + K);
+        }
+        const unsigned keep = (tvalid && m0 + srow[i] < M) ? 0xffffffffu : 0u;
+        v.x &= keep; v.y &= keep; v.z &= keep; v.w &= keep;
+        *reinterpret_cast<uint4*>(Xl + srow[i] * xp + sch[i] * 16) = v;
+      }
+    }
+    request(mt + 2, xr);
+    __syncthreads();
+    f32x4 acc[2];
+#pragma unroll
+    for (int h = 0; h < 2; ++h)
+#pragma unroll
+      for (int r = 0; r < 4; ++r) acc[h][r] = 0.f;
+    {
+      const char* Wb = Wt + (wave * 16 + l16) * xp + lq * 16;
+      const char* A0 = Xl + l16 * xp + lq * 16;
+      const char* A1 = A0 + 16 * xp;
+#pragma unroll
+      for (int kk = 0; kk < KT; ++kk) {
+        const bf16x8 wf = *reinterpret_cast<const bf16x8*>(Wb + kk * 64);
+        const bf16x8 a0 = *reinterpret_cast<const bf16x8*>(A0 + kk * 64);
+        const bf16x8 a1 = *reinterpret_cast<const bf16x8*>(A1 + kk * 64);
+        acc[0] = __builtin_amdgcn_mfma_f32_16x16x32_bf16(wf, a0, acc[0], 0, 0, 0);
+        acc[1] = __builtin_amdgcn_mfma_f32_16x16x32_bf16(wf, a1, acc[1], 0, 0, 0);
+      }
+    }
+    if (L::alias) __syncthreads();
+#pragma unroll
+    for (int h = 0; h < 2; ++h) {
+      const int prow = h * 16 + l16;
+      const uint32_t keep = (tvalid && m0 + prow < M) ? 0xffffffffu : 0u;
+      uint32_t w2[2];
+#pragma unroll
+      for (int j = 0; j < 2; ++j) {
+        w2[j] = cx_packbf(acc[h][2 * j], acc[h][2 * j + 1]);
+        if (want_stats) {
+          const uint32_t mk = w2[j] & keep;
+          const float rl = cx_bf_lo(mk), rh = cx_bf_hi(mk);
+          s1[2 * j] += rl;
+          s1[2 * j + 1] += rh;
+          s2[2 * j] += rl * rl;
+          s2[2 * j + 1] += rh * rh;
+        }
+      }
+      *reinterpret_cast<uint2*>(Ol + prow * OP + (wave * 16 + 4 * lq) * 2) = make_uint2(w2[0], w2[1]);
+    }
+    __syncthreads();
+    {
+      const uint4 o = *reinterpret_cast<const uint4*>(Ol + orow * OP + q * 16);
+      if (tvalid && m0 + orow < M) *reinterpret_cast<uint4*>(Y + (size_t)(m0 + orow) * p.ldy + q * 8) = o;
+    }
+    if (L::alias) __syncthreads();
+  };
+
+  const int n_pairs = (t1 - t0 + 1) >> 1;
+  for (int pr = 0; pr < n_pairs; ++pr) {
+    tile(t0 + 2 * pr, xa);
+    tile(t0 + 2 * pr + 1, xb);
+  }
+
+  if (want_stats) {
+    __syncthreads();
+    float* scratch = reinterpret_cast<float*>(Xl);
+    wg_stat_begin<8>(scratch, NO, tid, NT);
+#pragma unroll
+    for (int e = 0; e < 4; ++e) {
+#pragma unroll
+      for (int d = 1; d < 16; d <<= 1) {
+        s1[e] += __shfl_xor(s1[e], d);
+        s2[e] += __shfl_xor(s2[e], d);
+      }
+    }
+    if (l16 == 0) {
+#pragma unroll
+      for (int e = 0; e < 4; ++e) wg_stat_put(scratch, NO, wave, wave * 16 + 4 * lq + e, s1[e], s2[e]);
+    }
+    wg_stat_end<8>(scratch, NO, tid, NT, p.stat_sum, p.stat_sq, p.stat_det, (int)blockIdx.x, p.stat_replicas, p.stat_rstride, 0, p.N);
+  }
+}
+
+template <int PRO, int KT>
+int launch_fwdr(const CxConv& p, hipStream_t st) {
+  const long long M = (long long)p.B * p.Ho * p.Wo;
+  const int m_tiles = (int)((M + BM - 1) / BM);
+  int grid = m_tiles < 256 ? m_tiles : 256;
+  const int tpw = (m_tiles + grid - 1) / grid;
+  grid = (m_tiles + tpw - 1) / tpw;
+  constexpr size_t smem = Lds<KT>::total;
+  static bool attr_set = false;
+  if (!attr_set) {
+    (void)hipFuncSetAttribute(reinterpret_cast<const void*>(&pw_fwdr_kernel<PRO, KT>), hipFuncAttributeMaxDynamicSharedMemorySize, LDS_MAX);
+    attr_set = true;
+  }
+  if (const int e = stat_rows_check(p, grid)) return e;
+  CX_KTAG("pw_fwdr_kernel<%d, %d>", PRO, KT);
+  hipLaunchKernelGGL((pw_fwdr_kernel<PRO, KT>), dim3(grid), dim3(NT), smem, st, p, (int)M, m_tiles, tpw);
+  return launch_status();
+}
+
+template <int PRO>
+int launch_fwdr_n(const CxConv& p, hipStream_t st) {
+  switch (p.K / 32) {
+    case 9: return launch_fwdr<PRO, 9>(p, st);
+    case 10: return launch_fwdr<PRO, 10>(p, st);
+    case 11: return launch_fwdr<PRO, 11>(p, st);
+    case 12: return launch_fwdr<PRO, 12>(p, st);
+    case 13: return launch_fwdr<PRO, 13>(p, st);
+    case 14: return launch_fwdr<PRO, 14>(p, st);
+    default: return launch_fwdr<PRO, 15>(p, st);
+  }
+}
+
+}
+
+int cx_try_pw_fwdr(const CxConv& p, hipStream_t st, bool* handled) {
+  *handled = false;
+  const int form = ((p.kernel_hint >> 8) & 0xff) - 1;
+  const bool forced = form == CX_HINT_PARENT + 4;
+  if ((form >= 0 || (p.kernel_hint & 0xff)) && !forced) return 0;
+  if (p.mode != CX_MODE_CONV || p.kh != 1 || p.kw != 1 || p.stride != 1 || p.pad != 0 || p.tstride > 1) return 0;
+  if (p.epilogue != CX_EPI_STORE || p.accumulate || p.N != NO || (p.K % 32) || p.K <= 256 || p.K > 480) return 0;
+  if (p.prologue != CX_PRO_AFFINE_RELU && p.prologue != CX_PRO_NONE) return 0;
+  if (p.dtype != CX_DT_BF16) return 0;
+  if (!forced && (long long)p.B * p.Ho * p.Wo <= 200000) return 0;
+  *handled = true;
+  return p.prologue == CX_PRO_AFFINE_RELU ? launch_fwdr_n<CX_PRO_AFFINE_RELU>(p, st) : launch_fwdr_n<CX_PRO_NONE>(p, st);
+}
diff --git a/chexpert_amd/csrc/conv1x1_xs.hip b/chexpert_amd/csrc/conv1x1_xs.hip
--- a/chexpert_amd/csrc/conv1x1_xs.hip
+++ b/chexpert_amd/csrc/conv1x1_xs.hip
@@ -291,7 +291,8 @@
 int cx_try_pw_xs(const CxConv& p, hipStream_t st, bool* handled) {
   *handled = false;
   static const int env_on = cx_diag_int("CX_XS", 1);
-  const int hint_on = (p.kernel_hint & 0xff) - 1, hint_form = ((p.kernel_hint >> 8) & 0xff) - 1;
+  const int hint_on = (p.kernel_hint & 0xff) - 1, hint_f = ((p.kernel_hint >> 8) & 0xff) - 1;
+  const int hint_form = hint_f >= CX_HINT_PARENT ? -1 : hint_f;
   if (hint_on == 0 || (hint_form >= 0 && hint_form != 5) || (!env_on && hint_form != 5)) return 0;
   if (p.mode != CX_MODE_CONV || p.dtype != CX_DT_BF16 || p.kh != 1 || p.kw != 1 || p.stride != 1 || p.pad != 0 || p.tstride > 1) return 0;
   if (p.K != 64 && p.K != 128 && p.K != 256) return 0;
diff --git a/chexpert_amd/csrc/conv_gemm.hip b/chexpert_amd/csrc/conv_gemm.hip
--- a/chexpert_amd/csrc/conv_gemm.hip
+++ b/chexpert_amd/csrc/conv_gemm.hip
@@ -389,6 +389,7 @@
 int cx_try_pw_dgrad(const CxConv& p, hipStream_t st, bool* handled);
 int cx_try_pw_fwd(const CxConv& p, hipStream_t st, bool* handled);
 int cx_try_pw_fwdk(const CxConv& p, hipStream_t st, bool* handled);
+int cx_try_pw_fwdr(const CxConv& p, hipStream_t st, bool* handled);
 int cx_try_pw_xs(const CxConv& p, hipStream_t st, bool* handled);
 int cx_try_stem_fwd(const CxConv& p, hipStream_t st, bool* handled);
 int cx_conv_gemm_f32(const CxConv& p, hipStream_t st);
@@ -491,6 +492,8 @@
       if (handled) return rc;
       rc = cx_try_pw_fwd(p, st, &handled);
       if (handled) return rc;
+      rc = cx_try_pw_fwdr(p, st, &handled);
+      if (handled) return rc;
       rc = cx_try_pw_fwdk(p, st, &handled);
       if (handled) return rc;
       rc = cx_try_pw_xs(p, st, &handled);
diff --git a/chexpert_amd/csrc/conv_mm.hip b/chexpert_amd/csrc/conv_mm.hip
--- a/chexpert_amd/csrc/conv_mm.hip
+++ b/chexpert_amd/csrc/conv_mm.hip
@@ -583,7 +583,8 @@
   *handled = false;
   static const int env_on0 = cx_diag_int("CX_MM", 1);
   static const int env_form0 = cx_diag_int("CX_MM_FORM", 0);
-  const int g_mm_on = (p.kernel_hint & 0xff) - 1, g_mm_form = ((p.kernel_hint >> 8) & 0xff) - 1;
+  const int g_mm_on = (p.kernel_hint & 0xff) - 1, hint_f = ((p.kernel_hint >> 8) & 0xff) - 1;
+  const int g_mm_form = hint_f >= CX_HINT_PARENT ? -1 : hint_f;
   const bool pjoin = p.prologue == CX_PRO_JOIN;
   const int env_on = (p.epilogue == CX_EPI_JOIN || pjoin) ? 1 : g_mm_on >= 0 ? g_mm_on : env_on0;
   const int env_form = g_mm_form >= 0 ? g_mm_form : env_form0;
diff --git a/chexpert_amd/ops.py b/chexpert_amd/ops.py
--- a/chexpert_amd/ops.py
+++ b/chexpert_amd/ops.py
@@ -189,6 +189,7 @@
     return (0 if on < 0 else on + 1) | ((0 if form < 0 else form + 1) << 8)
 
 
+HINT_PARENT = 9
 KERNEL_HINT = 0
 
 
diff --git a/include/chexpert_hip.h b/include/chexpert_hip.h
--- a/include/chexpert_hip.h
+++ b/include/chexpert_hip.h
@@ -61,6 +61,7 @@
   int32_t pad2_;
 } CxConv;
 #define CX_KERNEL_HINT(on, form) ((((on) < 0) ? 0 : (on) + 1) | ((((form) < 0) ? 0 : (form) + 1) << 8))
+#define CX_HINT_PARENT 9
 
 typedef struct CxWgrad {
   const void* g; const void* g2;
@@ -149,6 +150,7 @@
 int cx_bn_coef_moments(float* mean, float* rstd, float count, const float* gamma, const float* beta, float eps, float momentum,
                        float* running_mean, float* running_var, float* scale, float* shift, int C, const float* sum, const float* sq,
                        int rows, int rstride, int c_lo, int c_n, void* stream);
+int cx_pw_fwdk_tile(int64_t M, int K);
 int cx_bn_coef_eval(const float* running_mean, const float* running_var, const float* gamma, const float* beta,
                     float eps, float* scale, float* shift, float* mean, float* rstd, int C, void* stream);
 
```

Result: no change. 9799 images/sec, median of 6 (+0.3%).
